# kyotovision-public/DRMNet

Measured on AMD Instinct MI355X. Metric: U-Net denoise steps/sec on 3x128x256 refmaps, higher is better.
Workload: dtype emulated fp32: f16 hi*hi + e4m3 cross terms (~15-bit products), fp32 acc; 1e-4 contract

## Files before the change

### drmnet_amd/_lib.py

```python
from __future__ import annotations

import ctypes as C
import os
from typing import Optional, Sequence

import torch

_HERE = os.path.dirname(os.path.abspath(__file__))
LIB_PATH = os.environ.get("DRM_LIB_PATH") or os.path.join(_HERE, "csrc", "libdrmnet_hip.so")
ABI_VERSION = 3
MAX_LEVELS = 8
LOSS_WORKSPACE_BYTES = 2048
DIFFUSION_LOSS_MAX_PARTS = 32


def diffusion_loss_workspace_bytes(B: int) -> int:
    return int(B) * DIFFUSION_LOSS_MAX_PARTS * 2 * 8


SYMBOLS = [
    "drm_abi_version", "drm_last_error",
    "drm_unet_create", "drm_unet_destroy", "drm_unet_param_count", "drm_unet_param_info", "drm_unet_load_params",
    "drm_unet_workspace_bytes", "drm_unet_forward",
    "drm_linear_forward", "drm_timestep_embedding", "drm_op_norm_act_conv", "drm_op_resblock", "drm_op_attention_block",
    "drm_drmnet_create", "drm_drmnet_destroy", "drm_drmnet_workspace_bytes", "drm_drmnet_set_batch_parts", "drm_drmnet_set_batch_part_min", "drm_drmnet_step", "drm_drmnet_sample",
    "drm_sampler_workspace_bytes", "drm_ddim_sample", "drm_ddim_sample_logged", "drm_ddpm_sample", "drm_ddim_sample_ex", "drm_ddpm_sample_ex", "drm_randn",
    "drm_profile_enable", "drm_profile_reset", "drm_profile_collect", "drm_unet_set_precision", "drm_set_op_precision",
    "drm_refmap_workspace_bytes", "drm_refmap_mask_make", "drm_erode_mask",
    "drm_unet_load_params_set", "drm_unet_use_set", "drm_set_graph_replay", "drm_set_upconv_split", "drm_graph_launches",
    "drm_map_chain", "drm_masked_log_range", "drm_luminance_scale", "drm_mirmap2envmap", "drm_hdr2ldr", "drm_resize", "drm_profile_variants",
    "drm_render_refmap", "drm_brdf_eval", "drm_render_refmap_views", "drm_validation_losses",
    "drm_render_refmap_lit", "drm_render_light_workspace_bytes",
    "drm_render_mesh_workspace_bytes", "drm_render_mesh",
    "drm_mesh_bvh_bytes", "drm_mesh_bvh_build", "drm_mesh_occluded", "drm_render_mesh_shadowed",
    "drm_obs_forward_process", "drm_diffusion_losses",
]


class UNetDesc(C.Structure):
    _fields_ = [
        ("kind", C.c_int32), ("in_channels", C.c_int32), ("model_channels", C.c_int32), ("out_channels", C.c_int32),
        ("num_res_blocks", C.c_int32), ("n_levels", C.c_int32), ("channel_mult", C.c_int32 * MAX_LEVELS),
        ("n_attn", C.c_int32), ("attention_resolutions", C.c_int32 * MAX_LEVELS),
    ]


class MaskBlend(C.Structure):
    _fields_ = [("mask", C.c_void_p), ("mask_channels", C.c_int32), ("x0", C.c_void_p), ("qcoef", C.POINTER(C.c_float)), ("qnoise", C.c_void_p), ("when", C.c_int32)]


class SamplerOptions(C.Structure):
    _fields_ = [("blend", C.POINTER(MaskBlend)), ("uncond", C.c_void_p), ("guidance_scale", C.c_float), ("noise_dropout", C.c_float), ("dropout_keep", C.c_void_p)]


class DrmnetCfg(C.Structure):
    _fields_ = [
        ("z_dim", C.c_int32), ("max_timesteps", C.c_int32), ("gamma", C.c_double), ("epsilon", C.c_float), ("delta", C.c_float),
        ("z0", C.c_float * 8),
    ]


def make_mask_blend(mask, x0, qcoef, qnoise, when: int, img_shape):
    import numpy as np
    import torch

    n, c, h, w = img_shape
    x0 = require_gpu_tensor(x0, "x0").float().contiguous()
    if tuple(x0.shape) != tuple(img_shape):
        raise RuntimeError(f"x0 must be {tuple(img_shape)}")
    mask = require_gpu_tensor(mask, "mask").float()
    if mask.dim() != 4 or mask.shape[2:] != x0.shape[2:] or mask.shape[1] not in (1, c) or mask.shape[0] not in (1, n):
        raise RuntimeError(f"mask must be [N or 1, 1 or {c}, {h}, {w}]")
    mask = mask.expand(n, mask.shape[1], h, w).contiguous()
    qc = np.ascontiguousarray(np.asarray(qcoef, dtype=np.float32))
    qn = None if qnoise is None else require_gpu_tensor(qnoise, "mask_noise").float().contiguous()
    if qn is not None and tuple(qn.shape) != (qc.shape[0],) + tuple(img_shape):
        raise RuntimeError(f"mask_noise must be [steps={qc.shape[0]}, N, C, H, W]")
    b = MaskBlend()
    b.mask, b.mask_channels, b.x0 = mask.data_ptr(), int(mask.shape[1]), x0.data_ptr()
    b.qcoef = qc.ctypes.data_as(C.POINTER(C.c_float))
    b.qnoise = None if qn is None else qn.data_ptr()
    b.when = int(when)
    return b, (mask, x0, qc, qn)


def make_sampler_options(img_shape, steps, blend=None, uncond=None, guidance_scale=1.0, noise_dropout=0.0, dropout_keep=None):
    o = SamplerOptions()
    keep = [blend]
    if blend is not None:
        o.blend = C.pointer(blend[0])
    if uncond is not None:
        u = require_gpu_tensor(uncond, "unconditional_conditioning").float().contiguous()
        if tuple(u.shape) != tuple(img_shape):
            raise RuntimeError(f"unconditional_conditioning must be {tuple(img_shape)}")
        o.uncond = u.data_ptr()
        keep.append(u)
    o.guidance_scale = float(guidance_scale)
    o.noise_dropout = float(noise_dropout)
    if dropout_keep is not None:
        k = require_gpu_tensor(dropout_keep, "dropout_keep").float().contiguous()
        if tuple(k.shape) != (int(steps),) + tuple(img_shape):
            raise RuntimeError(f"dropout_keep must be [steps={steps}, N, C, H, W]")
        o.dropout_keep = k.data_ptr()
        keep.append(k)
    return o, tuple(keep)


_lib: Optional[C.CDLL] = None


def lib() -> C.CDLL:
    global _lib
    if _lib is not None:
        return _lib
    if not os.path.exists(LIB_PATH):
        raise RuntimeError(
            f"{LIB_PATH} is missing: build it with `python -m drmnet_amd.build` (hipcc, gfx950). "
            "drmnet_amd has no CPU / PyTorch fallback for the hot path."
        )
    L = C.CDLL(LIB_PATH)
    vp, i32, i64p, fp = C.c_void_p, C.c_int, C.c_void_p, C.c_void_p
    L.drm_abi_version.restype = C.c_int
    L.drm_last_error.restype = C.c_char_p
    L.drm_unet_create.argtypes = [C.POINTER(UNetDesc), C.POINTER(vp)]
    L.drm_unet_destroy.argtypes = [vp]
    L.drm_unet_destroy.restype = None
    L.drm_unet_param_count.argtypes = [vp]
    L.drm_unet_param_info.argtypes = [vp, i32, C.c_char_p, i32, C.POINTER(C.c_int64), C.POINTER(C.c_int)]
    L.drm_unet_load_params.argtypes = [vp, C.POINTER(vp), i32, vp]
    L.drm_unet_load_params_set.argtypes = [vp, i32, C.POINTER(vp), i32, vp]
    L.drm_unet_use_set.argtypes = [vp, i32]
    L.drm_unet_workspace_bytes.argtypes = [vp, i32, i32, i32]
    L.drm_unet_workspace_bytes.restype = C.c_size_t
    L.drm_unet_forward.argtypes = [vp, fp, i32, fp, i32, vp, fp, i64p, fp, fp, i32, i32, i32, vp, C.c_size_t, vp]
    L.drm_linear_forward.argtypes = [fp, fp, fp, fp, i32, i32, i32, i32, i32, vp]
    L.drm_timestep_embedding.argtypes = [i64p, fp, i32, i32, vp]
    L.drm_op_norm_act_conv.argtypes = [fp, fp, fp, i32, fp, fp, i32, fp, fp, fp, i32, i32, i32, i32, i32, vp]
    L.drm_op_resblock.argtypes = [fp, i32, i32, fp, i32, fp, i32, C.POINTER(vp), i32, fp, i32, i32, i32, i32, vp]
    L.drm_op_attention_block.argtypes = [fp, C.POINTER(vp), fp, i32, i32, i32, i32, vp]
    L.drm_drmnet_create.argtypes = [vp, vp, C.POINTER(vp), C.POINTER(DrmnetCfg), C.POINTER(vp)]
    L.drm_drmnet_destroy.argtypes = [vp]
    L.drm_drmnet_destroy.restype = None
    L.drm_drmnet_workspace_bytes.argtypes = [vp, i32, i32, i32]
    L.drm_drmnet_workspace_bytes.restype = C.c_size_t
    L.drm_drmnet_set_batch_parts.argtypes = [vp, i32]
    L.drm_drmnet_set_batch_parts.restype = i32
    L.drm_drmnet_set_batch_part_min.argtypes = [vp, i32]
    L.drm_drmnet_set_batch_part_min.restype = i32
    L.drm_drmnet_step.argtypes = [vp, fp, fp, vp, i32, i32, fp, C.c_uint64, fp, fp, vp, i32, i32, i32, vp, C.c_size_t, vp]
    L.drm_drmnet_sample.argtypes = [vp, fp, fp, fp, fp, C.c_uint64, i32, fp, fp, vp, C.POINTER(C.c_int32), i32, i32, i32, vp, C.c_size_t, vp]
    L.drm_sampler_workspace_bytes.argtypes = [vp, i32, i32, i32]
    L.drm_sampler_workspace_bytes.restype = C.c_size_t
    L.drm_ddim_sample.argtypes = [vp, fp, fp, C.POINTER(C.c_int64), C.POINTER(C.c_float), i32, i32, fp, C.c_uint64, i32, i32, i32, vp, C.c_size_t, vp]
    L.drm_ddim_sample_logged.argtypes = [vp, fp, fp, C.POINTER(C.c_int64), C.POINTER(C.c_float), i32, i32, fp, C.c_uint64, i32, fp, fp, i32, C.POINTER(C.c_int32),
                                         i32, i32, i32, vp, C.c_size_t, vp]
    L.drm_ddpm_sample.argtypes = [vp, fp, fp, fp, C.POINTER(C.c_float), i32, i32, fp, C.c_uint64, i32, i32, i32, vp, C.c_size_t, vp]
    L.drm_ddim_sample_ex.argtypes = [vp, fp, fp, C.POINTER(C.c_int64), C.POINTER(C.c_float), i32, i32, fp, C.c_uint64, C.POINTER(SamplerOptions), i32, fp, fp, i32,
                                     C.POINTER(C.c_int32), i32, i32, i32, vp, C.c_size_t, vp]
    L.drm_ddpm_sample_ex.argtypes = [vp, fp, fp, fp, C.POINTER(C.c_float), i32, i32, fp, C.c_uint64, C.POINTER(SamplerOptions), i32, i32, i32, vp, C.c_size_t, vp]
    L.drm_randn.argtypes = [fp, C.c_size_t, C.c_uint64, C.c_uint64, vp]
    u8p = vp
    L.drm_refmap_workspace_bytes.argtypes = [C.c_int64, i32, C.c_float]
    L.drm_refmap_workspace_bytes.restype = C.c_size_t
    L.drm_refmap_mask_make.argtypes = [fp, fp, C.c_int64, i32, i32, C.c_float, i32, fp, u8p, vp, C.c_size_t, vp]
    L.drm_erode_mask.argtypes = [u8p, i32, i32, i32, u8p, vp]
    L.drm_unet_set_precision.argtypes = [vp, i32]
    L.drm_set_op_precision.argtypes = [i32]
    L.drm_profile_enable.argtypes = [i32]
    L.drm_profile_enable.restype = None
    L.drm_profile_reset.restype = None
    L.drm_profile_collect.argtypes = [C.POINTER(C.c_double), C.POINTER(C.c_double), C.POINTER(C.c_double), C.POINTER(C.c_int64)]
    L.drm_set_graph_replay.argtypes = [i32]
    L.drm_set_upconv_split.argtypes = [i32]
    L.drm_graph_launches.restype = C.c_int64
    L.drm_map_chain.argtypes = [fp, fp, C.c_int64, i32, C.POINTER(C.c_int32), C.POINTER(C.c_float), i32, fp, fp, fp, vp]
    L.drm_masked_log_range.argtypes = [fp, fp, i32, i32, i32, fp, fp, vp]
    L.drm_luminance_scale.argtypes = [fp, i32, i32, C.c_float, fp, vp]
    L.drm_mirmap2envmap.argtypes = [fp, fp, fp, i32, i32, i32, i32, i32, i32, i32, i32, vp]
    L.drm_hdr2ldr.argtypes = [fp, u8p, i32, C.c_float, C.c_float, fp, vp]
    L.drm_resize.argtypes = [fp, fp, i32, i32, i32, i32, i32, i32, vp]
    L.drm_profile_variants.argtypes = [C.c_char_p, C.c_size_t]
    L.drm_profile_variants.restype = C.c_size_t
    L.drm_render_refmap.argtypes = [fp, fp, fp, i32, i32, i32, i32, i32, i32, i32, vp]
    L.drm_brdf_eval.argtypes = [fp, i32, fp, fp, fp, fp, C.c_int64, vp]
    L.drm_render_refmap_views.argtypes = [fp, i32, fp, fp, fp, i32, i32, i32, i32, i32, i32, i32, vp]
    L.drm_render_refmap_lit.argtypes = [fp, i32, fp, fp, fp, i32, i32, i32, i32, i32, i32, i32, i32, vp, C.c_size_t, vp]
    L.drm_render_light_workspace_bytes.argtypes = [i32, i32, i32, i32]
    L.drm_render_light_workspace_bytes.restype = C.c_size_t
    L.drm_render_mesh_workspace_bytes.argtypes = [C.c_int64, i32, i32, i32, i32]
    L.drm_render_mesh_workspace_bytes.restype = C.c_size_t
    L.drm_render_mesh.argtypes = [fp, fp, vp, C.c_int64, C.c_int64, fp, fp, fp, fp, fp, fp, fp, i32, i32, i32, i32, i32, i32, i32, vp, C.c_size_t, vp]
    L.drm_mesh_bvh_bytes.argtypes = [C.c_int64]
    L.drm_mesh_bvh_bytes.restype = C.c_size_t
    L.drm_mesh_bvh_build.argtypes = [fp, vp, C.c_int64, C.c_int64, vp, C.c_size_t]
    L.drm_mesh_occluded.argtypes = [fp, vp, C.c_int64, C.c_int64, vp, fp, fp, vp, vp, C.c_int64, vp]
    L.drm_render_mesh_shadowed.argtypes = [fp, fp, vp, C.c_int64, C.c_int64, fp, fp, fp, fp, fp, fp, fp, i32, i32, i32, i32, i32, i32, i32, vp, C.c_size_t,
                                           vp, C.c_size_t, vp]
    L.drm_validation_losses.argtypes = [fp, fp, fp, vp, fp, fp, fp, vp, fp, C.c_double, i32, C.c_double, C.c_double, i32, C.c_int64, i32, vp, C.c_size_t,
                                        fp, vp]
    L.drm_obs_forward_process.argtypes = [fp, fp, vp, fp, fp, i32, C.c_float, i32, fp, fp, fp, C.c_uint64, fp, fp, fp, i32, i32, i32, i32, i32, i32, vp]
    L.drm_diffusion_losses.argtypes = [fp, fp, fp, vp, fp, fp, i32, i32, C.c_double, C.c_double, i32, C.c_int64, i32, vp, C.c_size_t, fp, fp, vp]
    if L.drm_abi_version() != ABI_VERSION:
        raise RuntimeError(f"libdrmnet_hip.so ABI version {L.drm_abi_version()} != {ABI_VERSION}: rebuild with `python -m drmnet_amd.build`")
    _lib = L
    return L


def check(status: int) -> None:
    if status != 0:
        msg = lib().drm_last_error()
        raise RuntimeError(f"drmnet_hip error {status}: {msg.decode() if msg else '?'}")


def ptr(t: Optional[torch.Tensor]) -> Optional[int]:
    return None if t is None else t.data_ptr()


def stream_ptr(device=None) -> int:
    return torch.cuda.current_stream(device).cuda_stream


def require_gpu_tensor(t: torch.Tensor, name: str, dtype=torch.float32) -> torch.Tensor:
    if not t.is_cuda:
        raise RuntimeError(f"{name} must live on the GPU (drmnet_amd has no CPU path); got device {t.device}")
    if t.dtype != dtype:
        raise RuntimeError(f"{name} must be {dtype}, got {t.dtype}")
    return t.contiguous()


def ptr_array(tensors: Sequence[torch.Tensor]):
    arr = (C.c_void_p * len(tensors))()
    for i, t in enumerate(tensors):
        arr[i] = t.data_ptr()
    return arr


class Workspace:

    def __init__(self):
        self.buf: Optional[torch.Tensor] = None

    def get(self, nbytes: int, device) -> torch.Tensor:
        if nbytes == 0:
            raise RuntimeError(f"workspace query failed: {lib().drm_last_error().decode()}")
        if self.buf is None or self.buf.numel() < nbytes or self.buf.device != torch.device(device):
            self.buf = None
            self.buf = torch.empty(nbytes, dtype=torch.uint8, device=device)
        return self.buf
```

### drmnet_amd/csrc/abi.hip

```cpp
#include <atomic>
#include <cstring>
#include <memory>

#include "bvh.h"
#include "profiler.h"
#include "samplers.h"

using namespace drm;

struct drm_unet {
  UNet net;
};
struct drm_drmnet {
  DrmnetSampler s;
};

namespace {

int make_arena(Arena& ar, void* ws, size_t bytes, size_t need) {
  if (need == 0) return DRM_ERR_INVALID;
  if (bytes < need || ws == nullptr) {
    set_error("workspace too small: need " + std::to_string(need) + " bytes, got " + std::to_string(bytes));
    return DRM_ERR_WORKSPACE;
  }
// ... 271 lines not shown
  });
}
void drm_drmnet_destroy(drm_drmnet* s) { delete s; }

size_t drm_drmnet_workspace_bytes(const drm_drmnet* s, int N, int H, int W) {
  if (!s) return 0;
  size_t r = 0;
  guarded([&]() -> int {
    r = s->s.workspace_bytes(N, H, W);
    return DRM_OK;
  });
  return r;
}

int drm_drmnet_set_batch_parts(drm_drmnet* s, int parts) {
  return guarded([&]() -> int {
    DRM_REQUIRE(s != nullptr, "drm_drmnet_set_batch_parts: null handle");
    DRM_REQUIRE(parts >= 1 && parts <= DrmnetSampler::PART_MAX, "drm_drmnet_set_batch_parts: 1 .. 4 parts");
    s->s.parts = parts;
    return DRM_OK;
  });
}

int drm_drmnet_set_batch_part_min(drm_drmnet* s, int rows) {
  return guarded([&]() -> int {
    DRM_REQUIRE(s != nullptr, "drm_drmnet_set_batch_part_min: null handle");
    DRM_REQUIRE(rows >= 1, "drm_drmnet_set_batch_part_min: at least one row per part");
    s->s.part_min = rows;
    return DRM_OK;
  });
}

int drm_drmnet_step(drm_drmnet* s, float* Lr_k, const float* LrK, const int32_t* rows, int n_active, int step, const float* noise,
                    uint64_t seed, float* zk_out, float* zK_out, int32_t* converged_out, int B, int H, int W, void* workspace,
                    size_t workspace_bytes, void* stream) {
  return guarded([&]() -> int {
    DRM_REQUIRE(s && Lr_k && LrK, "null argument");
    Arena ar;
    DRM_TRY(make_arena(ar, workspace, workspace_bytes, s->s.workspace_bytes(n_active, H, W)));
    return s->s.step(Lr_k, LrK, rows, n_active, step, noise, seed, zk_out, zK_out, converged_out, B, H, W, ar, static_cast<hipStream_t>(stream));
  });
}

int drm_drmnet_sample(drm_drmnet* s, const float* LrK, const float* cond, const float* noise0, const float* step_noise, uint64_t seed, int early_exit,
                      float* Lr0, float* zK, int32_t* K, int32_t* steps_done, int B, int H, int W, void* workspace, size_t workspace_bytes,
                      void* stream) {
  return guarded([&]() -> int {
    DRM_REQUIRE(s && LrK && cond && Lr0 && zK && K, "null argument");
    Arena ar;
    DRM_TRY(make_arena(ar, workspace, workspace_bytes, s->s.workspace_bytes(B, H, W)));
    return s->s.sample(LrK, cond, noise0, step_noise, seed, early_exit, Lr0, zK, K, steps_done, B, H, W, ar, static_cast<hipStream_t>(stream));
  });
}

size_t drm_sampler_workspace_bytes(const drm_unet* net, int N, int H, int W) {
  if (!net) return 0;
  size_t r = 0;
  guarded([&]() -> int {
    r = sampler_workspace_bytes(&const_cast<drm_unet*>(net)->net, N, H, W);
    return DRM_OK;
  });
  return r;
}

int drm_ddim_sample(drm_unet* net, float* x, const float* cond, const int64_t* timesteps, const float* coef, int S, int num_steps,
                    const float* noise, uint64_t seed, int N, int H, int W, void* workspace, size_t workspace_bytes, void* stream) {
  return guarded([&]() -> int {
    DRM_REQUIRE(net && x && cond, "null argument");
    const ChainIO io{x, cond, noise, seed, N, H, W};
    return run_chain(net, io, workspace, workspace_bytes, [&](Arena& ar) {
      return ddim_sample(&net->net, io, timesteps, coef, S, num_steps, ChainLog{}, drm_sampler_options{}, ar, static_cast<hipStream_t>(stream));
    });
  });
}

int drm_ddim_sample_logged(drm_unet* net, float* x, const float* cond, const int64_t* timesteps, const float* coef, int S, int num_steps,
                           const float* noise, uint64_t seed, int log_every_t, float* log_x, float* log_pred_x0, int log_slots, int32_t* n_logged, int N,
                           int H, int W, void* workspace, size_t workspace_bytes, void* stream) {
  return guarded([&]() -> int {
    DRM_REQUIRE(net && x && cond, "null argument");
    DRM_REQUIRE(log_every_t > 0 && log_x && log_pred_x0 && log_slots > 0, "ddim intermediates: log_every_t, both log buffers and their slot count");
    const ChainIO io{x, cond, noise, seed, N, H, W};
    const ChainLog log{log_every_t, log_x, log_pred_x0, log_slots, n_logged};
    return run_chain(net, io, workspace, workspace_bytes, [&](Arena& ar) {
      return ddim_sample(&net->net, io, timesteps, coef, S, num_steps, log, drm_sampler_options{}, ar, static_cast<hipStream_t>(stream));
    });
  });
}

int drm_ddpm_sample(drm_unet* net, float* x, float* pred_x0, const float* cond, const float* coef, int T_start, int clip_denoised,
                    const float* noise, uint64_t seed, int N, int H, int W, void* workspace, size_t workspace_bytes, void* stream) {
  return guarded([&]() -> int {
    DRM_REQUIRE(net && x && cond, "null argument");
    const ChainIO io{x, cond, noise, seed, N, H, W};
    return run_chain(net, io, workspace, workspace_bytes, [&](Arena& ar) {
      return ddpm_sample(&net->net, io, pred_x0, coef, T_start, clip_denoised, drm_sampler_options{}, ar, static_cast<hipStream_t>(stream));
    });
  });
}

int drm_ddim_sample_ex(drm_unet* net, float* x, const float* cond, const int64_t* timesteps, const float* coef, int S, int num_steps,
                       const float* noise, uint64_t seed, const drm_sampler_options* opt, int log_every_t, float* log_x, float* log_pred_x0, int log_slots,
                       int32_t* n_logged, int N, int H, int W, void* workspace, size_t workspace_bytes, void* stream) {
  return guarded([&]() -> int {
    DRM_REQUIRE(net && x && cond && opt, "null argument");
    DRM_REQUIRE(log_every_t <= 0 || (log_x && log_pred_x0 && log_slots > 0), "ddim intermediates: both log buffers and their slot count");
    const ChainIO io{x, cond, noise, seed, N, H, W};
    ChainLog log{0, nullptr, nullptr, log_slots, n_logged};
    if (log_every_t > 0) log = ChainLog{log_every_t, log_x, log_pred_x0, log_slots, n_logged};
    return run_chain(net, io, workspace, workspace_bytes, [&](Arena& ar) {
      return ddim_sample(&net->net, io, timesteps, coef, S, num_steps, log, *opt, ar, static_cast<hipStream_t>(stream));
    });
  });
}

int drm_ddpm_sample_ex(drm_unet* net, float* x, float* pred_x0, const float* cond, const float* coef, int T_start, int clip_denoised,
                       const float* noise, uint64_t seed, const drm_sampler_options* opt, int N, int H, int W, void* workspace, size_t workspace_bytes,
                       void* stream) {
  return guarded([&]() -> int {
    DRM_REQUIRE(net && x && cond && opt, "null argument");
    DRM_REQUIRE(opt->uncond == nullptr, "drm_ddpm_sample_ex: classifier-free guidance exists on the DDIM chain only (ddim.py:225-232; ddpm.py p_sample has none)");
    const ChainIO io{x, cond, noise, seed, N, H, W};
    return run_chain(net, io, workspace, workspace_bytes, [&](Arena& ar) {
      return ddpm_sample(&net->net, io, pred_x0, coef, T_start, clip_denoised, *opt, ar, static_cast<hipStream_t>(stream));
    });
  });
}

int drm_unet_set_precision(drm_unet* net, int precision) {
  return guarded([&]() -> int {
    DRM_REQUIRE(net && precision_valid(precision),
                "precision must be 0 (fp32 MFMA), 1 (split fp16 x3), 2 (plain fp16 operands), 3 (split fp16 with fp8 cross terms) or 4 (plain bf16 operands)");
    net->net.precision = precision;
    return DRM_OK;
  });
}
int drm_set_op_precision(int precision) {
  return guarded([&]() -> int {
    DRM_REQUIRE(precision_valid(precision),
                "precision must be 0 (fp32 MFMA), 1 (split fp16 x3), 2 (plain fp16 operands), 3 (split fp16 with fp8 cross terms) or 4 (plain bf16 operands)");
    g_op_precision.store(precision, std::memory_order_relaxed);
    return DRM_OK;
  });
}

int drm_set_upconv_split(int mode) {
  return guarded([&]() -> int {
    DRM_REQUIRE(mode >= 0 && mode <= 2, "upconv split mode: 0 = never, 1 = by the measured rule, 2 = wherever the form applies");
    set_upconv_split(mode);
    return DRM_OK;
  });
}

int drm_set_graph_replay(int on) {
  set_graph_replay(on != 0);
  return DRM_OK;
}
int64_t drm_graph_launches(void) { return (int64_t)graph_launches(); }

void drm_profile_enable(int on) { prof_enable(on); }
void drm_profile_reset(void) { prof_reset(); }
int drm_profile_collect(double* ms, double* flops, double* bytes, int64_t* launches) {
  return guarded([&]() -> int {
    DRM_REQUIRE(ms && flops && bytes && launches, "null argument");
    prof_collect(ms, flops, bytes, launches);
    return DRM_OK;
  });
}

int drm_randn(float* out, size_t n, uint64_t seed, uint64_t offset, void* stream) {
  return guarded([&]() -> int { return launch_randn(out, n, seed, offset, static_cast<hipStream_t>(stream)); });
}

size_t drm_refmap_workspace_bytes(int64_t n, int res, float angle_threshold) {
  if (n < 0 || res <= 0 || !(angle_threshold >= 0.f)) return 0;
  return refmap_workspace_bytes(n, res, angle_threshold);
}

int drm_refmap_mask_make(const float* colors, const float* normals, int64_t n, int channels, int res, float angle_threshold, int min_points,
                         float* refmap, uint8_t* refmask, void* workspace, size_t workspace_bytes, void* stream) {
  return guarded([&]() -> int {
    DRM_REQUIRE(refmap && refmask && workspace && (n == 0 || (colors && normals)), "drm_refmap_mask_make: null pointer");
    return launch_refmap_mask_make(colors, normals, n, channels, res, angle_threshold, min_points, refmap, refmask, workspace, workspace_bytes,
                                   static_cast<hipStream_t>(stream));
  });
}

int drm_erode_mask(const uint8_t* mask, int H, int W, int kernel_size, uint8_t* out, void* stream) {
  return guarded([&]() -> int {
    DRM_REQUIRE(mask && out, "drm_erode_mask: null pointer");
    return launch_erode_mask(mask, H, W, kernel_size, out, static_cast<hipStream_t>(stream));
  });
}


int drm_map_chain(const float* x, float* out, int64_t per_image, int B, const int32_t* ops, const float* args, int n_ops, const float* lo,
                  const float* hi, const float* scale, void* stream) {
  return guarded([&]() -> int { return launch_map_chain(x, out, per_image, B, ops, args, n_ops, lo, hi, scale, static_cast<hipStream_t>(stream)); });
}

int drm_masked_log_range(const float* x, const float* mask, int B, int C, int HW, float* lo, float* hi, void* stream) {
  return guarded([&]() -> int { return launch_masked_log_range(x, mask, B, C, HW, lo, hi, static_cast<hipStream_t>(stream)); });
}

int drm_luminance_scale(const float* x, int B, int HW, float scaler, float* scale, void* stream) {
  return guarded([&]() -> int { return launch_luminance_scale(x, B, HW, scaler, scale, static_cast<hipStream_t>(stream)); });
}

int drm_mirmap2envmap(const float* mirmap, const float* basis, float* out, int B, int C, int H, int W, int OH, int OW, int log_scale_interpolation,
                      int channels_last, void* stream) {
  return guarded([&]() -> int {
    return launch_mirmap2envmap(mirmap, basis, out, B, C, H, W, OH, OW, log_scale_interpolation, channels_last, static_cast<hipStream_t>(stream));
  });
}

int drm_hdr2ldr(const float* x, const uint8_t* mask, int HW, float alpha, float gamma, float* out, void* stream) {
  return guarded([&]() -> int { return launch_hdr2ldr(x, mask, HW, alpha, gamma, out, static_cast<hipStream_t>(stream)); });
}

size_t drm_profile_variants(char* buf, size_t cap) { return prof_variants_text(buf, cap); }

int drm_resize(const float* x, float* out, int planes, int IH, int IW, int OH, int OW, int mode, void* stream) {
  return guarded([&]() -> int { return launch_resize(x, out, planes, IH, IW, OH, OW, mode, static_cast<hipStream_t>(stream)); });
}


int drm_render_refmap(const float* z, const float* envmap, float* out, int B, int R, int EH, int EW, int quad, int subpixel, int flip, void* stream) {
  return guarded([&]() -> int {
    return launch_render_refmap(z, envmap, out, B, R, EH, EW, quad, subpixel, flip, static_cast<hipStream_t>(stream));
  });
}

int drm_render_refmap_views(const float* z, int L, const float* envmap, const float* view, float* out, int B, int R, int EH, int EW, int quad,
                            int subpixel, int flip, void* stream) {
  return guarded([&]() -> int {
    return launch_render_refmap_views(z, L, envmap, view, out, B, R, EH, EW, quad, subpixel, flip, static_cast<hipStream_t>(stream));
  });
}

size_t drm_render_light_workspace_bytes(int B, int EH, int EW, int light_samples) { return render_light_workspace_bytes(B, EH, EW, light_samples); }

int drm_render_refmap_lit(const float* z, int L, const float* envmap, const float* view, float* out, int B, int R, int EH, int EW, int quad, int subpixel,
                          int flip, int light_samples, void* workspace, size_t workspace_bytes, void* stream) {
  return guarded([&]() -> int {
    return launch_render_refmap_lit(z, L, envmap, view, out, B, R, EH, EW, quad, subpixel, flip, light_samples, workspace, workspace_bytes,
                                    static_cast<hipStream_t>(stream));
  });
}

size_t drm_render_mesh_workspace_bytes(int64_t F, int B, int H, int W, int subpixel) {
  return render_mesh_workspace_bytes((long long)F, B, H, W, subpixel);
}

int drm_render_mesh(const float* vertex_positions, const float* vertex_normals, const int32_t* faces, int64_t V, int64_t F, const float* z,
                    const float* envmap, const float* view, float* image, float* normal, float* depth, float* alpha, int B, int H, int W, int EH, int EW,
                    int quad, int subpixel, void* workspace, size_t workspace_bytes, void* stream) {
  return guarded([&]() -> int {
    return launch_render_mesh(vertex_positions, vertex_normals, faces, (long long)V, (long long)F, z, envmap, view, image, normal, depth, alpha, B, H, W,
                              EH, EW, quad, subpixel, workspace, workspace_bytes, static_cast<hipStream_t>(stream));
  });
}

size_t drm_mesh_bvh_bytes(int64_t F) { return mesh_bvh_bytes((long long)F); }

int drm_mesh_bvh_build(const float* vertex_positions, const int32_t* faces, int64_t V, int64_t F, void* bvh, size_t bytes) {
  return guarded([&]() -> int { return mesh_bvh_build(vertex_positions, faces, (long long)V, (long long)F, bvh, bytes); });
}

int drm_mesh_occluded(const float* vertex_positions, const int32_t* faces, int64_t V, int64_t F, const void* bvh, const float* origins, const float* dirs,
                      const int32_t* exclude, int32_t* out, int64_t N, void* stream) {
  return guarded([&]() -> int {
    return launch_mesh_occluded(vertex_positions, faces, (long long)V, (long long)F, bvh, origins, dirs, exclude, out, (long long)N,
                                static_cast<hipStream_t>(stream));
  });
}

int drm_render_mesh_shadowed(const float* vertex_positions, const float* vertex_normals, const int32_t* faces, int64_t V, int64_t F, const float* z,
                             const float* envmap, const float* view, float* image, float* normal, float* depth, float* alpha, int B, int H, int W, int EH,
                             int EW, int quad, int subpixel, void* workspace, size_t workspace_bytes, const void* bvh, size_t bvh_bytes, void* stream) {
  return guarded([&]() -> int {
    return launch_render_mesh_shadowed(vertex_positions, vertex_normals, faces, (long long)V, (long long)F, z, envmap, view, image, normal, depth, alpha, B,
                                       H, W, EH, EW, quad, subpixel, workspace, workspace_bytes, bvh, bvh_bytes, static_cast<hipStream_t>(stream));
  });
}

int drm_brdf_eval(const float* z, int z_rows, const float* n, const float* v, const float* l, float* out, int64_t N, void* stream) {
  return guarded([&]() -> int { return launch_brdf_eval(z, z_rows, n, v, l, out, (long long)N, static_cast<hipStream_t>(stream)); });
}


int drm_validation_losses(const float* model_out, const float* Lr_k, const float* Lr_km1, const int32_t* K, const float* z_out, const float* z_k,
                          const float* z_K, const int32_t* reversed_k, const float* z0, double gamma, int loss_type, double l_refmap_weight,
                          double l_refcode_weight, int B, int64_t per_row, int P, void* workspace, size_t workspace_bytes, float* out, void* stream) {
  return guarded([&]() -> int {
    return launch_validation_losses(model_out, Lr_k, Lr_km1, K, z_out, z_k, z_K, reversed_k, z0, gamma, loss_type, l_refmap_weight, l_refcode_weight, B,
                                    (long long)per_row, P, static_cast<double*>(workspace), workspace_bytes, out, static_cast<hipStream_t>(stream));
  });
}


int drm_obs_forward_process(const float* x, const float* mask, const int32_t* t, const float* sqrt_alphas_cumprod,
                            const float* sqrt_one_minus_alphas_cumprod, int T, float noisy_observe, int padding_mode, const float* e_observe,
                            const float* e_padding, const float* e_q, uint64_t seed, float* cond, float* x_noisy, float* noise, int B, int C, int H,
                            int W, int mask_H, int mask_W, void* stream) {
  return guarded([&]() -> int {
    return launch_obs_forward_process(x, mask, t, sqrt_alphas_cumprod, sqrt_one_minus_alphas_cumprod, T, noisy_observe, padding_mode, e_observe, e_padding,
// ... 16 lines not shown
```

### drmnet_amd/csrc/common.h

```cpp
#pragma once
#include <hip/hip_runtime.h>
#include <stdint.h>
#include <stdio.h>
#include <string>
#include "gn_fold.h"

namespace drm {

void set_error(const std::string& msg);
const char* last_error();

#define DRM_OK 0
#define DRM_ERR_INVALID 1
#define DRM_ERR_HIP 2
#define DRM_ERR_WORKSPACE 3
#define DRM_ERR_STATE 4

#define DRM_HIP_CHECK(expr)                                                                              \
  do {                                                                                                   \
    hipError_t _e = (expr);                                                                              \
    if (_e != hipSuccess) {                                                                              \
      ::drm::set_error(std::string(#expr) + " failed: " + hipGetErrorString(_e) + " at " + __FILE__ + ":" + \
                       std::to_string(__LINE__));                                                        \
      return DRM_ERR_HIP;                                                                                \
    }                                                                                                    \
  } while (0)

#define DRM_REQUIRE(cond, msg)                                    \
  do {                                                            \
    if (!(cond)) {                                                \
      ::drm::set_error(std::string("invalid argument: ") + (msg)); \
      return DRM_ERR_INVALID;                                     \
    }                                                             \
  } while (0)

#define DRM_TRY(expr)          \
  do {                         \
    int _s = (expr);           \
    if (_s != DRM_OK) return _s; \
  } while (0)

struct DeviceInfo {
  int ordinal = 0;
  int cus = 0;
  int xcds = 0;
  size_t lds_per_cu = 0;
};
const DeviceInfo* device_info();


struct ConvArgs {
  const float* src0 = nullptr;
  const float* src1 = nullptr;
  int C0 = 0, C1 = 0, up0 = 0;
  int N = 0, H = 0, W = 0;
  const float* gn_scale = nullptr;
  const float* gn_shift = nullptr;
  int silu = 0;
  const float* w = nullptr;
  const float* bias = nullptr;
  int taps = 9;
  int Cout = 0;
  const float* emb = nullptr;
  int emb_stride = 0;
  const float* res = nullptr;
  float* out = nullptr;
  int out_nchw = 0, cout_valid = 0;
  int cin_real = 0;
  int ksplit = 1;
  size_t split_stride = 0;
  float* split_ws = nullptr;
  unsigned* tile_ticket = nullptr;
  int terms = 3;
  int mx_site = 0;
#ifdef DRM_S2_STAMP
  unsigned* stamp_out = nullptr;
  int stamp_block = 0, stamp_tile0 = 0;
#endif
  double2* stat_out = nullptr;
  float* pool_out = nullptr;
  double2* pool_stat = nullptr;
  const float* w_inv_scale = nullptr;
  int ld0 = 0;
  int gn_ld = 0;
  long long w_img_stride_f4 = 0;
  const float* w_inv_img = nullptr;
  int prof_kind = -1;
  const float* in_inv = nullptr;
  GnFold gnf;
};
enum ConvKernel : unsigned char { CONV_NONE, CONV_IGEMM, CONV_PIPELINE };
enum ConvTile : unsigned char { TILE_256x256, TILE_256x192, TILE_256x128, TILE_128x128, TILE_256x64, TILE_128x64, TILE_128x32 };
enum SplitFinish : unsigned char { SPLIT_NONE, SPLIT_IN_LAUNCH, SPLIT_REDUCE };
struct ConvPlan {
  ConvKernel kernel = CONV_NONE;
  int terms = 0;
  ConvTile tile = TILE_128x32;
  int th = 0, tw = 0;
  bool ragged = false;
  int kc = 32;
  int ksplit = 1;
  SplitFinish finish = SPLIT_NONE;
  size_t tickets = 0;
  bool pool = false;
  bool gn_fold = false;
  bool split() const { return kernel == CONV_PIPELINE && terms != 0; }
};
ConvPlan plan_conv(const ConvArgs& a, int precision, bool want_pool = false, bool gn_foldable = false);
bool conv_split_weights(int precision, int cin);
int launch_conv(const ConvArgs& a, const ConvPlan& p, hipStream_t s);
int conv_tile_family(int H, int W, const int (*fam)[2], int n_fam);
size_t packed_conv_weight_split_floats(int taps, int CoutP, int CinP);
int launch_pack_conv_weight_split(const float* w, float* packed, float* scales, unsigned* scratch, int Cout, int Cin, int taps, int CoutP,
                                  int CinP, hipStream_t s, bool mx = false, bool bf16 = false);
enum Precision { PREC_FP32 = 0, PREC_F16X3 = 1, PREC_F16 = 2, PREC_F16MX = 3, PREC_BF16 = 4 };
inline bool precision_valid(int p) { return p >= PREC_FP32 && p <= PREC_BF16; }
inline int precision_terms(int p) { return p == PREC_F16 ? 1 : (p == PREC_BF16 ? 4 : (p == PREC_FP32 ? 0 : 3)); }
int launch_pack_conv_weight(const float* w, float* packed, int Cout, int Cin, int taps, int CoutP, int CinP, hipStream_t s);
int pack_conv_image(int precision, const float* w, float* packed, float* scale, unsigned* scratch, int Cout, int Cin, int taps, int CoutP, int CinP,
                    bool mx_site, hipStream_t s);
int launch_fold_upconv_weight(const float* w, float* wa, float* wb, int Cout, int C0, int C1, hipStream_t s);
int launch_fold_attn_params(const float* qkv_w, const float* qkv_b, const float* proj_w, const float* proj_b, float* w_out, float* b_out, int C,
                            hipStream_t s);
size_t packed_conv_weight_floats(int taps, int CoutP, int CinP);

int launch_chan_moments(const float* x, int N, int HW, int C, double* partial , double2* mom , hipStream_t s);
int chan_moments_splits(int HW, int C);
int launch_act_pow2_scale(const double2* mom0, int C0, int lo0, int hi0, double cnt0, const double2* mom1, int C1, double cnt1,
                          const unsigned* absmax_bits, int Ctab, int N, float* scale, float* shift, float* inv, hipStream_t s, int absmax_parts = 1);
int launch_gn_finalize(const double2* mom0, int C0, double inv0, const double2* mom1, int C1, double inv1, const float* gamma,
                       const float* beta, int N, float* scale, float* shift, hipStream_t s, double cnt0 = 0.0, double cnt1 = 0.0,
                       float* guard_scale = nullptr, float* guard_shift = nullptr, float* guard_inv = nullptr);

size_t refmap_workspace_bytes(long long n, int res, float thr);
int launch_refmap_mask_make(const float* colors, const float* normals, long long n, int C, int res, float thr, int min_points, float* refmap,
                            unsigned char* refmask, void* ws, size_t ws_bytes, hipStream_t s);
int launch_erode_mask(const unsigned char* mask, int H, int W, int k, unsigned char* out, hipStream_t s);
enum AttnForm : unsigned char {
  ATTN_SMALL,
  ATTN_CONV,
  ATTN_FLASH
};
struct AttnPlan {
  AttnForm form = ATTN_SMALL;
  int N = 0, H = 0, W = 0, C = 0;
  int terms = 0;
  bool split_qk = false, split_pv = false, guard = false;
  int group = 1;
  size_t scores_floats = 0;
  size_t ws_floats = 0;
  bool out_stats = true;
  ConvPlan qk[2], pv[2];
};
AttnPlan plan_attention(int N, int H, int W, int C, int precision);
struct AttnTables {
  float *wq = nullptr, *wk = nullptr, *wv = nullptr;
  float *q_tab = nullptr, *p_tab = nullptr, *zero_tab = nullptr;
  float *qk_inv = nullptr, *k_scale = nullptr, *k_inv = nullptr, *pv_inv = nullptr, *v_scale = nullptr, *v_inv = nullptr;
  float* q_scale = nullptr;
};
int launch_attention_core(const AttnPlan& p, const float* qkv, const double2* qkv_mom, const float* x, float* scores, float* out, double2* out_stat,
                          float* ws, hipStream_t s);
bool attention_flash_applicable(int T, int C, int terms);
int launch_attention_flash(const AttnPlan& p, const AttnTables& t, const float* qkv, const float* x, float* out, hipStream_t s);

int launch_map_chain(const float* x, float* out, long long per_image, int B, const int32_t* ops, const float* args, int n_ops, const float* lo,
                     const float* hi, const float* scale, hipStream_t s);
int launch_masked_log_range(const float* x, const float* mask, int B, int C, int HW, float* lo, float* hi, hipStream_t s);
int launch_luminance_scale(const float* x, int B, int HW, float scaler, float* scale, hipStream_t s);
int launch_mirmap2envmap(const float* mir, const float* basis, float* out, int B, int C, int H, int W, int OH, int OW, int log_interp, int nhwc,
                         hipStream_t s);
int launch_hdr2ldr(const float* x, const unsigned char* mask, int HW, float alpha, float gamma, float* out, hipStream_t s);
int launch_resize(const float* x, float* out, int planes, int IH, int IW, int OH, int OW, int mode, hipStream_t s);

int launch_render_refmap(const float* z, const float* env, float* out, int B, int R, int EH, int EW, int quad, int subpixel, int flip, hipStream_t s);
int launch_render_refmap_views(const float* z, int L, const float* env, const float* view, float* out, int B, int R, int EH, int EW, int quad,
                               int subpixel, int flip, hipStream_t s);
size_t render_light_workspace_bytes(int B, int EH, int EW, int light_samples);
int launch_render_refmap_lit(const float* z, int L, const float* env, const float* view, float* out, int B, int R, int EH, int EW, int quad, int subpixel,
                             int flip, int light_samples, void* workspace, size_t workspace_bytes, hipStream_t s);
constexpr int kMeshRecordWords = 20, kMeshHitWords = 4;
constexpr int kMeshRecIndex = 14, kMeshRecValid = 17;
__host__ __device__ __forceinline__ float mesh_sample_x(int c, int WS) { return (float)(2 * c + 1) / (float)WS - 1.0f; }
__host__ __device__ __forceinline__ float mesh_sample_y(int r, int HS, float aspect) { return aspect * (1.0f - (float)(2 * r + 1) / (float)HS); }
size_t render_mesh_workspace_bytes(long long F, int B, int H, int W, int subpixel);
int launch_mesh_visibility(const float* positions, const int32_t* faces, long long V, long long F, const float* view, int B, int H, int W, int subpixel,
                           float* records, float* hits, hipStream_t s);
int launch_render_mesh(const float* positions, const float* normals, const int32_t* faces, long long V, long long F, const float* z, const float* env,
                       const float* view, float* image, float* normal, float* depth, float* alpha, int B, int H, int W, int EH, int EW, int quad,
                       int subpixel, void* workspace, size_t workspace_bytes, hipStream_t s);
int launch_render_mesh_shadowed(const float* positions, const float* normals, const int32_t* faces, long long V, long long F, const float* z,
                                const float* env, const float* view, float* image, float* normal, float* depth, float* alpha, int B, int H, int W, int EH,
                                int EW, int quad, int subpixel, void* workspace, size_t workspace_bytes, const void* bvh, size_t bvh_bytes, hipStream_t s);
int launch_validation_losses(const float* model_out, const float* Lr_k, const float* Lr_km1, const int32_t* K, const float* z_out, const float* z_k,
                             const float* z_K, const int32_t* reversed_k, const float* z0, double gamma, int loss_type, double w_refmap,
                             double w_refcode, int B, long long per_row, int P, double* ws, size_t ws_bytes, float* out, hipStream_t s);
int launch_obs_forward_process(const float* x, const float* mask, const int32_t* t, const float* sqrt_ac, const float* sqrt_1mac, int T,
                               float noisy_observe, int padding_mode, const float* e_obs, const float* e_pad, const float* e_q, uint64_t seed,
                               float* cond, float* x_noisy, float* noise, int B, int C, int H, int W, int mask_H, int mask_W, hipStream_t s);
int launch_diffusion_losses(const float* model_out, const float* target, const float* invmask, const int32_t* t, const float* logvar,
                            const float* lvlb, int T, int loss_type, double w_simple, double w_elbo, int B, long long per_row, int C, double* ws,
                            size_t ws_bytes, float* out, float* rows_out, hipStream_t s);
int launch_brdf_eval(const float* z, int z_rows, const float* n, const float* v, const float* l, float* out, long long N, hipStream_t s);

int pack_input_absmax_parts(int H, int W);
int launch_pack_input(const float* x, const float* cond, const int* idx, float* out, int N, int H, int W, int Cx, int Cc, int CP, hipStream_t s,
                      unsigned* absmax_bits = nullptr);
int launch_avgpool2(const float* x, float* out, int N, int H, int W, int C, hipStream_t s, double2* stat = nullptr);
int launch_linear(const float* in, const float* w, const float* b, float* out, int N, int I, int O, int silu_in, int silu_out, hipStream_t s);
int launch_timestep_embedding(const int64_t* t, const float* tf, float* out, int N, int dim, hipStream_t s);
int launch_encoder_head(const float* x, const float* scale, const float* shift, const float* w, const float* b, float* out, int N, int HW,
                        int C, int O, hipStream_t s);
bool stem_direct_applicable(int Cin, int Cout);
size_t stem_weight_floats();
int launch_pack_stem_weight(const float* w, float* img, int Cout, int Cin, bool exact, hipStream_t s);
int launch_stem_conv(const float* x, int Cx, const float* cond, int Cc, const int* rows, const float* wimg, const float* bias, float* out, double2* stat,
                     int N, int H, int W, int Cout, bool exact, hipStream_t s);
int launch_nhwc_to_nchw(const float* x, float* out, int N, int H, int W, int C, hipStream_t s);
int launch_nchw_to_nhwc(const float* x, float* out, int N, int H, int W, int C, hipStream_t s);

}
```

### drmnet_amd/csrc/conv_split2.hip

```cpp
#include <algorithm>
#include <atomic>
#include <utility>
#include <vector>
#include <cstdio>
#include <string>

#include "common.h"
#include "profiler.h"

#ifdef DRM_S2_STAMP
#define S2_STAMP(id)                                                                               \
  do {                                                                                             \
    if (stamp_on && stamp_n < 120) {                                                               \
      unsigned long long t_;                                                                       \
      __builtin_amdgcn_sched_barrier(0);                                                           \
      asm volatile("s_memtime %0\n\ts_waitcnt lgkmcnt(0)" : "=s"(t_)::"memory");                   \
      __builtin_amdgcn_sched_barrier(0);                                                           \
      if (lane == 0) {                                                                             \
        stamp_lds[(wave * 120 + stamp_n) * 2] = (unsigned)(id);                                    \
        stamp_lds[(wave * 120 + stamp_n) * 2 + 1] = (unsigned)t_;                                  \
      }                                                                                            \
      ++stamp_n;                                                                                   \
    }                                                                                              \
  } while (0)
// ... 51 lines not shown
  static constexpr int G_PER = TPS * B_PER;
  static constexpr int G_F4 = TPS * B_F4;
  static constexpr int ST_F4 = TN * BN;
  static constexpr int LDS_F4 = A_F4 + R * G_F4 + ST_F4;
  static constexpr int A_CNT = 2 * A_SLOTS + 4;
  static __device__ __forceinline__ void rowmap(int row, int& img, int& py, int& px) {
    if constexpr (SUB48) {
      constexpr int SPI = (TH / 4) * (TW / 8);
      const int q = row >> 5, rr = row & 31;
      img = q / SPI;
      const int qq = q % SPI;
      py = (qq / (TW / 8)) * 4 + (rr >> 3);
      px = (qq % (TW / 8)) * 8 + (rr & 7);
    } else {
      img = row / (TH * TW);
      py = (row / TW) % TH;
      px = row % TW;
    }
  }
  static_assert(TAPS == 9 || TAPS == 4 || TAPS == 1, "3x3, 1x1, or the four parity 2x2 convs of a 3x3 over a nearest-x2 input");
  static_assert(TAPS % TPS == 0, "taps per step must divide the taps");
  static_assert(B_DMA_F4 % 64 == 0 && B_PER >= 1, "whole 1-KiB LDS-DMA instructions; a wave issues B_PER of them or none");
  static_assert(TERMS == 4 || TERMS == 3 || TERMS == 2 || TERMS == 1 || TERMS == 0,
                "3 = fp16 hi/lo split (fp32 accuracy), 2 = fp16 hi*hi + both cross terms in one block-scaled fp8 MFMA, 1 = plain fp16 operands, 4 = plain bf16 operands, 0 = fp32 operands (exact fp32 MFMA)");
  static_assert(ONE || B_DMA_F4 % NTHR == 0, "split mode: every wave owns the same number of distinct 1-KiB pieces");
  static_assert(TH * TW * TN == BM && TPI % OCT == 0 && TPI >= OCT, "tile / loader mapping");
  static_assert(R >= 2, "ring needs >= 2 slots");
};

__device__ __forceinline__ float silu2(float v) { return v * __builtin_amdgcn_rcpf(1.0f + __expf(-v)); }
__device__ __forceinline__ void split2(float v, _Float16& hi, _Float16& lo) {
  const float c = __builtin_amdgcn_fmed3f(v, -65504.0f, 65504.0f);
  hi = (_Float16)c;
  lo = (_Float16)fmaf((float)hi, -1.0f, c);
}
typedef float f32x2 __attribute__((ext_vector_type(2)));
typedef _Float16 f16x2 __attribute__((ext_vector_type(2)));
__device__ __forceinline__ unsigned cvt_pk_f16(float a, float b) { return __builtin_bit_cast(unsigned, __builtin_convertvector(f32x2{a, b}, f16x2)); }
template <int HALF>
__device__ __forceinline__ float sub_packed_f16(float c, unsigned pk) {
  float r;
  if constexpr (HALF == 0) asm("v_fma_mix_f32 %0, %1, 1.0, -%2 op_sel_hi:[0,0,1]" : "=v"(r) : "v"(c), "v"(pk));
  else asm("v_fma_mix_f32 %0, %1, 1.0, -%2 op_sel:[0,0,1] op_sel_hi:[0,0,1]" : "=v"(r) : "v"(c), "v"(pk));
  return r;
}
__device__ __forceinline__ void split8(const float (&v)[8], float lim_n, float lim_p, float (&c8)[8], unsigned (&hi)[4], float (&l8)[8]) {
#pragma unroll
  for (int k = 0; k < 8; ++k) c8[k] = __builtin_amdgcn_fmed3f(v[k], lim_n, lim_p);
#pragma unroll
  for (int k = 0; k < 4; ++k) {
    hi[k] = cvt_pk_f16(c8[2 * k], c8[2 * k + 1]);
    l8[2 * k] = sub_packed_f16<0>(c8[2 * k], hi[k]);
    l8[2 * k + 1] = sub_packed_f16<1>(c8[2 * k + 1], hi[k]);
  }
}
union F4H8b {
  float4 f4;
  f16x8 h8;
  bf16x8 b8;
};

template <int N>
__device__ __forceinline__ void wait_vmcnt() {
  static_assert(N >= 0 && N < 64, "vmcnt is a 6-bit counter");
  asm volatile("s_waitcnt vmcnt(%0)" ::"n"(N) : "memory");
}

__device__ __forceinline__ void glds16s(const void* sbase, unsigned voff, unsigned lds_dst) {
  unsigned keep;
  asm volatile("s_mov_b32 %0, m0\n\ts_mov_b32 m0, %3\n\ts_nop 0\n\tglobal_load_lds_dwordx4 %1, %2\n\ts_mov_b32 m0, %0"
               : "=&s"(keep)
               : "v"(voff), "s"(sbase), "s"(lds_dst)
               : "memory");
}
__device__ __forceinline__ void glds16(const void* gsrc, unsigned lds_dst) {
  unsigned keep;
  asm volatile("s_mov_b32 %0, m0\n\ts_mov_b32 m0, %2\n\ts_nop 0\n\tglobal_load_lds_dwordx4 %1, off\n\ts_mov_b32 m0, %0"
               : "=&s"(keep)
               : "v"(gsrc), "s"(lds_dst)
               : "memory");
}

typedef float f32x4 __attribute__((ext_vector_type(4)));
__device__ __forceinline__ void gload16x2(f32x4& d0, f32x4& d1, const void* p) {
  asm volatile("global_load_dwordx4 %0, %2, off\n\tglobal_load_dwordx4 %1, %2, off offset:16" : "=&v"(d0), "=&v"(d1) : "v"(p) : "memory");
}
__device__ __forceinline__ void tie_regs(f32x4& x0, f32x4& x1) { asm volatile("" : "+v"(x0), "+v"(x1)::"memory"); }
#ifdef DRM_SK_FENCED
__device__ __forceinline__ void gstore16_agent(void* p, const f32x4& v) { asm volatile("global_store_dwordx4 %0, %1, off\n\ts_nop 1" ::"v"(p), "v"(v) : "memory"); }
__device__ __forceinline__ void gload16_agent(f32x4& d, const void* p) { asm volatile("global_load_dwordx4 %0, %1, off" : "=&v"(d) : "v"(p) : "memory"); }
#else
__device__ __forceinline__ void gstore16_agent(void* p, const f32x4& v) { asm volatile("global_store_dwordx4 %0, %1, off sc1\n\ts_nop 1" ::"v"(p), "v"(v) : "memory"); }
__device__ __forceinline__ void gload16_agent(f32x4& d, const void* p) { asm volatile("global_load_dwordx4 %0, %1, off sc1" : "=&v"(d) : "v"(p) : "memory"); }
#endif
__device__ __forceinline__ void tie_reg(f32x4& x) { asm volatile("" : "+v"(x)::"memory"); }

template <int CTRL>
__device__ __forceinline__ float quad_perm(float x) {
  return __builtin_bit_cast(float, __builtin_amdgcn_update_dpp(0, __builtin_bit_cast(int, x), CTRL, 0xF, 0xF, false));
}
__device__ __forceinline__ void quad_transpose(float& x0, float& x1, float& x2, float& x3, int lane) {
  const bool b0 = lane & 1, b1 = lane & 2;
  float t;
  t = quad_perm<0xB1>(b0 ? x0 : x1);
  if (b0) x0 = t; else x1 = t;
  t = quad_perm<0xB1>(b0 ? x2 : x3);
  if (b0) x2 = t; else x3 = t;
  t = quad_perm<0x4E>(b1 ? x0 : x2);
  if (b1) x0 = t; else x2 = t;
  t = quad_perm<0x4E>(b1 ? x1 : x3);
  if (b1) x1 = t; else x3 = t;
}

template <int... I, typename F>
__device__ __forceinline__ void static_for(std::integer_sequence<int, I...>, F&& f) {
  (f(std::integral_constant<int, I>{}), ...);
}

struct TilePos {
  int n0, ty0, tx0, co0;
  long long wofs;
};

template <int TAPS, int TH, int TW, int WM, int WN, int MT, int NT, int R, int TPS, int TERMS = 3, bool RAG = false, bool SK = false, bool POOL = false>
__global__ __launch_bounds__(WM* WN * 64, 2) void conv_split2_kernel(ConvArgs a) {
  using C = S2Cfg<TAPS, TH, TW, WM, WN, MT, NT, R, TPS, TERMS>;
  static_assert(!POOL || (C::SUB48 && C::TN == 1 && !RAG && !SK), "pooled output: one-image tiles of 4 x 8 patches");
  extern __shared__ float4 lds[];
  float4* As = lds;
  float4* Bs = lds + C::A_F4;
  double* lst = reinterpret_cast<double*>(lds + C::A_F4 + R * C::G_F4);
  [[maybe_unused]] double* lst2 = lst + C::TN * C::BN * 2;

#ifndef DRM_NO_KERNARG_TOUCH
  {
    typedef const __attribute__((address_space(4))) int* kptr_t;
    kptr_t ka = (kptr_t)__builtin_amdgcn_kernarg_segment_ptr();
    int touch = 0;
#pragma unroll
    for (int o = 0; o < (int)sizeof(ConvArgs); o += 64) touch ^= __builtin_nontemporal_load(ka + o / 4);
    asm volatile("" ::"s"(touch));
  }
#endif
  const int tid = threadIdx.x;
  const int lane = tid & 63;
  const int wave = __builtin_amdgcn_readfirstlane(tid >> 6);
  const int r = lane & 31, h = lane >> 5;
  const int wm = wave / WN, wn = wave % WN;

  const int tiles_x = RAG ? (a.W + TW - 1) / TW : a.W / TW, tiles_y = RAG ? (a.H + TH - 1) / TH : a.H / TH;
  const int n_tiles = a.Cout / C::BN;
  const int total = ((a.N + C::TN - 1) / C::TN) * tiles_y * tiles_x * n_tiles;
  const int xcd = blockIdx.x & 7, jx = blockIdx.x >> 3;
  const int q8 = total >> 3, r8 = total & 7;
  const int x_start = xcd < r8 ? xcd * (q8 + 1) : r8 * (q8 + 1) + (xcd - r8) * q8;
  const int x_count = q8 + (xcd < r8 ? 1 : 0);
  const int J = ((int)gridDim.x - xcd + 7) >> 3;
  auto decode = [&](int logical) {
    TilePos t;
    const int n_tile = logical % n_tiles;
    int m_tile = logical / n_tiles;
    const int tx = m_tile % tiles_x;
    m_tile /= tiles_x;
    const int ty = m_tile % tiles_y;
    t.n0 = (m_tile / tiles_y) * C::TN;
    t.ty0 = ty * TH;
    t.tx0 = tx * TW;
    t.co0 = n_tile * C::BN;
    t.wofs = t.co0 + (long long)t.n0 * a.w_img_stride_f4;
    return t;
  };
  int k_tile = jx;
  if (k_tile >= x_count) return;
  TilePos cur = decode(x_start + k_tile);
#ifdef DRM_S2_STAMP
  unsigned* stamp_lds = reinterpret_cast<unsigned*>(lds + C::LDS_F4);
  int stamp_n = 0;
  int stamp_tiles = 0;
  bool stamp_on = false;
  if (a.stamp_out && (int)blockIdx.x == (a.stamp_block & 0xFFFF))
    for (int k = tid; k < C::NW * 240; k += C::NTHR) stamp_lds[k] = 0;
  stamp_on = a.stamp_out && (int)blockIdx.x == (a.stamp_block & 0xFFFF) && a.stamp_tile0 == 0;
  S2_STAMP(60);
#endif

  const int Ctot = a.C0 + a.C1;
  const int nch_all = Ctot / C::KC;
  const int ks = a.ksplit > 1 ? a.ksplit : 1;
  const int split = blockIdx.y;
  const int chunk0 = split * nch_all / ks;
  const int nchunks = (split + 1) * nch_all / ks - chunk0;
  const int NGT = nchunks * C::NG;
  constexpr bool FUSE = SK;
  static_assert(!SK || (WM == 4 && WN == 1 && MT == 1 && NT == 1 && !RAG), "split-K launches use the 128-row x 32-channel tiles (plan_conv)");
  const bool fused = FUSE && ks > 1 && a.split_ws != nullptr;
  float* const out_s = (fused ? a.split_ws : a.out) + (size_t)split * a.split_stride;
  const bool has_gn = a.gn_scale != nullptr;

  const int l_img = tid / C::TPI;
  const int l_tid = tid % C::TPI;
  const int l_o = tid % C::OCT;
  f32x4 areg[C::A_SLOTS][2];
  f32x4 sc[2], sh[2];
  unsigned avalid = 0;

  auto load_A_piece = [&](const TilePos& tp, int chunk, int piece) {
    const int c = (chunk0 + chunk) * C::KC;
    const float* src;
    int Cs, coff, up;
    if (c < a.C0) {
      src = a.src0; Cs = a.ld0 ? a.ld0 : a.C0; coff = c; up = a.up0;
    } else {
      src = a.src1; Cs = a.C1; coff = c - a.C0; up = 0;
    }
    const int Hs = up ? (a.H >> 1) : a.H, Ws = up ? (a.W >> 1) : a.W;
    const int l_n = tp.n0 + l_img;
    const int l_nc = l_n < a.N ? l_n : a.N - 1;
    if (piece == 0) avalid = 0;
#pragma unroll
    for (int j = 0; j < C::A_SLOTS; ++j) {
      if (j != piece) continue;
      const int lidx = l_tid + C::TPI * j;
      const int hpl = lidx / C::OCT;
      const int hy = hpl / C::WT, hx = hpl % C::WT;
      const int y = tp.ty0 + hy - C::HALO, x = tp.tx0 + hx - C::HALO;
      const bool ok = (lidx < C::HPI * C::OCT) && (l_n < a.N) && (y >= 0) && (y < a.H) && (x >= 0) && (x < a.W);
      const int yc = min(max(y, 0), a.H - 1), xc = min(max(x, 0), a.W - 1);
      const int ys = up ? (yc >> 1) : yc, xs = up ? (xc >> 1) : xc;
      const size_t pix = ((size_t)l_nc * Hs + ys) * Ws + xs;
      gload16x2(areg[j][0], areg[j][1], src + pix * Cs + coff + 8 * l_o);
      if (ok) avalid |= 1u << j;
    }
    if (piece == C::A_SLOTS) {
      const int tab_ld = a.gn_ld ? a.gn_ld : Ctot;
      const float* gs = has_gn ? a.gn_scale + (size_t)l_nc * tab_ld + c + 8 * l_o : a.src0;
      const float* gb = has_gn ? a.gn_shift + (size_t)l_nc * tab_ld + c + 8 * l_o : a.src0;
      gload16x2(sc[0], sc[1], gs);
      gload16x2(sh[0], sh[1], gb);
    }
  };
  auto load_A = [&](const TilePos& tp, int chunk) {
#pragma unroll
    for (int p = 0; p <= C::A_SLOTS; ++p) load_A_piece(tp, chunk, p);
  };
  auto tie_A = [&]() {
#pragma unroll
    for (int j = 0; j < C::A_SLOTS; ++j) tie_regs(areg[j][0], areg[j][1]);
    tie_regs(sc[0], sc[1]);
    tie_regs(sh[0], sh[1]);
  };
  auto transform_A_slot = [&](int j) {
    const int lidx = l_tid + C::TPI * j;
    if (lidx < C::HPI * C::OCT) {
      float v[8] = {areg[j][0].x, areg[j][0].y, areg[j][0].z, areg[j][0].w, areg[j][1].x, areg[j][1].y, areg[j][1].z, areg[j][1].w};
      if (has_gn) {
        const float s8[8] = {sc[0].x, sc[0].y, sc[0].z, sc[0].w, sc[1].x, sc[1].y, sc[1].z, sc[1].w};
        const float b8[8] = {sh[0].x, sh[0].y, sh[0].z, sh[0].w, sh[1].x, sh[1].y, sh[1].z, sh[1].w};
#pragma unroll
        for (int k = 0; k < 8; ++k) v[k] = fmaf(v[k], s8[k], b8[k]);
      }
      if (a.silu) {
#pragma unroll
        for (int k = 0; k < 8; ++k) v[k] = silu2(v[k]);
      }
      const bool ok = (avalid >> j) & 1u;
      if constexpr (TERMS == 0) {
        areg[j][0] = ok ? f32x4{v[0], v[1], v[2], v[3]} : f32x4{0.f, 0.f, 0.f, 0.f};
        areg[j][1] = ok ? f32x4{v[4], v[5], v[6], v[7]} : f32x4{0.f, 0.f, 0.f, 0.f};
      } else if constexpr (TERMS == 2) {
        float c8[8], l8[8];
        unsigned hi[4];
        split8(v, ok ? -MX_A_LIM : 0.f, ok ? MX_A_LIM : 0.f, c8, hi, l8);
        s16x2 q[4];
#pragma unroll
        for (int k = 0; k < 2; ++k) {
          s16x2 z = {0, 0};
          z = __builtin_amdgcn_cvt_scalef32_pk_fp8_f32(z, l8[4 * k], l8[4 * k + 1], MX_AL_DIV, false);
          q[k] = __builtin_amdgcn_cvt_scalef32_pk_fp8_f32(z, l8[4 * k + 2], l8[4 * k + 3], MX_AL_DIV, true);
          s16x2 y = {0, 0};
          y = __builtin_amdgcn_cvt_scalef32_pk_fp8_f32(y, c8[4 * k], c8[4 * k + 1], MX_AH_DIV, false);
          q[2 + k] = __builtin_amdgcn_cvt_scalef32_pk_fp8_f32(y, c8[4 * k + 2], c8[4 * k + 3], MX_AH_DIV, true);
        }
        areg[j][0] = f32x4{__builtin_bit_cast(float, hi[0]), __builtin_bit_cast(float, hi[1]), __builtin_bit_cast(float, hi[2]), __builtin_bit_cast(float, hi[3])};
        areg[j][1] = f32x4{__builtin_bit_cast(float, q[0]), __builtin_bit_cast(float, q[1]), __builtin_bit_cast(float, q[2]), __builtin_bit_cast(float, q[3])};
      } else if constexpr (TERMS == 4) {
        F4H8b hi;
#pragma unroll
        for (int k = 0; k < 8; ++k) hi.b8[k] = (__bf16)(ok ? v[k] : 0.f);
        areg[j][0] = f32x4{hi.f4.x, hi.f4.y, hi.f4.z, hi.f4.w};
      } else {
        float c8[8], l8[8];
        unsigned hi[4];
        split8(v, ok ? -65504.0f : 0.f, ok ? 65504.0f : 0.f, c8, hi, l8);
        areg[j][0] = f32x4{__builtin_bit_cast(float, hi[0]), __builtin_bit_cast(float, hi[1]), __builtin_bit_cast(float, hi[2]), __builtin_bit_cast(float, hi[3])};
        if constexpr (TERMS == 3)
          areg[j][1] = f32x4{__builtin_bit_cast(float, cvt_pk_f16(l8[0], l8[1])), __builtin_bit_cast(float, cvt_pk_f16(l8[2], l8[3])),
                             __builtin_bit_cast(float, cvt_pk_f16(l8[4], l8[5])), __builtin_bit_cast(float, cvt_pk_f16(l8[6], l8[7]))};
      }
    }
  };
  auto write_A_slot = [&](float4* Ad, int j) {
    const int lidx = l_tid + C::TPI * j;
    if (lidx < C::HPI * C::OCT) {
      const int hpl = lidx / C::OCT;
      const int pixel = l_img * C::HPIP + (hpl / C::WT) * C::WTP + (hpl % C::WT);
      const float4 w0 = make_float4(areg[j][0].x, areg[j][0].y, areg[j][0].z, areg[j][0].w);
      const float4 w1 = make_float4(areg[j][1].x, areg[j][1].y, areg[j][1].z, areg[j][1].w);
      if constexpr (TERMS == 0) {
        Ad[(2 * l_o) * C::HPS + pixel] = w0;
        Ad[(2 * l_o + 1) * C::HPS + pixel] = w1;
      } else if constexpr (TERMS == 2) {
        Ad[l_o * C::HPS + pixel] = w0;
        reinterpret_cast<float2*>(Ad + (4 + (l_o >> 1)) * C::HPS + pixel)[l_o & 1] = make_float2(w1.x, w1.y);
        reinterpret_cast<float2*>(Ad + (6 + (l_o >> 1)) * C::HPS + pixel)[l_o & 1] = make_float2(w1.z, w1.w);
      } else {
        Ad[l_o * C::HPS + pixel] = w0;
        if (TERMS == 3) Ad[(4 + l_o) * C::HPS + pixel] = w1;
      }
    }
  };
  auto transform_A = [&]() {
    tie_A();
#pragma unroll
    for (int j = 0; j < C::A_SLOTS; ++j) transform_A_slot(j);
  };
  auto write_A = [&](float4* Ad) {
#pragma unroll
    for (int j = 0; j < C::A_SLOTS; ++j) write_A_slot(Ad, j);
  };
  auto store_A = [&](float4* Ad) {
    transform_A();
    write_A(Ad);
  };
  const unsigned lds_bs = __builtin_amdgcn_readfirstlane(
      (unsigned)(uintptr_t)(__attribute__((address_space(3))) void*)(Bs));
  unsigned dma_voff[C::B_PER];
#pragma unroll
  for (int j = 0; j < C::B_PER; ++j) {
    const int idx = (wave * 64 + C::NTHR * j) % C::B_DMA_F4 + lane;
    dma_voff[j] = (unsigned)((idx / C::BN) * a.Cout + idx % C::BN) * 16u;
  }
  auto issue_G1 = [&](int gseq, int g_in_tile, long long co0, int k) {
    const int slot = gseq % R;
    const int chunk = g_in_tile / C::NG, g = g_in_tile - chunk * C::NG;
    const int u = k / C::B_PER, j = k % C::B_PER;
    const int tap = g * TPS + u;
    const float4* wp = reinterpret_cast<const float4*>(a.w) + (((size_t)tap * nch_all + chunk0 + chunk) * 8) * a.Cout + co0;
    const int base = (wave * 64 + C::NTHR * j) % C::B_DMA_F4;
    unsigned vo = dma_voff[0];
#pragma unroll
    for (int jj = 1; jj < C::B_PER; ++jj) vo = (j == jj) ? dma_voff[jj] : vo;
    glds16s(wp, vo, lds_bs + (unsigned)(slot * C::G_F4 + u * C::B_F4 + base) * 16u);
  };
  auto issue_G = [&](int gseq, int g_in_tile, long long co0) {
    const int slot = gseq % R;
    const int chunk = g_in_tile / C::NG, g = g_in_tile - chunk * C::NG;
#pragma unroll
    for (int u = 0; u < TPS; ++u) {
      const int tap = g * TPS + u;
      const float4* wp = reinterpret_cast<const float4*>(a.w) + (((size_t)tap * nch_all + chunk0 + chunk) * 8) * a.Cout + co0;
#pragma unroll
      for (int j = 0; j < C::B_PER; ++j) {
        const int base = (wave * 64 + C::NTHR * j) % C::B_DMA_F4;
        glds16s(wp, dma_voff[j], lds_bs + (unsigned)(slot * C::G_F4 + u * C::B_F4 + base) * 16u);
      }
    }
  };

  int a_base[MT], b_base[NT];
#pragma unroll
  for (int i = 0; i < MT; ++i) {
    const int row = (wm * MT + i) * 32 + r;
    int img, py, px;
    C::rowmap(row, img, py, px);
    a_base[i] = img * C::HPIP + py * C::WTP + px;
  }
#pragma unroll
  for (int c = 0; c < NT; ++c) b_base[c] = (wn * NT + c) * 32 + r;

  f32x16 acc[MT][NT];
#pragma unroll
  for (int i = 0; i < MT; ++i)
#pragma unroll
    for (int c = 0; c < NT; ++c)
#pragma unroll
      for (int e = 0; e < 16; ++e) acc[i][c][e] = 0.f;

  const float inv_scale = a.w_inv_scale ? *a.w_inv_scale : 1.0f;
  constexpr int PPI = TH * TW;
  const bool st = a.stat_out != nullptr;
  if (st) {
    for (int k = tid; k < C::TN * C::BN * 2; k += C::NTHR) lst[k] = 0.0;
  }
  if constexpr (POOL) {
    for (int k = tid; k < C::TN * C::BN * 2; k += C::NTHR) lst2[k] = 0.0;
  }

  int gseq = 0;
  {
    int k2 = k_tile;
    TilePos tp = cur;
    int gi = 0;
#pragma unroll
    for (int G = 0; G < R - 1; ++G) {
      if (gi >= NGT) {
        gi = 0;
        if (k2 + J < x_count) {
          k2 += J;
          tp = decode(x_start + k2);
        }
      }
      issue_G(gseq++, gi++, tp.wofs);
    }
  }
  S2_STAMP(61);
  if (a.gnf.mom0) {
    float* scr = reinterpret_cast<float*>(As);
    const bool tab_in_lds = a.N == 1 && (80 + 2 * Ctot) * (int)sizeof(float) <= C::A_F4 * 16;
#pragma unroll
    for (int p = 0; p < C::A_SLOTS; ++p) load_A_piece(cur, 0, p);
    for (int n = 0; n < a.N; ++n) gn_finalize_image(a.gnf, n, tid, C::NTHR, scr, tab_in_lds ? scr + 80 : nullptr);
    S2_STAMP(62);
    wait_vmcnt<0>();
    if (!tab_in_lds) {
      gn_lds_barrier();
      load_A_piece(cur, 0, C::A_SLOTS);
    } else {
      const float4* t4 = reinterpret_cast<const float4*>(scr + 80 + chunk0 * C::KC + 8 * l_o);
      const float4 s0 = t4[0], s1 = t4[1], b0 = t4[Ctot / 4], b1 = t4[Ctot / 4 + 1];
      sc[0] = f32x4{s0.x, s0.y, s0.z, s0.w}; sc[1] = f32x4{s1.x, s1.y, s1.z, s1.w};
      sh[0] = f32x4{b0.x, b0.y, b0.z, b0.w}; sh[1] = f32x4{b1.x, b1.y, b1.z, b1.w};
      gn_lds_barrier();
    }
  } else {
    load_A(cur, 0);
  }
  wait_vmcnt<0>();
  S2_STAMP(63);
  store_A(As);
  if (TAPS == 1) {
    if (nchunks > 1) load_A(cur, 1);
    else if (k_tile + J < x_count) load_A(decode(x_start + k_tile + J), 0);
  }
  asm volatile("s_waitcnt lgkmcnt(0)" ::: "memory");
  __builtin_amdgcn_s_barrier();
  S2_STAMP(64);

  constexpr int A_G = (C::NG >= 3) ? C::NG - 2 : 0;
  const bool y_first = (C::NW == 8) && (wave >= C::NW / 2);
  if (TAPS != 1 && C::NW == 8 && wave >= C::NW / 2) __builtin_amdgcn_s_setprio(1);
  constexpr int BASE = C::G_PER * (R - 2);
  int step = 0;
  while (true) {
    const bool has_next = k_tile + J < x_count;
    const TilePos nxt = has_next ? decode(x_start + k_tile + J) : cur;
#ifdef DRM_S2_STAMP
    stamp_on = a.stamp_out && (int)blockIdx.x == (a.stamp_block & 0xFFFF) && stamp_tiles >= a.stamp_tile0;
    ++stamp_tiles;
    S2_STAMP(1);
#endif
    [[maybe_unused]] int par_off = 0;
    if constexpr (TAPS == 4) {
      const int par = cur.co0 / (a.Cout >> 2);
      par_off = __builtin_amdgcn_readfirstlane((par >> 1) * C::WTP + (par & 1));
    }
    auto mma_tap = [&](const float4* Ab, const float4* Bc, int tapoff, auto&& hook) {
      if constexpr (TERMS == 0) {
#pragma unroll
        for (int j = 0; j < 4; ++j) {
          const int gi = 2 * j + h;
          float4 af[MT], bf[NT];
#pragma unroll
          for (int i = 0; i < MT; ++i) af[i] = Ab[gi * C::HPS + a_base[i] + tapoff];
#pragma unroll
          for (int c = 0; c < NT; ++c) bf[c] = Bc[gi * C::BN + b_base[c]];
#pragma unroll
          for (int i = 0; i < MT; ++i)
#pragma unroll
            for (int c = 0; c < NT; ++c) {
              acc[i][c] = __builtin_amdgcn_mfma_f32_32x32x2f32(af[i].x, bf[c].x, acc[i][c], 0, 0, 0);
              acc[i][c] = __builtin_amdgcn_mfma_f32_32x32x2f32(af[i].y, bf[c].y, acc[i][c], 0, 0, 0);
              acc[i][c] = __builtin_amdgcn_mfma_f32_32x32x2f32(af[i].z, bf[c].z, acc[i][c], 0, 0, 0);
              acc[i][c] = __builtin_amdgcn_mfma_f32_32x32x2f32(af[i].w, bf[c].w, acc[i][c], 0, 0, 0);
            }
          if (j == 0 || j == 2) {
            __builtin_amdgcn_sched_barrier(0);
            hook(j >> 1);
            __builtin_amdgcn_sched_barrier(0);
          }
        }
        return;
      }
      if constexpr (TERMS == 2) {
        {
          i32x8 am[MT], bm[NT];
#pragma unroll
          for (int i = 0; i < MT; ++i) {
            const float4 p0 = Ab[(4 + h) * C::HPS + a_base[i] + tapoff], p1 = Ab[(6 + h) * C::HPS + a_base[i] + tapoff];
            am[i] = i32x8{__builtin_bit_cast(int, p0.x), __builtin_bit_cast(int, p0.y), __builtin_bit_cast(int, p0.z), __builtin_bit_cast(int, p0.w),
                          __builtin_bit_cast(int, p1.x), __builtin_bit_cast(int, p1.y), __builtin_bit_cast(int, p1.z), __builtin_bit_cast(int, p1.w)};
          }
#pragma unroll
          for (int c = 0; c < NT; ++c) {
            const float4 p0 = Bc[(4 + h) * C::BN + b_base[c]], p1 = Bc[(6 + h) * C::BN + b_base[c]];
            bm[c] = i32x8{__builtin_bit_cast(int, p0.x), __builtin_bit_cast(int, p0.y), __builtin_bit_cast(int, p0.z), __builtin_bit_cast(int, p0.w),
                          __builtin_bit_cast(int, p1.x), __builtin_bit_cast(int, p1.y), __builtin_bit_cast(int, p1.z), __builtin_bit_cast(int, p1.w)};
          }
          const int sa = h ? MX_SA_AH : MX_SA_AL, sb = h ? MX_SB_BL : MX_SB_BH;
#pragma unroll
          for (int i = 0; i < MT; ++i)
#pragma unroll
            for (int c = 0; c < NT; ++c) acc[i][c] = __builtin_amdgcn_mfma_scale_f32_32x32x64_f8f6f4(am[i], bm[c], acc[i][c], 0, 0, 0, sa, 0, sb);
        }
        __builtin_amdgcn_sched_barrier(0);
        hook(0);
        __builtin_amdgcn_sched_barrier(0);
#pragma unroll
        for (int s2 = 0; s2 < 2; ++s2) {
          const int seg = s2 * 2 + h;
          F4H8b ah[MT], bh[NT];
#pragma unroll
          for (int i = 0; i < MT; ++i) ah[i].f4 = Ab[seg * C::HPS + a_base[i] + tapoff];
#pragma unroll
          for (int c = 0; c < NT; ++c) bh[c].f4 = Bc[seg * C::BN + b_base[c]];
#pragma unroll
          for (int i = 0; i < MT; ++i)
#pragma unroll
            for (int c = 0; c < NT; ++c) acc[i][c] = __builtin_amdgcn_mfma_f32_32x32x16_f16(ah[i].h8, bh[c].h8, acc[i][c], 0, 0, 0);
          if (s2 == 0) {
            __builtin_amdgcn_sched_barrier(0);
            hook(1);
            __builtin_amdgcn_sched_barrier(0);
          }
        }
        return;
      }
#pragma unroll
      for (int s2 = 0; s2 < 2; ++s2) {
        const int seg = s2 * 2 + h;
        F4H8b ah[MT], al[MT], bh[NT], bl[NT];
#pragma unroll
        for (int i = 0; i < MT; ++i) {
          ah[i].f4 = Ab[seg * C::HPS + a_base[i] + tapoff];
          if (TERMS == 3) al[i].f4 = Ab[(4 + seg) * C::HPS + a_base[i] + tapoff];
        }
#pragma unroll
        for (int c = 0; c < NT; ++c) {
          bh[c].f4 = Bc[seg * C::BN + b_base[c]];
          if (TERMS == 3) bl[c].f4 = Bc[(4 + seg) * C::BN + b_base[c]];
        }
        static_for(std::make_integer_sequence<int, 3>{}, [&](auto tc) {
          constexpr int t = decltype(tc)::value;
          constexpr int T0 = (TERMS == 3) ? 0 : 2;
          if constexpr (t >= T0) {
#pragma unroll
            for (int i = 0; i < MT; ++i)
#pragma unroll
              for (int c = 0; c < NT; ++c) {
                if constexpr (t == 0) acc[i][c] = __builtin_amdgcn_mfma_f32_32x32x16_f16(al[i].h8, bh[c].h8, acc[i][c], 0, 0, 0);
                if constexpr (t == 1) acc[i][c] = __builtin_amdgcn_mfma_f32_32x32x16_f16(ah[i].h8, bl[c].h8, acc[i][c], 0, 0, 0);
                if constexpr (t == 2 && TERMS != 4) acc[i][c] = __builtin_amdgcn_mfma_f32_32x32x16_f16(ah[i].h8, bh[c].h8, acc[i][c], 0, 0, 0);
                if constexpr (t == 2 && TERMS == 4) acc[i][c] = __builtin_amdgcn_mfma_f32_32x32x16_bf16(ah[i].b8, bh[c].b8, acc[i][c], 0, 0, 0);
              }
            if constexpr (t == T0) {
              __builtin_amdgcn_sched_barrier(0);
              hook(s2);
              __builtin_amdgcn_sched_barrier(0);
            }
          }
        });
      }
    };
    auto issue_ahead = [&](int gi0) {
      int gi = gi0 + (R - 1);
// ... 383 lines not shown
            for (int g = 0; g < 4; ++g) ev[g] = a.emb ? a.emb[(size_t)nimg[g] * a.emb_stride + co] : 0.f;
#pragma unroll
            for (int e = 0; e < 16; ++e) rv[e] = a.res ? a.res[(pixb[e >> 2] + (e & 3)) * a.Cout + co] : 0.f;
            auto sum_groups = [&](auto G0c, auto NGc, auto NKc) {
              constexpr int G0 = decltype(G0c)::value, NGR = decltype(NGc)::value, NK = decltype(NKc)::value;
              f32x4 t[NGR][NK];
#pragma unroll
              for (int gg = 0; gg < NGR; ++gg)
#pragma unroll
                for (int k = 0; k < NK; ++k)
                  gload16_agent(t[gg][k], &a.split_ws[(size_t)(k < ks ? k : 0) * a.split_stride + (pixb[G0 + gg] + (r & 3)) * a.Cout + cq]);
              asm volatile("s_waitcnt vmcnt(0)" ::: "memory");
#pragma unroll
              for (int gg = 0; gg < NGR; ++gg)
#pragma unroll
                for (int k = 0; k < NK; ++k) tie_reg(t[gg][k]);
#pragma unroll
              for (int gg = 0; gg < NGR; ++gg) {
                f32x4 sacc = t[gg][0];
#pragma unroll
                for (int k = 1; k < NK; ++k)
                  if (k < ks) { sacc.x += t[gg][k].x; sacc.y += t[gg][k].y; sacc.z += t[gg][k].z; sacc.w += t[gg][k].w; }
                const int g = G0 + gg;
                v[4 * g] = sacc.x; v[4 * g + 1] = sacc.y; v[4 * g + 2] = sacc.z; v[4 * g + 3] = sacc.w;
                quad_transpose(v[4 * g], v[4 * g + 1], v[4 * g + 2], v[4 * g + 3], r);
              }
            };
            using I0 = std::integral_constant<int, 0>;
            using I2 = std::integral_constant<int, 2>;
            using I4 = std::integral_constant<int, 4>;
            using I8 = std::integral_constant<int, 8>;
            if (ks <= 4) {
              sum_groups(I0{}, I4{}, I4{});
            } else {
              sum_groups(I0{}, I2{}, I8{});
              sum_groups(I2{}, I2{}, I8{});
            }
            S2_STAMP(74);
            float s0 = 0.f, q0 = 0.f, s1 = 0.f, q1 = 0.f;
#pragma unroll
            for (int e = 0; e < 16; ++e) {
              const int g = e >> 2;
              const float x = v[e] + bias + ev[g] + rv[e];
              v[e] = x;
              if (okg[g]) {
                if (e < 8) { s0 += x; q0 += x * x; } else { s1 += x; q1 += x * x; }
              }
            }
#pragma unroll
            for (int g = 0; g < 4; ++g) {
              quad_transpose(v[4 * g], v[4 * g + 1], v[4 * g + 2], v[4 * g + 3], r);
              if (okg[g]) *reinterpret_cast<float4*>(&a.out[(pixb[g] + (r & 3)) * a.Cout + cq]) = make_float4(v[4 * g], v[4 * g + 1], v[4 * g + 2], v[4 * g + 3]);
            }
            if (st) {
              const int row0 = wm * 32;
              if (PPI >= 32) {
                s0 += s1;
                q0 += q1;
              }
              double* d = lst + ((size_t)(row0 / PPI) * C::BN + col) * 2;
              atomicAdd(d, (double)s0);
              atomicAdd(d + 1, (double)q0);
              if (PPI < 32) {
                double* d2 = lst + ((size_t)((row0 + 16) / PPI) * C::BN + col) * 2;
                atomicAdd(d2, (double)s1);
                atomicAdd(d2 + 1, (double)q1);
              }
            }
            fused_last = true;
            S2_STAMP(75);
          }
        }
      }
    }
    if constexpr (TAPS == 4) {
      static_assert(!RAG && !SK && !POOL, "the parity form has no ragged, split-K or pooled instantiation");
      const int CoutR = a.Cout >> 2;
      const int par = cur.co0 / CoutR, pa = par >> 1, pb = par & 1;
      const int cob = cur.co0 - par * CoutR;
      const size_t H2 = 2 * (size_t)a.H, W2 = 2 * (size_t)a.W;
#pragma unroll
      for (int i = 0; i < MT; ++i) {
        size_t pix2[4];
        bool okg[4];
#pragma unroll
        for (int g = 0; g < 4; ++g) {
          const int row = (wm * MT + i) * 32 + 8 * g + 4 * h;
          int img, py, px;
          C::rowmap(row, img, py, px);
          const int n = cur.n0 + img;
          okg[g] = n < a.N;
          pix2[g] = ((size_t)(okg[g] ? n : a.N - 1) * H2 + (2 * (cur.ty0 + py) + pa)) * W2 + (2 * (cur.tx0 + px) + pb);
        }
#pragma unroll
        for (int c = 0; c < NT; ++c) {
          const int cq = cob + (wn * NT + c) * 32 + (r & ~3);
#pragma unroll
          for (int g = 0; g < 4; ++g) {
            float v0 = acc[i][c][4 * g] * inv_scale, v1 = acc[i][c][4 * g + 1] * inv_scale, v2 = acc[i][c][4 * g + 2] * inv_scale,
                  v3 = acc[i][c][4 * g + 3] * inv_scale;
#pragma unroll
            for (int k = 0; k < 4; ++k) acc[i][c][4 * g + k] = 0.f;
            quad_transpose(v0, v1, v2, v3, r);
            if (okg[g]) *reinterpret_cast<float4*>(&a.out[(pix2[g] + 2 * (r & 3)) * CoutR + cq]) = make_float4(v0, v1, v2, v3);
          }
        }
      }
    }
    if (st && (ks == 1 || fused_last) && (!has_next || nxt.n0 != cur.n0 || nxt.co0 != cur.co0)) {
      asm volatile("s_waitcnt lgkmcnt(0)" ::: "memory");
      __builtin_amdgcn_s_barrier();
      for (int k = tid; k < C::TN * C::BN * 2; k += C::NTHR) {
        const int img = k / (C::BN * 2), rem = k % (C::BN * 2);
        const int n = cur.n0 + img;
#ifdef DRM_S2_STAMP
        if (a.stamp_block & 0x40000) {
          if (n < a.N) *(reinterpret_cast<double*>(a.stat_out + (size_t)n * a.Cout + cur.co0) + rem) = lst[k];
        } else
#endif
        if (n < a.N) atomicAdd(reinterpret_cast<double*>(a.stat_out + (size_t)n * a.Cout + cur.co0) + rem, lst[k]);
        lst[k] = 0.0;
        if constexpr (POOL) {
          atomicAdd(reinterpret_cast<double*>(a.pool_stat + (size_t)n * a.Cout + cur.co0) + rem, lst2[k]);
          lst2[k] = 0.0;
        }
      }
      asm volatile("s_waitcnt lgkmcnt(0)" ::: "memory");
      __builtin_amdgcn_s_barrier();
    }
    S2_STAMP(10);
    if (!has_next) break;
    k_tile += J;
    cur = nxt;
  }
  wait_vmcnt<0>();
#ifdef DRM_S2_STAMP
  if (a.stamp_out && (int)blockIdx.x == (a.stamp_block & 0xFFFF)) {
    asm volatile("s_waitcnt lgkmcnt(0)" ::: "memory");
    __builtin_amdgcn_s_barrier();
    for (int k = tid; k < C::NW * 240; k += C::NTHR) a.stamp_out[k] = stamp_lds[k];
  }
#endif
}

template <int TAPS, int TH, int TW, int WM, int WN, int MT, int NT, int R, int TPS, int TERMS = 3, bool RAG = false, bool SK = false, bool POOL = false>
static int launch_s2(const ConvArgs& a, hipStream_t s) {
  using C = S2Cfg<TAPS, TH, TW, WM, WN, MT, NT, R, TPS, TERMS>;
  auto kern = conv_split2_kernel<TAPS, TH, TW, WM, WN, MT, NT, R, TPS, TERMS, RAG, SK, POOL>;
  DRM_REQUIRE(RAG || (a.H % TH == 0 && a.W % TW == 0), "conv tile does not divide the map");
  DRM_REQUIRE(POOL == (a.pool_out != nullptr), "pooled output: only launches plan_conv pools");
  DRM_REQUIRE(!POOL || (a.pool_stat && a.stat_out && a.ksplit <= 1 && !a.out_nchw), "pooled output: needs both statistics tables, no split-K");
  if constexpr (TAPS == 4) {
    static_assert(!RAG && !SK && !POOL, "the parity form has no ragged, split-K or pooled instantiation");
    DRM_REQUIRE(!a.bias && !a.emb && !a.res && !a.stat_out && !a.out_nchw && a.ksplit <= 1 && !a.gnf.mom0 && !a.in_inv && a.w_img_stride_f4 == 0,
                "parity (4-tap) conv: weight un-scaling only -- no bias, emb, residual, statistics, split-K or GroupNorm fold");
    DRM_REQUIRE(a.C1 == 0 && !a.up0 && a.Cout % 4 == 0 && (a.Cout / 4) % C::BN == 0, "parity (4-tap) conv: one stored source, a Cout tile inside one parity");
  }
  const size_t lds_bytes = (size_t)(C::LDS_F4 + (POOL ? C::ST_F4 : 0)) * sizeof(float4);
  static_assert((C::LDS_F4 + (POOL ? C::ST_F4 : 0)) * 16 <= 160 * 1024, "LDS budget");
  const DeviceInfo* di = device_info();
  if (!di) return DRM_ERR_STATE;
  static std::atomic<uint64_t> attr_mask{0};
  if (lds_bytes > 48 * 1024 && !(attr_mask.load(std::memory_order_acquire) >> di->ordinal & 1)) {
    DRM_HIP_CHECK(hipFuncSetAttribute(reinterpret_cast<const void*>(kern), hipFuncAttributeMaxDynamicSharedMemorySize, (int)lds_bytes));
    attr_mask.fetch_or(uint64_t(1) << di->ordinal, std::memory_order_release);
  }
  const int groups = (a.N + C::TN - 1) / C::TN;
  const long long tiles = (long long)groups * ((a.H + TH - 1) / TH) * ((a.W + TW - 1) / TW) * (a.Cout / C::BN);
  DRM_REQUIRE(tiles > 0 && tiles < (1ll << 31), "conv grid size");
  const int per_cu = std::max(1, std::min((int)(di->lds_per_cu / lds_bytes), 8 / C::NW));
  long long grid = (long long)di->cus * per_cu;
  const int ngt = ((a.C0 + a.C1) / C::KC) * C::NG;
  const int ks = a.ksplit > 1 ? a.ksplit : 1;
  constexpr bool FUSE = SK;
  DRM_REQUIRE(ks == 1 || (!a.out_nchw && a.split_stride > 0 && a.w_img_stride_f4 == 0 && ((a.C0 + a.C1) / C::KC) / ks >= 1 && ks <= 8 &&
                          (a.split_ws ? (FUSE && a.tile_ticket != nullptr) : !a.stat_out)),
              "split-K launch contract");
  if (tiles < grid || ngt < R - 1 || (TAPS == 1 && ngt < 2) || ks > 1) grid = tiles;
  {
    const double cin = a.cin_real > 0 ? a.cin_real : (a.C0 + a.C1), cout = a.out_nchw ? a.cout_valid : a.Cout;
    const double px = (double)a.N * a.H * a.W;
    const double px_in = (double)a.N * ((a.H >> a.up0) * (a.W >> a.up0)) * a.C0 + px * a.C1;
    prof_tag(a.N, a.H, a.W, a.C0 + a.C1, a.Cout);
    if (prof_enabled()) {
      static const std::string vname = [] {
        char b[192];
        snprintf(b, sizeof b, "void drm::conv_split2_kernel<%d, %d, %d, %d, %d, %d, %d, %d, %d, %d, %s, %s, %s>", TAPS, TH, TW, WM, WN, MT, NT, R, TPS, TERMS,
                 RAG ? "true" : "false", SK ? "true" : "false", POOL ? "true" : "false");
        return std::string(b);
      }();
      prof_variant(vname.c_str());
    }
    DRM_REQUIRE(a.w_img_stride_f4 == 0 || (C::TN == 1 && ks == 1), "per-image weights need one image per tile (H*W a multiple of the 256-pixel tile)");
    constexpr int ALG_TAPS = (TAPS == 4) ? 9 : TAPS;
    ProfScope ps(a.prof_kind == PROF_KINDS ? -1 : (a.prof_kind >= 0 ? a.prof_kind : (TAPS != 1 ? PROF_CONV3 : PROF_CONV1)), 2.0 * px * ALG_TAPS * cin * cout,
                 4.0 * (px_in + px * cout * (a.res ? 2 : 1) + (double)TAPS * cin * cout), s);
#ifdef DRM_S2_STAMP
    static const char* stamp_file = getenv("DRM_S2_STAMP_FILE");
    if (stamp_file && lds_bytes + 7680 <= di->lds_per_cu) {
      static unsigned* dbuf = nullptr;
      if (!dbuf) DRM_HIP_CHECK(hipMalloc(reinterpret_cast<void**>(&dbuf), 8192));
      DRM_HIP_CHECK(hipMemsetAsync(dbuf, 0, 8192, s));
      ConvArgs at = a;
      at.stamp_out = dbuf;
      at.stamp_block = getenv("DRM_S2_STAMP_BLOCK") ? atoi(getenv("DRM_S2_STAMP_BLOCK")) : 8;
      at.stamp_tile0 = getenv("DRM_S2_STAMP_TILE0") ? atoi(getenv("DRM_S2_STAMP_TILE0")) : 2;
      DRM_HIP_CHECK(hipFuncSetAttribute(reinterpret_cast<const void*>(kern), hipFuncAttributeMaxDynamicSharedMemorySize, (int)lds_bytes + 7680));
      hipLaunchKernelGGL(kern, dim3((unsigned)grid, (unsigned)ks), dim3(C::NTHR), lds_bytes + 7680, s, at);
      DRM_HIP_CHECK(hipStreamSynchronize(s));
      std::vector<unsigned> h(2048);
      DRM_HIP_CHECK(hipMemcpy(h.data(), dbuf, 8192, hipMemcpyDeviceToHost));
      if (FILE* f = fopen(stamp_file, "a")) {
        fprintf(f, "launch taps %d tile %dx%d C %d->%d map %dx%d N %d grid %lld\n", TAPS, TH, TW, a.C0 + a.C1, a.Cout, a.H, a.W, a.N, grid);
        for (int w = 0; w < 8; ++w) {
          fprintf(f, "wave %d:", w);
          for (int k = 0; k < 120 && h[(w * 120 + k) * 2]; ++k) fprintf(f, " %u:%u", h[(w * 120 + k) * 2], h[(w * 120 + k) * 2 + 1]);
          fprintf(f, "\n");
        }
        fclose(f);
      }
    } else if (static const char* fl = getenv("DRM_S2_FLAGS"); fl) {
      ConvArgs at = a;
      at.stamp_block = atoi(fl) & ~0xFFFF;
      hipLaunchKernelGGL(kern, dim3((unsigned)grid, (unsigned)ks), dim3(C::NTHR), lds_bytes, s, at);
    } else
#endif
    hipLaunchKernelGGL(kern, dim3((unsigned)grid, (unsigned)ks), dim3(C::NTHR), lds_bytes, s, a);
  }
  DRM_HIP_CHECK(hipGetLastError());
  return DRM_OK;
}

static int no_form(const ConvPlan& p) {
  set_error("conv plan: form " + std::to_string((int)p.tile) + " on " + std::to_string(p.th) + "x" + std::to_string(p.tw) + (p.ragged ? " ragged" : "") +
            " pixel tiles, terms " + std::to_string(p.terms) + ", is not instantiated");
  return DRM_ERR_STATE;
}

template <int TAPS, int TH, int TW, int TERMS>
static int launch_s2_tile(const ConvArgs& a, const ConvPlan& p, hipStream_t s) {
  constexpr int TPS = (TAPS == 9) ? 3 : (TAPS == 4 ? 2 : 1), RG = (TAPS == 1) ? 4 : 2;
  constexpr bool T16 = TH == 16 && TW == 16, ROWS256 = TAPS == 1 || TH >= 8;
  if constexpr (TAPS == 4) {
    if (p.ragged || p.pool || p.ksplit > 1) return no_form(p);
    if (p.tile == TILE_256x192) {
      if constexpr (T16 && (TERMS == 3 || TERMS == 2)) return launch_s2<TAPS, TH, TW, 4, 2, 2, 3, RG, TPS, TERMS>(a, s);
    } else if (p.tile == TILE_256x128) {
      if constexpr (ROWS256) return launch_s2<TAPS, TH, TW, 4, 2, 2, 2, RG, TPS, TERMS>(a, s);
    } else if (p.tile == TILE_128x128) {
      if constexpr (!ROWS256) return launch_s2<TAPS, TH, TW, 2, 2, 2, 2, RG, TPS, TERMS>(a, s);
    } else if (p.tile == TILE_256x64) {
      if constexpr (ROWS256) return launch_s2<TAPS, TH, TW, 4, 2, 2, 1, RG, TPS, TERMS>(a, s);
    } else if constexpr (!T16) {
      if (p.tile == TILE_128x64) return launch_s2<TAPS, TH, TW, 2, 2, 2, 1, RG, TPS, TERMS>(a, s);
      if (p.tile == TILE_128x32) return launch_s2<TAPS, TH, TW, 4, 1, 1, 1, RG, TPS, TERMS>(a, s);
    }
    return no_form(p);
  } else if (p.ragged) {
    if constexpr (TERMS != 0 && !T16 && !(TH == 4 && TW == 8)) {
      if (p.tile == TILE_128x64) return launch_s2<TAPS, TH, TW, 2, 2, 2, 1, RG, TPS, TERMS, true>(a, s);
      if (p.tile == TILE_128x32) return launch_s2<TAPS, TH, TW, 4, 1, 1, 1, RG, TPS, TERMS, true>(a, s);
    }
  } else if (p.tile == TILE_256x256) {
    if constexpr (TAPS == 1 && T16 && TERMS == 3) return launch_s2<TAPS, TH, TW, 4, 2, 2, 4, 2, 1, TERMS>(a, s);
  } else if (p.tile == TILE_256x192) {
    if constexpr (T16 && (TERMS == 3 || (TAPS == 9 && TERMS == 2))) return launch_s2<TAPS, TH, TW, 4, 2, 2, 3, 3, 1, TERMS>(a, s);
  } else if (p.tile == TILE_256x128 && p.pool) {
    if constexpr (TAPS == 9 && T16) return launch_s2<TAPS, TH, TW, 4, 2, 2, 2, RG, TPS, TERMS, false, false, true>(a, s);
  } else if (p.tile == TILE_256x128) {
    if constexpr (ROWS256) return launch_s2<TAPS, TH, TW, 4, 2, 2, 2, RG, TPS, TERMS>(a, s);
  } else if (p.tile == TILE_128x128) {
    if constexpr (!ROWS256) return launch_s2<TAPS, TH, TW, 2, 2, 2, 2, 3, 1, TERMS>(a, s);
  } else if (p.tile == TILE_256x64) {
    if constexpr (ROWS256) return launch_s2<TAPS, TH, TW, 4, 2, 2, 1, RG, TPS, TERMS>(a, s);
  } else if constexpr (!T16) {
    if (p.tile == TILE_128x64) return launch_s2<TAPS, TH, TW, 2, 2, 2, 1, RG, TPS, TERMS>(a, s);
    if (p.tile == TILE_128x32 && p.finish == SPLIT_IN_LAUNCH) return launch_s2<TAPS, TH, TW, 4, 1, 1, 1, RG, TPS, TERMS, false, true>(a, s);
    if (p.tile == TILE_128x32) return launch_s2<TAPS, TH, TW, 4, 1, 1, 1, RG, TPS, TERMS>(a, s);
  }
  return no_form(p);
}

template <int TAPS, int TERMS>
int dispatch_s2(const ConvArgs& a, const ConvPlan& p, hipStream_t s) {
  if (p.th == 16 && p.tw == 16) return launch_s2_tile<TAPS, 16, 16, TERMS>(a, p, s);
  if (p.th == 8 && p.tw == 16) return launch_s2_tile<TAPS, 8, 16, TERMS>(a, p, s);
  if (p.th == 8 && p.tw == 8) return launch_s2_tile<TAPS, 8, 8, TERMS>(a, p, s);
  if (p.th == 4 && p.tw == 8) return launch_s2_tile<TAPS, 4, 8, TERMS>(a, p, s);
  if (p.th == 4 && p.tw == 4) return launch_s2_tile<TAPS, 4, 4, TERMS>(a, p, s);
  return no_form(p);
}

#ifdef DRM_S2_UNIT
template int dispatch_s2<DRM_S2_UNIT / 10, DRM_S2_UNIT % 10>(const ConvArgs&, const ConvPlan&, hipStream_t);
#else
extern template int dispatch_s2<9, 0>(const ConvArgs&, const ConvPlan&, hipStream_t);
extern template int dispatch_s2<1, 0>(const ConvArgs&, const ConvPlan&, hipStream_t);
extern template int dispatch_s2<9, 1>(const ConvArgs&, const ConvPlan&, hipStream_t);
extern template int dispatch_s2<1, 1>(const ConvArgs&, const ConvPlan&, hipStream_t);
extern template int dispatch_s2<9, 4>(const ConvArgs&, const ConvPlan&, hipStream_t);
extern template int dispatch_s2<1, 4>(const ConvArgs&, const ConvPlan&, hipStream_t);
extern template int dispatch_s2<9, 2>(const ConvArgs&, const ConvPlan&, hipStream_t);
extern template int dispatch_s2<9, 3>(const ConvArgs&, const ConvPlan&, hipStream_t);
extern template int dispatch_s2<4, 0>(const ConvArgs&, const ConvPlan&, hipStream_t);
extern template int dispatch_s2<4, 1>(const ConvArgs&, const ConvPlan&, hipStream_t);
extern template int dispatch_s2<4, 2>(const ConvArgs&, const ConvPlan&, hipStream_t);
extern template int dispatch_s2<4, 3>(const ConvArgs&, const ConvPlan&, hipStream_t);
extern template int dispatch_s2<4, 4>(const ConvArgs&, const ConvPlan&, hipStream_t);
extern template int dispatch_s2<1, 3>(const ConvArgs&, const ConvPlan&, hipStream_t);
int launch_igemm(const ConvArgs& a, const ConvPlan& p, hipStream_t s);

constexpr long long S2_MIN_WIDE_TILES = 176;
constexpr int GN_FOLD_MAX_N = 4;

bool conv_split_weights(int precision, int cin) { return precision != PREC_FP32 && cin % 32 == 0; }

ConvPlan plan_conv(const ConvArgs& a, int precision, bool want_pool, bool gn_foldable) {
  ConvPlan p;
  const int Ctot = a.C0 + a.C1, hw = a.H * a.W;
  const bool split = precision != PREC_FP32, chunks = Ctot % 32 == 0 && a.C0 % 32 == 0;
  const long long rows = (long long)a.N * hw;
  auto wgs = [&](int bm, int bn) { return ((rows + bm - 1) / bm) * (a.Cout / bn); };
  if (a.w_img_stride_f4 != 0) {
    if (!split || a.H % 16 != 0 || a.W % 16 != 0 || a.Cout % 128 != 0 || Ctot % 128 != 0) return p;
  }
  if (!chunks || (!split && (a.H % 4 != 0 || a.W % 4 != 0))) {
    static const int fam[4][2] = {{8, 16}, {8, 8}, {4, 8}, {4, 4}};
    const int f = conv_tile_family(a.H, a.W, fam, 4);
    p.kernel = CONV_IGEMM;
    p.th = fam[f][0]; p.tw = fam[f][1];
    p.tile = a.Cout % 128 == 0 ? TILE_128x128 : (a.Cout % 64 == 0 ? TILE_128x64 : TILE_128x32);
    p.kc = chunks ? 32 : 8;
    return p;
  }
  p.kernel = CONV_PIPELINE;
  p.terms = (precision == PREC_F16MX && a.mx_site) ? 2 : precision_terms(precision);
  p.gn_fold = gn_foldable && a.N <= GN_FOLD_MAX_N;
  static const int whole[5][4] = {{16, 16, 8, 16}, {8, 16, 8, 16}, {8, 8, 8, 8}, {4, 8, 4, 8}, {4, 4, 4, 4}};
  const int* fw = nullptr;
  for (const auto& f : whole)
    if (!fw && a.H % f[0] == 0 && a.W % f[1] == 0) fw = f;
  if (!fw) {
    static const int fam[3][2] = {{8, 16}, {8, 8}, {4, 4}};
    const int f = conv_tile_family(a.H, a.W, fam, 3);
    p.th = fam[f][0]; p.tw = fam[f][1];
    p.ragged = true;
    p.tile = a.Cout % 64 == 0 ? TILE_128x64 : TILE_128x32;
    return p;
  }
  int wide = 1;
  if (a.taps == 9 && !a.out_nchw && a.w_img_stride_f4 == 0 && a.Cout % 128 == 0 && hw <= 128 &&
      ((a.H % 8 == 0 && a.W % 16 == 0) || (a.H % 4 == 0 && a.W % 8 == 0)) && rows >= 1024) {
    const int bm = (a.taps == 1 || (a.H % 8 == 0 && a.W % 16 == 0)) ? 256 : 128;
    const long long tiles = ((rows + bm - 1) / bm) * (a.Cout / 128);
    if (tiles < S2_MIN_WIDE_TILES) wide = (int)std::max<long long>(std::min<long long>(std::min<long long>(8, Ctot / 32 / 2), std::max<long long>(1, 256 / tiles)), 1);
  }
  const bool t16 = fw[0] == 16 && fw[1] == 16, rows256 = a.taps == 1 || fw[0] >= 8;
  auto tile = [&](ConvTile t, bool r256) {
    p.tile = t;
    p.th = r256 ? fw[0] : fw[2];
    p.tw = r256 ? fw[1] : fw[3];
  };
  if (a.taps == 1 && t16 && p.terms == 3 && a.Cout % 256 == 0 && wgs(256, 256) >= 512) {
    tile(TILE_256x256, true);
  } else if (t16 && (p.terms == 3 || (a.taps != 1 && p.terms == 2)) && a.Cout % 192 == 0 && wgs(256, 192) >= 512) {
    tile(TILE_256x192, true);
  } else if (a.Cout % 128 == 0 && (wgs(256, 128) >= S2_MIN_WIDE_TILES || wide > 1)) {
    tile(rows256 ? TILE_256x128 : TILE_128x128, rows256);
    p.pool = want_pool && split && a.taps == 9 && t16 && !a.out_nchw;
  } else if (a.Cout % 64 == 0 && wgs(256, 64) >= 256) {
    tile(rows256 ? TILE_256x64 : TILE_128x64, rows256);
  } else if (a.Cout % 64 == 0 && wgs(128, 64) >= 256) {
    tile(TILE_128x64, false);
  } else {
    tile(TILE_128x32, false);
  }
  p.ksplit = wide;
  if (wide == 1 && p.tile == TILE_128x32 && !a.out_nchw && a.w_img_stride_f4 == 0)
    p.ksplit = (int)std::max<long long>(std::min<long long>(std::min<long long>(8, Ctot / 32 / 4), 640 / std::max<long long>(wgs(128, 32), 1)), 1);
  if (p.ksplit > 1) {
    p.finish = (hw >= 128 && wide == 1) ? SPLIT_IN_LAUNCH : SPLIT_REDUCE;
    if (p.finish == SPLIT_IN_LAUNCH) p.tickets = ((size_t)a.N * hw / 128 + (size_t)hw / 16 + 2) * (size_t)(a.Cout / 32);
  }
  return p;
}

__global__ __launch_bounds__(256) void splitk_reduce_small_kernel(const float4* __restrict__ partial, size_t slab_f4, int ks, const float* __restrict__ bias,
                                                                  const float* __restrict__ emb, int emb_stride, const float* res ,
                                                                  float4* out, double2* __restrict__ stat, int HW, int Cout) {
  __shared__ float red[256][8];
  const int n = blockIdx.y, q4 = Cout >> 2;
  const int ql = threadIdx.x & 15, pl = threadIdx.x >> 4;
  const int q = blockIdx.x * 16 + ql;
  float4 b = make_float4(0.f, 0.f, 0.f, 0.f);
  if (q < q4) {
    if (bias) b = reinterpret_cast<const float4*>(bias)[q];
    if (emb) {
      const float4 e = *reinterpret_cast<const float4*>(emb + (size_t)n * emb_stride + 4 * q);
      b.x += e.x; b.y += e.y; b.z += e.z; b.w += e.w;
    }
  }
  float s[4] = {0.f, 0.f, 0.f, 0.f}, ss[4] = {0.f, 0.f, 0.f, 0.f};
#pragma unroll 4
  for (int p = pl; p < HW && q < q4; p += 16) {
    const size_t idx = ((size_t)n * HW + p) * q4 + q;
    float4 acc = partial[idx];
    for (int k = 1; k < ks; ++k) {
      const float4 t = partial[idx + (size_t)k * slab_f4];
      acc.x += t.x; acc.y += t.y; acc.z += t.z; acc.w += t.w;
    }
    float4 v = make_float4(acc.x + b.x, acc.y + b.y, acc.z + b.z, acc.w + b.w);
    if (res) {
      const float4 r = reinterpret_cast<const float4*>(res)[idx];
      v.x += r.x; v.y += r.y; v.z += r.z; v.w += r.w;
    }
    out[idx] = v;
    s[0] += v.x; s[1] += v.y; s[2] += v.z; s[3] += v.w;
    ss[0] += v.x * v.x; ss[1] += v.y * v.y; ss[2] += v.z * v.z; ss[3] += v.w * v.w;
  }
  if (stat) {
#pragma unroll
    for (int k = 0; k < 4; ++k) {
      red[threadIdx.x][k] = s[k];
      red[threadIdx.x][4 + k] = ss[k];
    }
    __syncthreads();
    if (pl == 0 && q < q4) {
#pragma unroll
      for (int k = 0; k < 4; ++k) {
        double a = 0.0, c2 = 0.0;
        for (int j = 0; j < 16; ++j) {
          a += (double)red[j * 16 + ql][k];
          c2 += (double)red[j * 16 + ql][4 + k];
        }
        double2* d = stat + (size_t)n * Cout + 4 * q + k;
        *d = make_double2(d->x + a, d->y + c2);
      }
    }
  }
}

static int launch_splitk_reduce(const ConvArgs& a, const float* partial, hipStream_t s) {
  const int HW = a.H * a.W;
  DRM_REQUIRE(a.ksplit > 1 && a.split_stride % 4 == 0 && a.Cout % 4 == 0 && HW <= 256, "split-K reduction arguments (maps of more than 256 pixels finish inside the conv launch)");
  hipLaunchKernelGGL(splitk_reduce_small_kernel, dim3((a.Cout / 4 + 15) / 16, a.N), dim3(256), 0, s, reinterpret_cast<const float4*>(partial),
                     a.split_stride / 4, a.ksplit, a.bias, a.emb, a.emb_stride, a.res, reinterpret_cast<float4*>(a.out), a.stat_out, HW, a.Cout);
  DRM_HIP_CHECK(hipGetLastError());
  return DRM_OK;
}

int launch_conv(const ConvArgs& a, const ConvPlan& p, hipStream_t s) {
  DRM_REQUIRE(a.taps == 9 || a.taps == 1 || a.taps == 4, "conv taps must be 9, 1 or 4 (the parity form of a 3x3 over a nearest-x2 input)");
  DRM_REQUIRE(a.taps != 4 || (p.kernel == CONV_PIPELINE && p.finish == SPLIT_NONE), "the parity (4-tap) form runs on the pipeline kernel, un-split");
  DRM_REQUIRE(a.N > 0 && a.H > 0 && a.W > 0, "conv shape");
  DRM_REQUIRE(!a.up0 || (a.H % 2 == 0 && a.W % 2 == 0), "upsampled source needs even output size");
  DRM_REQUIRE(a.ksplit == p.ksplit && (p.ksplit == 1 || a.split_ws), "split-K launch without its slab workspace");
  if (p.kernel == CONV_IGEMM) return launch_igemm(a, p, s);
  DRM_REQUIRE(p.kernel == CONV_PIPELINE, "no conv kernel takes this shape (per-image weights: split modes, maps of whole 16x16 tiles, 128-channel multiples)");
  DRM_REQUIRE(a.Cout % 32 == 0 && (a.C0 + a.C1) % 32 == 0 && a.C0 % 32 == 0, "split conv needs channels % 32 == 0");
  DRM_REQUIRE(a.terms == p.terms, "ConvArgs::terms differs from the plan");
  DRM_REQUIRE(p.terms != 2 || (a.taps != 1 && a.gn_scale && !a.in_inv && a.w_img_stride_f4 == 0), "f16mx: 3x3 convs on a GroupNorm-ed input only");
  auto run = [&](const ConvArgs& x) -> int {
    if (a.taps == 4) switch (p.terms) {
      case 0: return dispatch_s2<4, 0>(x, p, s);
      case 1: return dispatch_s2<4, 1>(x, p, s);
      case 2: return dispatch_s2<4, 2>(x, p, s);
      case 3: return dispatch_s2<4, 3>(x, p, s);
      case 4: return dispatch_s2<4, 4>(x, p, s);
      default: return no_form(p);
    }
    switch (p.terms) {
      case 0: return a.taps == 9 ? dispatch_s2<9, 0>(x, p, s) : dispatch_s2<1, 0>(x, p, s);
      case 1: return a.taps == 9 ? dispatch_s2<9, 1>(x, p, s) : dispatch_s2<1, 1>(x, p, s);
      case 2: return dispatch_s2<9, 2>(x, p, s);
      case 3: return a.taps == 9 ? dispatch_s2<9, 3>(x, p, s) : dispatch_s2<1, 3>(x, p, s);
      case 4: return a.taps == 9 ? dispatch_s2<9, 4>(x, p, s) : dispatch_s2<1, 4>(x, p, s);
    }
    return no_form(p);
  };
  if (p.finish != SPLIT_REDUCE) return run(a);
  ConvArgs part = a;
  part.out = a.split_ws;
  part.split_ws = nullptr;
  part.bias = nullptr; part.emb = nullptr; part.res = nullptr; part.stat_out = nullptr;
  DRM_TRY(run(part));
  return launch_splitk_reduce(a, a.split_ws, s);
}
#endif

}
```

### drmnet_amd/csrc/engine.hip

```cpp
#include "engine.h"

#include <algorithm>
#include <atomic>
#include <deque>
#include <mutex>

namespace drm {

static thread_local std::string g_err;
void set_error(const std::string& msg) { g_err = msg; }
const char* last_error() { return g_err.c_str(); }

const DeviceInfo* device_info() {
  constexpr int MAX_DEV = 64;
  static DeviceInfo info[MAX_DEV];
  static std::atomic<int> state[MAX_DEV];
  int dev = 0;
  if (hipGetDevice(&dev) != hipSuccess || dev < 0 || dev >= MAX_DEV) {
    set_error("device_info: no current HIP device");
    return nullptr;
  }
  int st = state[dev].load(std::memory_order_acquire);
  if (st == 0) {
    static std::mutex mu;
// ... 258 lines not shown
      DRM_REQUIRE(i + 3 < params.size() && ptrs[i + 1] && ptrs[i + 2] && ptrs[i + 3], "attention block parameters of " + p.name);
      float* fb = staging + (size_t)p.cout * p.cin;
      DRM_TRY(launch_fold_attn_params(ptrs[i], ptrs[i + 1], ptrs[i + 2], ptrs[i + 3], staging, fb, p.cin, s));
      DRM_HIP_CHECK(hipMemcpyAsync(wbuf + params[i + 1].dst, fb, (size_t)p.cout * sizeof(float), hipMemcpyDeviceToDevice, s));
      w = staging;
    }
    if (p.kind == PK_COPY) {
      DRM_HIP_CHECK(hipMemcpyAsync(wbuf + p.dst, w, p.count * sizeof(float), hipMemcpyDeviceToDevice, s));
    } else {
      DRM_TRY(conv(w, p.dst, p.scale_dst, p.cout, p.cin, p.taps, p.coutp, p.cinp, p.mx_site));
      if (p.up_c0) {
        const int c0 = p.up_c0, c1 = p.cin - p.up_c0;
        float* wa = staging;
        float* wb = staging + (size_t)16 * p.cout * c0;
        DRM_TRY(launch_fold_upconv_weight(w, wa, wb, p.cout, c0, c1, s));
        DRM_TRY(conv(wa, p.upa_dst, p.upa_scale, 4 * p.cout, c0, 4, 4 * p.cout, c0, p.mx_site));
        DRM_TRY(conv(wb, p.upb_dst, p.upb_scale, p.cout, c1, 9, p.cout, c1, p.mx_site));
      }
    }
  }
  return DRM_OK;
}

int UNet::load(const float* const* ptrs, int count, hipStream_t s, int set) {
  DRM_REQUIRE(set >= 0 && set < NSETS, "weight set index");
  if (!wsets[set]) DRM_HIP_CHECK(hipMalloc(reinterpret_cast<void**>(&wsets[set]), wbuf_floats * sizeof(float)));
  float* wbuf = wsets[set];
  loaded[set] = false;
  Scratch staging(s);
  if (staging_floats()) DRM_TRY(staging.reserve(staging_floats() * sizeof(float)));
  DRM_TRY(pack(ptrs, count, wbuf, precision, static_cast<float*>(staging.p), s));
  if (stem_direct_w >= 0) DRM_TRY(launch_pack_stem_weight(ptrs[stem_param], wbuf + stem_direct_w, desc.model_channels, desc.in_channels, precision == PREC_FP32, s));
  loaded[set] = true;
  loaded_precision[set] = precision;
  return DRM_OK;
}


Act new_act(Ctx& c, int C, int H, int W) {
  Act a;
  a.C = C; a.H = H; a.W = W;
  a.p = c.ar->alloc<float>((size_t)c.N * H * W * C);
  a.mom = reinterpret_cast<double2*>(c.ar->alloc_stats((size_t)c.N * C * sizeof(double2), &a.mom_zeroed));
  return a;
}

int ensure_moments(Ctx& c, Act& a) {
  if (a.mom_valid) return DRM_OK;
  const int hs = a.H >> a.up, ws = a.W >> a.up;
  const size_t m = c.ar->mark();
  const int splits = chan_moments_splits(hs * ws, a.C);
  double* partial = c.ar->alloc<double>((size_t)c.N * splits * a.C * 2);
  if (!c.dry()) DRM_TRY(launch_chan_moments(a.p, c.N, hs * ws, a.C, partial, a.mom, c.s));
  c.ar->release(m);
  a.mom_valid = true;
  return DRM_OK;
}

int expect_raw_sums(Ctx& c, Act& a) {
  if (!c.dry() && !a.mom_zeroed) DRM_HIP_CHECK(hipMemsetAsync(a.mom, 0, (size_t)c.N * a.C * sizeof(double2), c.s));
  a.mom_valid = true;
  a.mom_sums = true;
  return DRM_OK;
}

static void splitk_workspace(Ctx& c, ConvArgs& a, const ConvPlan& p) {
  a.ksplit = p.ksplit;
  if (p.ksplit <= 1) return;
  a.split_stride = (size_t)a.N * a.H * a.W * a.Cout;
  if (p.finish == SPLIT_IN_LAUNCH) {
    bool zeroed = false;
    a.tile_ticket = reinterpret_cast<unsigned*>(c.ar->alloc_stats(p.tickets * sizeof(unsigned), &zeroed));
    if (!zeroed && !c.dry()) (void)hipMemsetAsync(a.tile_ticket, 0, p.tickets * sizeof(unsigned), c.s);
  }
  a.split_ws = c.ar->alloc<float>(a.split_stride * a.ksplit);
}

int run_conv(Ctx& c, ConvArgs& a, const ConvPlan& p, const float* Wb, size_t scale_off, Act* stats_for) {
  if (p.kernel == CONV_PIPELINE) {
    a.w_inv_scale = c.split() ? Wb + scale_off + 1 : nullptr;
    a.terms = p.terms;
    if (stats_for && !a.out_nchw) {
      DRM_TRY(expect_raw_sums(c, *stats_for));
      a.stat_out = stats_for->mom;
    }
  }
  return launch_conv(a, p, c.s);
}

int raw_input_guard(Ctx& c, ConvArgs& a, const ConvPlan& p, Act* x0, int lo0, int hi0, Act* x1, const unsigned* absmax_bits, int Ctab, int absmax_parts) {
  if (!p.split()) return DRM_OK;
  float* sc = c.ar->alloc<float>((size_t)c.N * Ctab);
  float* sh = c.ar->alloc<float>((size_t)c.N * Ctab);
  float* inv = c.ar->alloc<float>((size_t)c.N);
  if (x0) DRM_TRY(ensure_moments(c, *x0));
  if (x1) DRM_TRY(ensure_moments(c, *x1));
  if (c.dry()) return DRM_OK;
  DRM_TRY(launch_act_pow2_scale(x0 ? x0->mom : nullptr, x0 ? x0->C : 0, lo0, hi0, x0 ? x0->mom_cnt() : 0.0, x1 ? x1->mom : nullptr, x1 ? x1->C : 0,
                                x1 ? x1->mom_cnt() : 0.0, absmax_bits, Ctab, c.N, sc, sh, inv, c.s, absmax_parts));
  a.gn_scale = sc;
  a.gn_shift = sh;
  a.in_inv = inv;
  return DRM_OK;
}

int gn_params(Ctx& c, Act& x0, Act* x1, const float* gamma, const float* beta, float* scale, float* shift, ConvArgs* guard_for, ConvArgs* fold_into) {
  DRM_TRY(ensure_moments(c, x0));
  if (x1) DRM_TRY(ensure_moments(c, *x1));
  const int Ctot = x0.C + (x1 ? x1->C : 0);
  float *gs = nullptr, *gh = nullptr, *gi = nullptr;
  if (guard_for) {
    gs = c.ar->alloc<float>((size_t)c.N * Ctot);
    gh = c.ar->alloc<float>((size_t)c.N * Ctot);
    gi = c.ar->alloc<float>((size_t)c.N);
    guard_for->gn_scale = gs;
    guard_for->gn_shift = gh;
    guard_for->in_inv = gi;
  }
  if (c.dry()) return DRM_OK;
  if (fold_into) {
    GnFold& f = fold_into->gnf;
    f.mom0 = x0.mom; f.C0 = x0.C; f.inv0 = x0.mom_inv(); f.cnt0 = x0.mom_cnt();
    f.mom1 = x1 ? x1->mom : nullptr; f.C1 = x1 ? x1->C : 0; f.inv1 = x1 ? x1->mom_inv() : 1.0; f.cnt1 = x1 ? x1->mom_cnt() : 0.0;
    f.gamma = gamma; f.beta = beta; f.scale = scale; f.shift = shift;
    f.guard_scale = gs; f.guard_shift = gh; f.guard_inv = gi;
    return DRM_OK;
  }
  return launch_gn_finalize(x0.mom, x0.C, x0.mom_inv(), x1 ? x1->mom : nullptr, x1 ? x1->C : 0, x1 ? x1->mom_inv() : 1.0, gamma, beta, c.N, scale,
                            shift, c.s, x0.mom_cnt(), x1 ? x1->mom_cnt() : 0.0, gs, gh, gi);
}

static int arena_ok(const Ctx& c) {
  if (!c.ar->failed) return DRM_OK;
  set_error("workspace too small: need more than " + std::to_string(c.ar->cap) + " bytes (query drm_unet_workspace_bytes for this shape and precision)");
  return DRM_ERR_WORKSPACE;
}

static std::atomic<int> g_upconv_split{1};
void set_upconv_split(int mode) { g_upconv_split.store(mode); }

struct UpconvSplit {
  bool on = false;
  ConvArgs a4, b9;
  ConvPlan p4, p9;
};
static UpconvSplit plan_upconv_split(const Ctx& c, const ResLayer& r, const ConvArgs& a, const ConvPlan& pa, const Act& x0, const Act* x1) {
  UpconvSplit u;
  const int mode = g_upconv_split.load(std::memory_order_relaxed);
  if (mode == 0 || !r.up_c0 || !x0.up || !x1 || x0.C != r.up_c0 || !upconv_split_packable(x0.C, x1->C, r.cout)) return u;
  auto plain = [](const ConvPlan& p) { return p.kernel == CONV_PIPELINE && !p.ragged && p.ksplit == 1 && !p.gn_fold && !p.pool; };
  if (!plain(pa)) return u;
  u.a4.C0 = x0.C; u.a4.N = a.N; u.a4.H = a.H >> 1; u.a4.W = a.W >> 1; u.a4.taps = 4; u.a4.Cout = 4 * r.cout; u.a4.mx_site = 1;
  u.b9.C0 = x1->C; u.b9.N = a.N; u.b9.H = a.H; u.b9.W = a.W; u.b9.taps = 9; u.b9.Cout = r.cout; u.b9.mx_site = 1;
  u.p4 = plan_conv(u.a4, c.precision);
  u.p9 = plan_conv(u.b9, c.precision);
  if (!plain(u.p4) || !plain(u.p9)) return u;
  static const int tile_bn[] = {256, 192, 128, 128, 64, 64, 32};
  if (r.cout % tile_bn[u.p4.tile] != 0) return u;
  if (mode == 1 && (u.p4.tile > TILE_256x128 || u.p9.tile > TILE_256x128)) return u;
  u.on = true;
  return u;
}

int run_resblock(Ctx& c, const float* Wb, const ResLayer& r, Act& x0, Act* x1, const float* emb_all, int emb_stride, Act& out, Act* pool, bool* pooled) {
  DRM_TRY(arena_ok(c));
  const int H = x0.H, W = x0.W;
  const int C0 = x0.C, C1 = x1 ? x1->C : 0;
  DRM_REQUIRE(C0 + C1 == r.cin, "resblock input channels");
  DRM_REQUIRE(!x1 || (x1->H == H && x1->W == W && !x1->up), "resblock skip tensor shape");
  DRM_REQUIRE(r.has_skip || (!x1 && !x0.up), "identity skip on a concatenated / upsampled input is not supported");
  const size_t mark = c.ar->mark();
  float* sc1 = c.ar->alloc<float>((size_t)c.N * r.cin);
  float* sh1 = c.ar->alloc<float>((size_t)c.N * r.cin);
  Act h1 = new_act(c, r.cout, H, W);
  float* sc2 = c.ar->alloc<float>((size_t)c.N * r.cout);
  float* sh2 = c.ar->alloc<float>((size_t)c.N * r.cout);
  ConvArgs k;
  ConvArgs a;
  a.src0 = x0.p; a.src1 = x1 ? x1->p : nullptr; a.C0 = C0; a.C1 = C1; a.up0 = x0.up;
  a.N = c.N; a.H = H; a.W = W; a.taps = 9; a.Cout = r.cout; a.mx_site = 1;
  const ConvPlan pa = plan_conv(a, c.precision, false, true);
  ConvPlan pk;
  if (r.has_skip) {
    k.C0 = C0; k.C1 = C1; k.N = c.N; k.H = H; k.W = W; k.taps = 1; k.Cout = r.cout;
    pk = plan_conv(k, c.precision);
  }
  DRM_TRY(gn_params(c, x0, x1, Wb + r.n1_w, Wb + r.n1_b, sc1, sh1, pk.split() ? &k : nullptr, pa.gn_fold ? &a : nullptr));
  splitk_workspace(c, a, pa);
  UpconvSplit up = plan_upconv_split(c, r, a, pa, x0, x1);
  if (up.on) {
    if (!c.dry()) {
      ConvArgs& a4 = up.a4;
      a4.src0 = x0.p; a4.gn_scale = sc1; a4.gn_shift = sh1; a4.gn_ld = r.cin; a4.silu = 1;
      a4.w = Wb + r.c1a_w; a4.out = h1.p;
      DRM_TRY(run_conv(c, a4, up.p4, Wb, r.c1a_s, nullptr));
      ConvArgs& b9 = up.b9;
      b9.src0 = x1->p; b9.gn_scale = sc1 + x0.C; b9.gn_shift = sh1 + x0.C; b9.gn_ld = r.cin; b9.silu = 1;
      b9.w = Wb + r.c1b_w; b9.bias = Wb + r.c1_b;
      b9.emb = emb_all ? emb_all + r.emb_off : nullptr; b9.emb_stride = emb_stride;
      b9.res = h1.p; b9.out = h1.p;
      DRM_TRY(run_conv(c, b9, up.p9, Wb, r.c1b_s, &h1));
    }
  } else if (!c.dry()) {
    a.gn_scale = sc1; a.gn_shift = sh1; a.silu = 1;
    a.w = Wb + r.c1_w; a.bias = Wb + r.c1_b;
    a.emb = emb_all ? emb_all + r.emb_off : nullptr; a.emb_stride = emb_stride;
    a.out = h1.p;
    DRM_TRY(run_conv(c, a, pa, Wb, r.c1_s, &h1));
  }
  ConvArgs b;
  b.src0 = h1.p; b.C0 = r.cout; b.N = c.N; b.H = H; b.W = W; b.taps = 9; b.Cout = r.cout; b.mx_site = 1;
  const ConvPlan pb = plan_conv(b, c.precision, pool != nullptr, true);
  DRM_TRY(gn_params(c, h1, nullptr, Wb + r.n2_w, Wb + r.n2_b, sc2, sh2, nullptr, pb.gn_fold ? &b : nullptr));
  splitk_workspace(c, b, pb);
  if (pooled) *pooled = pb.pool;
  if (pb.pool) DRM_TRY(expect_raw_sums(c, *pool));
  if (r.has_skip) splitk_workspace(c, k, pk);
  if (!c.dry()) {
    const float* res = x0.p;
    if (r.has_skip) {
      k.src0 = x0.p; k.src1 = x1 ? x1->p : nullptr; k.up0 = x0.up;
      k.w = Wb + r.sk_w; k.bias = Wb + r.sk_b;
      k.out = out.p;
      DRM_TRY(run_conv(c, k, pk, Wb, r.sk_s, nullptr));
      res = out.p;
    }
    b.gn_scale = sc2; b.gn_shift = sh2; b.silu = 1;
    b.w = Wb + r.c2_w; b.bias = Wb + r.c2_b;
    b.res = res; b.out = out.p;
    if (pb.pool) {
      b.pool_out = pool->p;
      b.pool_stat = pool->mom;
    }
    DRM_TRY(run_conv(c, b, pb, Wb, r.c2_s, &out));
  }
  c.ar->release(mark);
  return DRM_OK;
}

int run_attention(Ctx& c, const float* Wb, const AttnLayer& l, Act& x, Act& out) {
  DRM_REQUIRE(!x.up && x.C == l.ch, "attention input");
  DRM_TRY(arena_ok(c));
  const int H = x.H, W = x.W, T = H * W, C = l.ch;
  const size_t mark = c.ar->mark();
  float* sc = c.ar->alloc<float>((size_t)c.N * C);
  float* sh = c.ar->alloc<float>((size_t)c.N * C);
  ConvArgs a;
  a.C0 = C; a.N = c.N; a.H = H; a.W = W; a.taps = 1; a.Cout = 3 * C;
  const ConvPlan pa = plan_conv(a, c.precision, false, true);
  DRM_TRY(gn_params(c, x, nullptr, Wb + l.n_w, Wb + l.n_b, sc, sh, nullptr, pa.gn_fold ? &a : nullptr));
  Act qkv_act = new_act(c, 3 * C, H, W);
  float* qkv = qkv_act.p;
  const AttnPlan ap = plan_attention(c.N, H, W, C, c.precision);
  float* scores = ap.scores_floats ? c.ar->alloc<float>(ap.scores_floats) : nullptr;
  (void)c.ar->alloc<float>((size_t)c.N * T * C);
  const size_t proj_tab = (size_t)c.N * C;
  float* aws = ap.ws_floats ? c.ar->alloc<float>(ap.ws_floats + proj_tab) : nullptr;
  splitk_workspace(c, a, pa);
  {
    ConvArgs p;
    p.C0 = C; p.N = c.N; p.H = H; p.W = W; p.taps = 1; p.Cout = C;
    const ConvPlan pp = plan_conv(p, c.precision);
    if (pp.ksplit > 1) {
      bool zeroed = false;
      if (pp.finish == SPLIT_IN_LAUNCH) (void)c.ar->alloc_stats(pp.tickets * sizeof(unsigned), &zeroed);
      (void)c.ar->alloc<float>((size_t)c.N * T * C * pp.ksplit);
    }
  }
  if (ap.out_stats) DRM_TRY(expect_raw_sums(c, out));
  if (!c.dry()) {
    a.src0 = x.p;
    a.gn_scale = sc; a.gn_shift = sh; a.silu = 0;
    a.w = Wb + l.qkv_w; a.bias = Wb + l.qkv_b; a.out = qkv;
    DRM_TRY(run_conv(c, a, pa, Wb, l.qkv_s, &qkv_act));
    DRM_TRY(launch_attention_core(ap, qkv, qkv_act.mom, x.p, scores, out.p, out.mom, aws, c.s));
  }
  c.ar->release(mark);
  if (!ap.out_stats) {
    out.mom_valid = false;
    DRM_TRY(ensure_moments(c, out));
  }
  return DRM_OK;
}


int UNet::dry_forward(int N, int H, int W, Arena& probe) {
  probe.dry = true;
  const int Cx = desc.kind == 0 ? desc.out_channels : desc.in_channels / 2;
  return forward(nullptr, Cx, nullptr, desc.in_channels - Cx, nullptr, nullptr, nullptr, nullptr, nullptr, N, H, W, probe, nullptr);
}

int UNet::forward(const float* x, int Cx, const float* cond, int Cc, const int32_t* rows, const float* t_emb, const int64_t* t,
                  const float* tf, float* out, int N, int H, int W, Arena& ar, hipStream_t s) {
  DRM_REQUIRE(ar.dry || loaded[active], "drm_unet_forward before drm_unet_load_params (weight set " + std::to_string(active) + ")");
  DRM_REQUIRE(N > 0, "batch size");
  DRM_REQUIRE(Cx + Cc == desc.in_channels, "x/cond channels must sum to in_channels");
  const int down = 1 << (desc.n_levels - 1);
  DRM_REQUIRE(H > 0 && W > 0 && H % down == 0 && W % down == 0,
              "H and W must be multiples of " + std::to_string(down) + " (2^(levels-1): each of the " + std::to_string(desc.n_levels - 1) + " Downsample layers halves the map)");
  const int n_t = (t_emb != nullptr) + (t != nullptr) + (tf != nullptr);
  if (!ar.dry) {
    if (desc.kind == 0) DRM_REQUIRE(n_t == 1, "timesteps and t_emb cannot be specified at the same time");
    else DRM_REQUIRE(n_t == 1 && t_emb == nullptr, "EncoderUNetModel takes timesteps");
  }
  DRM_REQUIRE(ar.dry || loaded_precision[active] == precision, "precision changed after drm_unet_load_params: reload the parameters");
  Ctx c{&ar, s, N, precision};
  const float* Wb = wsets[active];
  const int mc = desc.model_channels;

  ar.st_active = true;
  ar.st_off = 0;
  if (!ar.dry) {
    const auto key = std::make_tuple(N, H, W, precision);
    auto it = stats_pool_cache.find(key);
    if (it == stats_pool_cache.end()) {
      Arena probe;
      DRM_TRY(dry_forward(N, H, W, probe));
      it = stats_pool_cache.emplace(key, probe.st_off).first;
    }
    ar.st_cap = it->second;
    ar.st_base = reinterpret_cast<char*>(ar.alloc_bytes(ar.st_cap));
    if (ar.st_base) DRM_HIP_CHECK(hipMemsetAsync(ar.st_base, 0, ar.st_cap, s));
  }
  struct PoolScope {
    Arena& a;
    ~PoolScope() {
      if (a.dry) a.peak += (a.st_off + 255) & ~size_t(255);
      a.st_active = false;
      a.st_base = nullptr;
    }
  } pool_scope{ar};

  const bool stem_direct = stem_direct_w >= 0;
  Act xin;
  const int amax_parts = pack_input_absmax_parts(H, W);
  unsigned* amax = nullptr;
  if (!stem_direct) {
    xin = new_act(c, in_cp, H, W);
    amax = c.ar->alloc<unsigned>((size_t)N * amax_parts);
  }
  float* temb = c.ar->alloc<float>((size_t)N * mc);
  float* e1 = c.ar->alloc<float>((size_t)N * emb_dim);
  float* emb = c.ar->alloc<float>((size_t)N * emb_dim);
  float* emb_all = c.ar->alloc<float>((size_t)N * emb_total);
  DRM_TRY(arena_ok(c));
  if (!c.dry()) {
    if (!stem_direct) DRM_TRY(launch_pack_input(x, cond, rows, xin.p, N, H, W, Cx, Cc, in_cp, s, amax));
    const float* te = t_emb;
    if (!te) {
      DRM_TRY(launch_timestep_embedding(t, tf, temb, N, mc, s));
      te = temb;
    }
    DRM_TRY(launch_linear(te, Wb + te0_w, Wb + te0_b, e1, N, mc, emb_dim, 0, 1, s));
    DRM_TRY(launch_linear(e1, Wb + te2_w, Wb + te2_b, emb, N, emb_dim, emb_dim, 0, 0, s));
    DRM_TRY(launch_linear(emb, Wb + embcat_w, Wb + embcat_b, emb_all, N, emb_dim, emb_total, 1, 0, s));
  }

  std::deque<Act> acts;
  auto make = [&](int C_, int H_, int W_) -> Act* {
    acts.push_back(new_act(c, C_, H_, W_));
    return &acts.back();
  };
  std::vector<Act*> hs;
  Act* h = make(mc, H, W);
  if (stem_direct) {
    DRM_TRY(expect_raw_sums(c, *h));
    if (!c.dry()) DRM_TRY(launch_stem_conv(x, Cx, cond, Cc, rows, Wb + stem_direct_w, Wb + stem_b, h->p, h->mom, N, H, W, mc, precision == PREC_FP32, s));
  } else {
    ConvArgs a;
    a.C0 = in_cp; a.N = N; a.H = H; a.W = W; a.taps = 9; a.Cout = mc;
    const ConvPlan pa = plan_conv(a, precision);
    DRM_TRY(raw_input_guard(c, a, pa, nullptr, 0, 0, nullptr, amax, in_cp, amax_parts));
    if (!c.dry()) {
      a.src0 = xin.p; a.w = Wb + stem_w; a.bias = Wb + stem_b; a.out = h->p; a.cin_real = desc.in_channels;
      DRM_TRY(run_conv(c, a, pa, Wb, stem_s, h));
    }
  }
  hs.push_back(h);

  Act* pool_buf = nullptr;
  bool pool_done = false;
  auto run_layers = [&](std::vector<Layer>& ls, Act* skip, bool down_next = false) -> int {
    for (size_t li = 0; li < ls.size(); ++li) {
      Layer& l = ls[li];
      if (l.kind == Layer::RES) {
        Act* o = make(l.res.cout, h->H, h->W);
        Act* po = nullptr;
        bool pooled = false;
        if (down_next && li + 1 == ls.size() && h->H % 2 == 0 && h->W % 2 == 0) po = make(l.res.cout, h->H / 2, h->W / 2);
        DRM_TRY(run_resblock(c, Wb, l.res, *h, (li == 0) ? skip : nullptr, emb_all, emb_total, *o, po, &pooled));
        pool_buf = po;
        pool_done = pooled;
        h = o;
      } else if (l.kind == Layer::ATTN) {
        Act* o = make(l.attn.ch, h->H, h->W);
        DRM_TRY(run_attention(c, Wb, l.attn, *h, *o));
        h = o;
      } else if (l.kind == Layer::DOWN) {
        DRM_REQUIRE(!h->up, "downsample of an upsampled tensor");
        Act* o = pool_buf ? pool_buf : make(h->C, h->H / 2, h->W / 2);
        const bool done = pool_buf && pool_done;
        pool_buf = nullptr;
        pool_done = false;
// ... 58 lines not shown
```

### drmnet_amd/csrc/gn.hip

```cpp
#include "common.h"
#include "gn_fold.h"
#include "profiler.h"

namespace drm {

int chan_moments_splits(int HW, int C) {
  int s = HW / 64;
  if (s < 1) s = 1;
  if (s > 64) s = 64;
  return s;
}

__global__ __launch_bounds__(256) void chan_moments_partial_kernel(const float* __restrict__ x, int HW, int C, int splits,
                                                                    double* __restrict__ partial) {
  __shared__ double red[2][4][64][4];
  const int s = blockIdx.x, n = blockIdx.y;
  const int qx = threadIdx.x, py = threadIdx.y;
  const int q4 = C >> 2;
  const int p0 = (int)(((long long)HW * s) / splits), p1 = (int)(((long long)HW * (s + 1)) / splits);
  const float4* xp = reinterpret_cast<const float4*>(x) + (size_t)n * HW * q4;
  for (int qb = 0; qb < q4; qb += 64) {
    const int q = qb + qx;
    double sum[4] = {0.0, 0.0, 0.0, 0.0}, sq[4] = {0.0, 0.0, 0.0, 0.0};
    if (q < q4) {
      for (int p = p0 + py; p < p1; p += 4) {
        const float4 v = xp[(size_t)p * q4 + q];
        sum[0] += v.x; sum[1] += v.y; sum[2] += v.z; sum[3] += v.w;
        sq[0] += (double)v.x * v.x; sq[1] += (double)v.y * v.y; sq[2] += (double)v.z * v.z; sq[3] += (double)v.w * v.w;
      }
    }
#pragma unroll
    for (int k = 0; k < 4; ++k) {
      red[0][py][qx][k] = sum[k];
      red[1][py][qx][k] = sq[k];
    }
    __syncthreads();
    if (py == 0 && q < q4) {
      double* o = partial + (((size_t)n * splits + s) * C + 4 * q) * 2;
#pragma unroll
      for (int k = 0; k < 4; ++k) {
        o[2 * k] = red[0][0][qx][k] + red[0][1][qx][k] + red[0][2][qx][k] + red[0][3][qx][k];
        o[2 * k + 1] = red[1][0][qx][k] + red[1][1][qx][k] + red[1][2][qx][k] + red[1][3][qx][k];
      }
    }
    __syncthreads();
  }
}

__global__ void chan_moments_reduce_kernel(const double* __restrict__ partial, int N, int C, int splits, double inv_hw, double2* __restrict__ mom) {
  const int i = blockIdx.x * blockDim.x + threadIdx.x;
  if (i >= N * C) return;
  const int n = i / C, c = i % C;
  double s = 0.0, q = 0.0;
  for (int k = 0; k < splits; ++k) {
    const double* p = partial + (((size_t)n * splits + k) * C + c) * 2;
    s += p[0];
    q += p[1];
  }
  mom[i] = make_double2(s * inv_hw, q * inv_hw);
}

int launch_chan_moments(const float* x, int N, int HW, int C, double* partial, double2* mom, hipStream_t s) {
  DRM_REQUIRE(C % 4 == 0, "chan_moments: C % 4");
  const int splits = chan_moments_splits(HW, C);
  prof_tag(N, HW, 1, C, C);
  ProfScope ps(PROF_GNSTATS, 3.0 * N * (double)HW * C, 4.0 * N * (double)HW * C, s);
  hipLaunchKernelGGL(chan_moments_partial_kernel, dim3(splits, N), dim3(64, 4), 0, s, x, HW, C, splits, partial);
  DRM_HIP_CHECK(hipGetLastError());
  const int total = N * C;
  hipLaunchKernelGGL(chan_moments_reduce_kernel, dim3((total + 255) / 256), dim3(256), 0, s, partial, N, C, splits, 1.0 / (double)HW, mom);
  DRM_HIP_CHECK(hipGetLastError());
  return DRM_OK;
}

__global__ __launch_bounds__(256) void gn_finalize_kernel(const double2* __restrict__ mom0, int C0, double inv0,
                                                           const double2* __restrict__ mom1, int C1, double inv1,
                                                           const float* __restrict__ gamma, const float* __restrict__ beta,
                                                           float* __restrict__ scale, float* __restrict__ shift, double cnt0, double cnt1,
                                                           float* __restrict__ guard_scale, float* __restrict__ guard_shift,
                                                           float* __restrict__ guard_inv) {
  __shared__ __attribute__((aligned(16))) float scratch[72];
  GnFold f;
  f.mom0 = mom0; f.mom1 = mom1; f.C0 = C0; f.C1 = C1; f.inv0 = inv0; f.inv1 = inv1; f.cnt0 = cnt0; f.cnt1 = cnt1;
  f.gamma = gamma; f.beta = beta; f.scale = scale; f.shift = shift;
  f.guard_scale = guard_scale; f.guard_shift = guard_shift; f.guard_inv = guard_inv;
  gn_finalize_image(f, blockIdx.x, threadIdx.x, 256, scratch);
}

__global__ __launch_bounds__(256) void act_pow2_scale_kernel(const double2* __restrict__ mom0, int C0, int lo0, int hi0, double cnt0,
                                                             const double2* __restrict__ mom1, int C1, double cnt1,
                                                             const unsigned* __restrict__ absmax_bits, int absmax_parts, int Ctab,
                                                             float* __restrict__ scale, float* __restrict__ shift, float* __restrict__ inv) {
  __shared__ double red[4];
  __shared__ float s_scale;
  const int n = blockIdx.x, t = threadIdx.x;
  double m = 0.0;
  if (mom0)
    for (int c = lo0 + t; c < hi0; c += 256) m = fmax(m, mom0[(size_t)n * C0 + c].y * (cnt0 > 0 ? cnt0 : 1.0));
  if (mom1)
    for (int c = t; c < C1; c += 256) m = fmax(m, mom1[(size_t)n * C1 + c].y * (cnt1 > 0 ? cnt1 : 1.0));
  if (absmax_bits)
    for (int i = t; i < absmax_parts; i += 256) {
      const double v = (double)__uint_as_float(absmax_bits[(size_t)n * absmax_parts + i]);
      m = fmax(m, v * v);
    }
#pragma unroll
  for (int o = 32; o > 0; o >>= 1) m = fmax(m, __shfl_xor(m, o));
  if ((t & 63) == 0) red[t >> 6] = m;
  __syncthreads();
  if (t == 0) {
    double bound = sqrt(fmax(fmax(red[0], red[1]), fmax(red[2], red[3])));
    int k = 0;
    if (bound > 0.0 && bound < INFINITY) {
      int e;
      frexp(bound, &e);
      k = 15 - e;
      k = k > 90 ? 90 : (k < -90 ? -90 : k);
    }
    s_scale = ldexpf(1.0f, k);
    inv[n] = ldexpf(1.0f, -k);
  }
  __syncthreads();
  const float sc = s_scale;
  for (int c = t; c < Ctab; c += 256) {
    scale[(size_t)n * Ctab + c] = sc;
    shift[(size_t)n * Ctab + c] = 0.f;
  }
}

int launch_act_pow2_scale(const double2* mom0, int C0, int lo0, int hi0, double cnt0, const double2* mom1, int C1, double cnt1,
                          const unsigned* absmax_bits, int Ctab, int N, float* scale, float* shift, float* inv, hipStream_t s, int absmax_parts) {
  DRM_REQUIRE((mom0 || absmax_bits) && scale && shift && inv && N > 0 && Ctab > 0, "act_pow2_scale: arguments");
  hipLaunchKernelGGL(act_pow2_scale_kernel, dim3(N), dim3(256), 0, s, mom0, C0, lo0, hi0, cnt0, mom1, C1, cnt1, absmax_bits, absmax_parts, Ctab, scale,
                     shift, inv);
  DRM_HIP_CHECK(hipGetLastError());
  return DRM_OK;
}

int launch_gn_finalize(const double2* mom0, int C0, double inv0, const double2* mom1, int C1, double inv1, const float* gamma,
                       const float* beta, int N, float* scale, float* shift, hipStream_t s, double cnt0, double cnt1, float* guard_scale,
                       float* guard_shift, float* guard_inv) {
  DRM_REQUIRE((C0 + C1) % 32 == 0, "GroupNorm32 needs channels % 32 == 0");
  hipLaunchKernelGGL(gn_finalize_kernel, dim3(N), dim3(256), 0, s, mom0, C0, inv0, mom1, C1, inv1, gamma, beta, scale, shift, cnt0, cnt1, guard_scale,
                     guard_shift, guard_inv);
  DRM_HIP_CHECK(hipGetLastError());
  return DRM_OK;
}

}
```

### drmnet_amd/csrc/gn_fold.h

```cpp
#pragma once
#include <hip/hip_runtime.h>

namespace drm {

struct GnFold {
  const double2* mom0 = nullptr;
  const double2* mom1 = nullptr;
  int C0 = 0, C1 = 0;
  double inv0 = 1.0, inv1 = 1.0;
  double cnt0 = 0.0, cnt1 = 0.0;
  const float* gamma = nullptr;
  const float* beta = nullptr;
  float* scale = nullptr;
  float* shift = nullptr;
  float* guard_scale = nullptr;
  float* guard_shift = nullptr;
  float* guard_inv = nullptr;
};

__device__ __forceinline__ void gn_lds_barrier() {
  asm volatile("s_waitcnt lgkmcnt(0)" ::: "memory");
  __builtin_amdgcn_s_barrier();
  asm volatile("" ::: "memory");
}

constexpr int GN_FOLD_PRELOAD = 6;
__device__ __forceinline__ void gn_finalize_image(const GnFold& f, int n, int t, int nthreads, float* lds, float* lds_tab = nullptr) {
  float* g_mean = lds;
  float* g_rstd = lds + 32;
  const int C0 = f.C0, C1 = f.C1, C = C0 + C1, cpg = C / 32;
  float gm[GN_FOLD_PRELOAD], bt[GN_FOLD_PRELOAD];
  const bool pre = C <= GN_FOLD_PRELOAD * nthreads;
  if (pre) {
#pragma unroll
    for (int k = 0; k < GN_FOLD_PRELOAD; ++k) {
      const int c = min(t + k * nthreads, C - 1);
      gm[k] = f.gamma[c];
      bt[k] = f.beta[c];
    }
  }
  if (f.guard_scale) {
    double* red = reinterpret_cast<double*>(lds + 64);
    double m = 0.0;
    if (t < 256) {
      for (int c = t; c < C; c += 256)
        m = fmax(m, c < C0 ? f.mom0[(size_t)n * C0 + c].y * (f.cnt0 > 0 ? f.cnt0 : 1.0) : f.mom1[(size_t)n * C1 + (c - C0)].y * (f.cnt1 > 0 ? f.cnt1 : 1.0));
#pragma unroll
      for (int o = 32; o > 0; o >>= 1) m = fmax(m, __shfl_xor(m, o));
      if ((t & 63) == 0) red[t >> 6] = m;
    }
    gn_lds_barrier();
    const double bound = sqrt(fmax(fmax(red[0], red[1]), fmax(red[2], red[3])));
    int k = 0;
    if (bound > 0.0 && bound < INFINITY) {
      int e;
      frexp(bound, &e);
      k = 15 - e;
      k = k > 90 ? 90 : (k < -90 ? -90 : k);
    }
    const float gs = ldexpf(1.0f, k);
    if (t == 0) f.guard_inv[n] = ldexpf(1.0f, -k);
    for (int c = t; c < C; c += nthreads) {
      f.guard_scale[(size_t)n * C + c] = gs;
      f.guard_shift[(size_t)n * C + c] = 0.f;
    }
  }
  if (t < 256) {
    const int g = t >> 3, j = t & 7;
    double m = 0.0, q = 0.0;
    for (int k = j; k < cpg; k += 8) {
      const int c = g * cpg + k;
      if (c < C0) {
        const double2 v = f.mom0[(size_t)n * C0 + c];
        m += v.x * f.inv0;
        q += v.y * f.inv0;
      } else {
        const double2 v = f.mom1[(size_t)n * C1 + (c - C0)];
        m += v.x * f.inv1;
        q += v.y * f.inv1;
      }
    }
#pragma unroll
    for (int o = 4; o > 0; o >>= 1) {
      m += __shfl_xor(m, o);
      q += __shfl_xor(q, o);
    }
    if (j == 0) {
      m /= cpg;
      q /= cpg;
      double var = q - m * m;
      if (var < 0.0) var = 0.0;
      g_mean[g] = (float)m;
      g_rstd[g] = (float)(1.0 / sqrt(var + 1e-5));
    }
  }
  gn_lds_barrier();
  if (pre) {
#pragma unroll
    for (int k = 0; k < GN_FOLD_PRELOAD; ++k) {
      const int c = t + k * nthreads;
      if (c < C) {
        const int g = c / cpg;
        const float sc = g_rstd[g] * gm[k], sh = bt[k] - g_mean[g] * sc;
        f.scale[(size_t)n * C + c] = sc;
        f.shift[(size_t)n * C + c] = sh;
        if (lds_tab) {
          lds_tab[c] = sc;
          lds_tab[C + c] = sh;
        }
      }
    }
  } else {
    for (int c = t; c < C; c += nthreads) {
      const int g = c / cpg;
      const float sc = g_rstd[g] * f.gamma[c], sh = f.beta[c] - g_mean[g] * sc;
      f.scale[(size_t)n * C + c] = sc;
      f.shift[(size_t)n * C + c] = sh;
      if (lds_tab) {
        lds_tab[c] = sc;
        lds_tab[C + c] = sh;
      }
    }
  }
  gn_lds_barrier();
}

}
```

### drmnet_amd/ops.py

```python
from __future__ import annotations

from typing import Optional, Sequence

import torch

from . import _lib


def set_precision(precision: str) -> None:
    modes = {"fp32": 0, "f16x3": 1, "f16": 2, "f16mx": 3, "bf16": 4}
    if precision not in modes:
        raise ValueError(f"precision must be one of {list(modes)}")
    _lib.check(_lib.lib().drm_set_op_precision(modes[precision]))


def set_graph_replay(on: bool) -> None:
    _lib.check(_lib.lib().drm_set_graph_replay(int(bool(on))))


def set_upconv_split(mode: int) -> None:
    _lib.check(_lib.lib().drm_set_upconv_split(int(mode)))


UPCONV_TAP_GROUPS = {0: {0: (0,), 1: (1, 2)}, 1: {0: (0, 1), 1: (2,)}}


def fold_upconv_weight(w: torch.Tensor, c0: int):
    cout = w.shape[0]
    w0 = w[:, :c0].double()
    wa = torch.zeros((4, cout, c0, 2, 2), dtype=torch.float64, device=w.device)
    for a in (0, 1):
        for b in (0, 1):
            for dy in (0, 1):
                for dx in (0, 1):
                    for ky in UPCONV_TAP_GROUPS[a][dy]:
                        for kx in UPCONV_TAP_GROUPS[b][dx]:
                            wa[2 * a + b, :, :, dy, dx] += w0[:, :, ky, kx]
    return wa.reshape(4 * cout, c0, 2, 2).to(w.dtype), w[:, c0:].contiguous()


def graph_launches() -> int:
    return int(_lib.lib().drm_graph_launches())


def _dev(t: torch.Tensor):
    return torch.cuda.device(t.device)


@torch.no_grad()
def linear(x, weight, bias=None, silu_in=False, silu_out=False):
    x = _lib.require_gpu_tensor(x, "x")
    weight = _lib.require_gpu_tensor(weight, "weight")
    bias = None if bias is None else _lib.require_gpu_tensor(bias, "bias")
    n, i = x.shape
    o = weight.shape[0]
    out = torch.empty((n, o), dtype=torch.float32, device=x.device)
    with _dev(x):
        _lib.check(_lib.lib().drm_linear_forward(x.data_ptr(), weight.data_ptr(), _lib.ptr(bias), out.data_ptr(), n, i, o, int(silu_in), int(silu_out), _lib.stream_ptr(x.device)))
    return out


@torch.no_grad()
def timestep_embedding(timesteps, dim):
    t = _lib.require_gpu_tensor(timesteps.long(), "timesteps", torch.int64)
    out = torch.empty((t.shape[0], dim), dtype=torch.float32, device=t.device)
    with _dev(t):
        _lib.check(_lib.lib().drm_timestep_embedding(t.data_ptr(), out.data_ptr(), t.shape[0], dim, _lib.stream_ptr(t.device)))
    return out


@torch.no_grad()
def norm_act_conv(x, weight, bias=None, gamma=None, beta=None, silu=False, emb=None, residual=None):
    x = _lib.require_gpu_tensor(x, "x")
    weight = _lib.require_gpu_tensor(weight, "weight")
    n, cin, h, w = x.shape
    cout, k = weight.shape[0], weight.shape[-1]
    ts = [None if t is None else _lib.require_gpu_tensor(t, "arg") for t in (bias, gamma, beta, emb, residual)]
    bias, gamma, beta, emb, residual = ts
    out = torch.empty((n, cout, h, w), dtype=torch.float32, device=x.device)
    with _dev(x):
        _lib.check(_lib.lib().drm_op_norm_act_conv(x.data_ptr(), _lib.ptr(gamma), _lib.ptr(beta), int(silu), weight.data_ptr(), _lib.ptr(bias), k,
                                                    _lib.ptr(emb), _lib.ptr(residual), out.data_ptr(), n, cin, cout, h, w, _lib.stream_ptr(x.device)))
    return out


@torch.no_grad()
def resblock(params: Sequence[torch.Tensor], x0, emb, x1=None, up0=False):
    x0 = _lib.require_gpu_tensor(x0, "x0")
    emb = _lib.require_gpu_tensor(emb, "emb")
    params = [_lib.require_gpu_tensor(p, "param") for p in params]
    n, c0 = x0.shape[0], x0.shape[1]
    h, w = x0.shape[2] * (2 if up0 else 1), x0.shape[3] * (2 if up0 else 1)
    c1 = 0
    if x1 is not None:
        x1 = _lib.require_gpu_tensor(x1, "x1")
        c1 = x1.shape[1]
    cout = params[2].shape[0]
    out = torch.empty((n, cout, h, w), dtype=torch.float32, device=x0.device)
    arr = _lib.ptr_array(params)
    with _dev(x0):
        _lib.check(_lib.lib().drm_op_resblock(x0.data_ptr(), c0, int(up0), _lib.ptr(x1), c1, emb.data_ptr(), emb.shape[1], arr, len(params),
                                               out.data_ptr(), n, cout, h, w, _lib.stream_ptr(x0.device)))
    return out


@torch.no_grad()
def attention_block(params: Sequence[torch.Tensor], x):
    x = _lib.require_gpu_tensor(x, "x")
    params = [_lib.require_gpu_tensor(p, "param") for p in params]
    n, c, h, w = x.shape
    out = torch.empty_like(x)
    arr = _lib.ptr_array(params)
    with _dev(x):
        _lib.check(_lib.lib().drm_op_attention_block(x.data_ptr(), arr, out.data_ptr(), n, c, h, w, _lib.stream_ptr(x.device)))
    return out


@torch.no_grad()
def randn(shape, seed: int, offset: int = 0, device="cuda"):
    out = torch.empty(shape, dtype=torch.float32, device=device)
    with torch.cuda.device(out.device):
        _lib.check(_lib.lib().drm_randn(out.data_ptr(), out.numel(), seed, offset, _lib.stream_ptr(out.device)))
    return out



LOSS_TYPES = {"l1": 0, "l2": 1}


@torch.no_grad()
def validation_losses(model_out, Lr_k, Lr_km1, K, z_out, z_k, z_K, reversed_k, z0, gamma: float, loss_type: str = "l2", l_refmap_weight: float = 1.0,
                      l_refcode_weight: float = 1.0) -> torch.Tensor:
    if loss_type not in LOSS_TYPES:
        raise NotImplementedError(f"unknown loss type '{loss_type}'")
    model_out = _lib.require_gpu_tensor(model_out, "model_out")
    dev = model_out.device
    B = model_out.shape[0]
    maps = [model_out] + [_lib.require_gpu_tensor(t, n) for t, n in ((Lr_k, "Lr_k"), (Lr_km1, "Lr_km1"))]
    if any(t.shape != model_out.shape for t in maps):
        raise RuntimeError(f"model_out, Lr_k and Lr_km1 must share one shape, got {[tuple(t.shape) for t in maps]}")
    codes = [_lib.require_gpu_tensor(t, n) for t, n in ((z_out, "z_out"), (z_k, "z_k"), (z_K, "z_K"))]
    P = codes[0].shape[-1]
    if any(tuple(t.shape) != (B, P) for t in codes):
        raise RuntimeError(f"z_out, z_k and z_K must be [B={B}, P], got {[tuple(t.shape) for t in codes]}")
    ints = [_lib.require_gpu_tensor(t.to(torch.int32), n, torch.int32) for t, n in ((K, "K"), (reversed_k, "reversed_k"))]
    if any(tuple(t.shape) != (B,) for t in ints):
        raise RuntimeError(f"K and reversed_k must be [B={B}]")
    z0 = _lib.require_gpu_tensor(z0.to(dev, torch.float32), "z0")
    if z0.numel() != P:
        raise RuntimeError(f"z0 must have {P} entries")
    ws = torch.empty(_lib.LOSS_WORKSPACE_BYTES // 8, dtype=torch.float64, device=dev)
    out = torch.empty(3, dtype=torch.float32, device=dev)
    with torch.cuda.device(dev):
        _lib.check(_lib.lib().drm_validation_losses(maps[0].data_ptr(), maps[1].data_ptr(), maps[2].data_ptr(), ints[0].data_ptr(), codes[0].data_ptr(),
                                                    codes[1].data_ptr(), codes[2].data_ptr(), ints[1].data_ptr(), z0.data_ptr(), float(gamma),
                                                    LOSS_TYPES[loss_type], float(l_refmap_weight), float(l_refcode_weight), B,
                                                    model_out.numel() // B, P, ws.data_ptr(), ws.numel() * 8, out.data_ptr(), _lib.stream_ptr(dev)))
    return out



PADDING_MODES = {"zeros": 0, "noise": 1}


@torch.no_grad()
def obs_forward_process(x, mask, t, sqrt_alphas_cumprod, sqrt_one_minus_alphas_cumprod, noisy_observe: float = 0.0, padding_mode: str = "noise", *,
                        e_observe=None, e_padding=None, e_q=None, seed: int = 0, want_cond: bool = True, want_q: bool = True):
    if padding_mode not in PADDING_MODES:
        raise NotImplementedError(f"padding_mode {padding_mode!r}")
    if not (want_cond or want_q):
        raise ValueError("obs_forward_process: nothing asked for")
    x = _lib.require_gpu_tensor(x, "x")
    if x.ndim != 4:
        raise RuntimeError("obs_forward_process expects x [B, C, H, W]")
# ... 179 lines not shown
```

### include/drmnet_hip.h

```cpp
#ifndef DRMNET_HIP_H
#define DRMNET_HIP_H

#include <stddef.h>
#include <stdint.h>

#ifdef __cplusplus
extern "C" {
#endif

#define DRM_ABI_VERSION 3
#define DRM_MAX_LEVELS 8

int drm_abi_version(void);
const char* drm_last_error(void);

typedef struct drm_unet_desc {
  int32_t kind;
  int32_t in_channels;
  int32_t model_channels;
  int32_t out_channels;
  int32_t num_res_blocks;
  int32_t n_levels;
  int32_t channel_mult[DRM_MAX_LEVELS];
  int32_t n_attn;
  int32_t attention_resolutions[DRM_MAX_LEVELS];
} drm_unet_desc;

typedef struct drm_unet drm_unet;

int drm_unet_create(const drm_unet_desc* desc, drm_unet** out);
void drm_unet_destroy(drm_unet* net);

int drm_unet_param_count(const drm_unet* net);
int drm_unet_param_info(const drm_unet* net, int index, char* name, int name_cap, int64_t shape[4], int* ndim);

int drm_unet_load_params(drm_unet* net, const float* const* ptrs, int count, void* stream);

#define DRM_WEIGHT_SETS 2
int drm_unet_load_params_set(drm_unet* net, int set, const float* const* ptrs, int count, void* stream);
int drm_unet_use_set(drm_unet* net, int set);

#define DRM_PREC_FP32 0
#define DRM_PREC_F16X3 1
#define DRM_PREC_F16 2
#define DRM_PREC_F16MX 3
#define DRM_PREC_BF16 4
int drm_unet_set_precision(drm_unet* net, int precision);
int drm_set_op_precision(int precision);

size_t drm_unet_workspace_bytes(const drm_unet* net, int N, int H, int W);

int drm_unet_forward(drm_unet* net, const float* x, int Cx, const float* cond, int Cc, const int32_t* rows, const float* t_emb,
                     const int64_t* timesteps, const float* timesteps_f, float* out, int N, int H, int W, void* workspace,
                     size_t workspace_bytes, void* stream);

int drm_linear_forward(const float* in, const float* w, const float* b, float* out, int N, int I, int O, int silu_in, int silu_out, void* stream);
int drm_timestep_embedding(const int64_t* timesteps, float* out, int N, int dim, void* stream);
int drm_op_norm_act_conv(const float* x, const float* gamma, const float* beta, int silu, const float* w, const float* b, int ksize,
                         const float* emb, const float* residual, float* out, int N, int Cin, int Cout, int H, int W, void* stream);
int drm_op_resblock(const float* x0, int C0, int up0, const float* x1, int C1, const float* emb, int emb_dim, const float* const* params,
                    int n_params, float* out, int N, int Cout, int H, int W, void* stream);
int drm_op_attention_block(const float* x, const float* const* params, float* out, int N, int C, int H, int W, void* stream);

typedef struct drm_drmnet_cfg {
  int32_t z_dim;
  int32_t max_timesteps;
  double gamma;
  float epsilon, delta;
  float z0[8];
} drm_drmnet_cfg;

typedef struct drm_drmnet drm_drmnet;

int drm_drmnet_create(drm_unet* illnet, drm_unet* refnet, const float* const* zemb, const drm_drmnet_cfg* cfg, drm_drmnet** out);
void drm_drmnet_destroy(drm_drmnet* s);
size_t drm_drmnet_workspace_bytes(const drm_drmnet* s, int N, int H, int W);
int drm_drmnet_set_batch_parts(drm_drmnet* s, int parts);
int drm_drmnet_set_batch_part_min(drm_drmnet* s, int rows);

int drm_drmnet_step(drm_drmnet* s, float* Lr_k, const float* LrK, const int32_t* rows, int n_active, int step, const float* noise,
                    uint64_t seed, float* zk_out, float* zK_out, int32_t* converged_out, int B, int H, int W, void* workspace,
                    size_t workspace_bytes, void* stream);

int drm_drmnet_sample(drm_drmnet* s, const float* LrK, const float* cond, const float* noise0, const float* step_noise, uint64_t seed, int early_exit,
                      float* Lr0, float* zK, int32_t* K, int32_t* steps_done, int B, int H, int W, void* workspace, size_t workspace_bytes,
                      void* stream);

int drm_ddim_sample(drm_unet* net, float* x, const float* cond, const int64_t* timesteps, const float* coef, int S, int num_steps,
                    const float* noise, uint64_t seed, int N, int H, int W, void* workspace, size_t workspace_bytes, void* stream);

int drm_ddim_sample_logged(drm_unet* net, float* x, const float* cond, const int64_t* timesteps, const float* coef, int S, int num_steps,
                           const float* noise, uint64_t seed, int log_every_t, float* log_x, float* log_pred_x0, int log_slots, int32_t* n_logged, int N,
                           int H, int W, void* workspace, size_t workspace_bytes, void* stream);

int drm_ddpm_sample(drm_unet* net, float* x, float* pred_x0, const float* cond, const float* coef, int T_start, int clip_denoised,
                    const float* noise, uint64_t seed, int N, int H, int W, void* workspace, size_t workspace_bytes, void* stream);

typedef struct drm_mask_blend {
  const float* mask;
  int mask_channels;
  const float* x0;
  const float* qcoef;
  const float* qnoise;
  int when;
} drm_mask_blend;

typedef struct drm_sampler_options {
  const drm_mask_blend* blend;
  const float* uncond;
  float guidance_scale;
  float noise_dropout;
  const float* dropout_keep;
} drm_sampler_options;

int drm_ddim_sample_ex(drm_unet* net, float* x, const float* cond, const int64_t* timesteps, const float* coef, int S, int num_steps,
                       const float* noise, uint64_t seed, const drm_sampler_options* opt, int log_every_t, float* log_x, float* log_pred_x0, int log_slots,
                       int32_t* n_logged, int N, int H, int W, void* workspace, size_t workspace_bytes, void* stream);
int drm_ddpm_sample_ex(drm_unet* net, float* x, float* pred_x0, const float* cond, const float* coef, int T_start, int clip_denoised,
                       const float* noise, uint64_t seed, const drm_sampler_options* opt, int N, int H, int W, void* workspace, size_t workspace_bytes,
                       void* stream);

size_t drm_sampler_workspace_bytes(const drm_unet* net, int N, int H, int W);

int drm_set_graph_replay(int on);

int drm_set_upconv_split(int mode);
int64_t drm_graph_launches(void);

#define DRM_PROFILE_KINDS 5
void drm_profile_enable(int on);
void drm_profile_reset(void);
int drm_profile_collect(double* ms, double* flops, double* bytes, int64_t* launches);
size_t drm_profile_variants(char* buf, size_t cap);

int drm_randn(float* out, size_t n, uint64_t seed, uint64_t offset, void* stream);

size_t drm_refmap_workspace_bytes(int64_t n, int res, float angle_threshold);
int drm_refmap_mask_make(const float* colors, const float* normals, int64_t n, int channels, int res, float angle_threshold, int min_points,
                         float* refmap, uint8_t* refmask, void* workspace, size_t workspace_bytes, void* stream);

int drm_erode_mask(const uint8_t* mask, int H, int W, int kernel_size, uint8_t* out, void* stream);

#define DRM_MAP_LOG_P1 0
#define DRM_MAP_LOG10 1
#define DRM_MAP_LOWERBOUND 2
#define DRM_MAP_UNIT_TO_SIGNED 3
#define DRM_MAP_NORM_LOG 4
#define DRM_MAP_EXP_M1 5
#define DRM_MAP_EXP10 6
#define DRM_MAP_SIGNED_TO_UNIT 7
#define DRM_MAP_DENORM_LOG 8
#define DRM_MAP_IMG_MUL 9
#define DRM_MAP_IMG_DIV 10
#define DRM_MAP_CLIP0 11
int drm_map_chain(const float* x, float* out, int64_t per_image, int B, const int32_t* ops, const float* args, int n_ops, const float* lo,
                  const float* hi, const float* scale, void* stream);
int drm_masked_log_range(const float* x, const float* mask, int B, int C, int HW, float* lo, float* hi, void* stream);
int drm_luminance_scale(const float* x, int B, int HW, float scaler, float* scale, void* stream);
int drm_mirmap2envmap(const float* mirmap, const float* basis, float* out, int B, int C, int H, int W, int OH, int OW, int log_scale_interpolation,
                      int channels_last, void* stream);
int drm_hdr2ldr(const float* x, const uint8_t* mask, int HW, float alpha, float gamma, float* out, void* stream);
#define DRM_RESIZE_NEAREST 0
#define DRM_RESIZE_BILINEAR_AA 1
#define DRM_RESIZE_BICUBIC_AA 2
int drm_resize(const float* x, float* out, int planes, int IH, int IW, int OH, int OW, int mode, void* stream);

int drm_render_refmap(const float* z, const float* envmap, float* out, int B, int R, int EH, int EW, int quad, int subpixel, int flip, void* stream);
int drm_render_refmap_views(const float* z, int L, const float* envmap, const float* view, float* out, int B, int R, int EH, int EW, int quad,
                            int subpixel, int flip, void* stream);
size_t drm_render_light_workspace_bytes(int B, int EH, int EW, int light_samples);
int drm_render_refmap_lit(const float* z, int L, const float* envmap, const float* view, float* out, int B, int R, int EH, int EW, int quad,
                          int subpixel, int flip, int light_samples, void* workspace, size_t workspace_bytes, void* stream);
size_t drm_render_mesh_workspace_bytes(int64_t F, int B, int H, int W, int subpixel);
int drm_render_mesh(const float* vertex_positions, const float* vertex_normals, const int32_t* faces, int64_t V, int64_t F, const float* z,
                    const float* envmap, const float* view, float* image, float* normal, float* depth, float* alpha, int B, int H, int W, int EH, int EW,
                    int quad, int subpixel, void* workspace, size_t workspace_bytes, void* stream);
size_t drm_mesh_bvh_bytes(int64_t F);
int drm_mesh_bvh_build(const float* vertex_positions, const int32_t* faces, int64_t V, int64_t F, void* bvh, size_t bytes);
int drm_mesh_occluded(const float* vertex_positions, const int32_t* faces, int64_t V, int64_t F, const void* bvh, const float* origins, const float* dirs,
                      const int32_t* exclude, int32_t* out, int64_t N, void* stream);
int drm_render_mesh_shadowed(const float* vertex_positions, const float* vertex_normals, const int32_t* faces, int64_t V, int64_t F, const float* z,
                             const float* envmap, const float* view, float* image, float* normal, float* depth, float* alpha, int B, int H, int W, int EH,
                             int EW, int quad, int subpixel, void* workspace, size_t workspace_bytes, const void* bvh, size_t bvh_bytes, void* stream);
int drm_brdf_eval(const float* z, int z_rows, const float* n, const float* v, const float* l, float* out, int64_t N, void* stream);

#define DRM_LOSS_L1 0
#define DRM_LOSS_L2 1
#define DRM_LOSS_WORKSPACE_BYTES 2048
int drm_validation_losses(const float* model_out, const float* Lr_k, const float* Lr_km1, const int32_t* K, const float* z_out, const float* z_k,
                          const float* z_K, const int32_t* reversed_k, const float* z0, double gamma, int loss_type, double l_refmap_weight,
                          double l_refcode_weight, int B, int64_t per_row, int P, void* workspace, size_t workspace_bytes, float* out, void* stream);

#define DRM_PAD_ZEROS 0
#define DRM_PAD_NOISE 1
int drm_obs_forward_process(const float* x, const float* mask, const int32_t* t, const float* sqrt_alphas_cumprod,
                            const float* sqrt_one_minus_alphas_cumprod, int T, float noisy_observe, int padding_mode, const float* e_observe,
                            const float* e_padding, const float* e_q, uint64_t seed, float* cond, float* x_noisy, float* noise, int B, int C, int H,
                            int W, int mask_H, int mask_W, void* stream);
#define DRM_DIFFUSION_LOSS_MAX_PARTS 32
#define DRM_DIFFUSION_LOSS_WORKSPACE_BYTES(B) ((size_t)(B) * DRM_DIFFUSION_LOSS_MAX_PARTS * 2 * sizeof(double))
int drm_diffusion_losses(const float* model_out, const float* target, const float* invmask, const int32_t* t, const float* logvar,
                         const float* lvlb_weights, int T, int loss_type, double l_simple_weight, double original_elbo_weight, int B,
                         int64_t per_row, int C, void* workspace, size_t workspace_bytes, float* out, float* loss_simple_rows, void* stream);

#ifdef __cplusplus
}
#endif
#endif
```

Baseline: 888.6.

## Fold GroupNorm finalize into conv prologue per XCD image range for larger batches

Extends the GroupNorm-finalize fold into the conv pipeline prologue. Previously it applied only to batches of at most 4. Now each XCD finalizes just the images its tile range covers, using a batched, unrolled finalize routine, up to a capped range. It also enables the fold for the 4-tap parity upconv split path. This removes separate gn_finalize kernel launches for bigger batches. In exchange each workgroup does redundant finalize work for several images in its prologue, which adds prologue latency.

```diff
diff --git a/drmnet_amd/_lib.py b/drmnet_amd/_lib.py
--- a/drmnet_amd/_lib.py
+++ b/drmnet_amd/_lib.py
@@ -28,6 +28,7 @@
     "drm_profile_enable", "drm_profile_reset", "drm_profile_collect", "drm_unet_set_precision", "drm_set_op_precision",
     "drm_refmap_workspace_bytes", "drm_refmap_mask_make", "drm_erode_mask",
     "drm_unet_load_params_set", "drm_unet_use_set", "drm_set_graph_replay", "drm_set_upconv_split", "drm_graph_launches",
+    "drm_set_gn_fold", "drm_conv_xcd_images", "drm_conv_max_xcd_images", "drm_conv_plan_gn_fold",
     "drm_map_chain", "drm_masked_log_range", "drm_luminance_scale", "drm_mirmap2envmap", "drm_hdr2ldr", "drm_resize", "drm_profile_variants",
     "drm_render_refmap", "drm_brdf_eval", "drm_render_refmap_views", "drm_validation_losses",
     "drm_render_refmap_lit", "drm_render_light_workspace_bytes",
@@ -172,6 +173,10 @@
     L.drm_profile_collect.argtypes = [C.POINTER(C.c_double), C.POINTER(C.c_double), C.POINTER(C.c_double), C.POINTER(C.c_int64)]
     L.drm_set_graph_replay.argtypes = [i32]
     L.drm_set_upconv_split.argtypes = [i32]
+    L.drm_set_gn_fold.argtypes = [i32]
+    L.drm_conv_xcd_images.argtypes = [i32, i32, i32, i32, C.POINTER(C.c_int), C.POINTER(C.c_int)]
+    L.drm_conv_max_xcd_images.argtypes = [i32, i32, i32]
+    L.drm_conv_plan_gn_fold.argtypes = [i32, i32, i32, i32, i32, i32, i32, C.POINTER(C.c_int)]
     L.drm_graph_launches.restype = C.c_int64
     L.drm_map_chain.argtypes = [fp, fp, C.c_int64, i32, C.POINTER(C.c_int32), C.POINTER(C.c_float), i32, fp, fp, fp, vp]
     L.drm_masked_log_range.argtypes = [fp, fp, i32, i32, i32, fp, fp, vp]
diff --git a/drmnet_amd/csrc/abi.hip b/drmnet_amd/csrc/abi.hip
--- a/drmnet_amd/csrc/abi.hip
+++ b/drmnet_amd/csrc/abi.hip
@@ -447,6 +447,40 @@
   });
 }
 
+int drm_set_gn_fold(int mode) {
+  return guarded([&]() -> int {
+    DRM_REQUIRE(mode >= 0 && mode <= 2, "GroupNorm fold mode: 0 = batches of at most 4 only, 1 = by the measured rule, 2 = wherever the routine takes the range");
+    set_gn_fold(mode);
+    return DRM_OK;
+  });
+}
+int drm_conv_xcd_images(int N, int images_per_tile, int tiles_per_group, int xcd, int* first, int* last) {
+  if (N <= 0 || images_per_tile <= 0 || tiles_per_group <= 0 || xcd < 0 || xcd > 7 || !first || !last) return -1;
+  if ((long long)((N + images_per_tile - 1) / images_per_tile) * tiles_per_group >= (1ll << 31)) return -1;
+  return conv_xcd_images(N, images_per_tile, tiles_per_group, xcd, *first, *last) ? 1 : 0;
+}
+int drm_conv_max_xcd_images(int N, int images_per_tile, int tiles_per_group) {
+  if (N <= 0 || images_per_tile <= 0 || tiles_per_group <= 0) return -1;
+  if ((long long)((N + images_per_tile - 1) / images_per_tile) * tiles_per_group >= (1ll << 31)) return -1;
+  return conv_max_xcd_images(N, images_per_tile, tiles_per_group);
+}
+int drm_conv_plan_gn_fold(int N, int H, int W, int Cin, int Cout, int taps, int precision, int* out) {
+  return guarded([&]() -> int {
+    DRM_REQUIRE(out && N > 0 && H > 0 && W > 0 && Cin > 0 && Cout > 0 && (taps == 9 || taps == 1) && precision_valid(precision), "drm_conv_plan_gn_fold: arguments");
+    ConvArgs a;
+    a.C0 = Cin; a.N = N; a.H = H; a.W = W; a.taps = taps; a.Cout = Cout; a.mx_site = taps == 9;
+    const ConvPlan p = plan_conv(a, precision, false, true);
+    DRM_REQUIRE(p.kernel == CONV_PIPELINE, "drm_conv_plan_gn_fold: the shape does not run on the pipeline kernel");
+    static const int bm[] = {256, 256, 256, 128, 256, 128, 128}, bn[] = {256, 192, 128, 128, 64, 64, 32};
+    out[0] = p.th; out[1] = p.tw;
+    out[2] = bm[p.tile] / (p.th * p.tw);
+    out[3] = ((H + p.th - 1) / p.th) * ((W + p.tw - 1) / p.tw) * (Cout / bn[p.tile]);
+    out[4] = conv_plan_max_xcd_images(a, p);
+    out[5] = p.folds_gn() ? 1 : 0;
+    return DRM_OK;
+  });
+}
+
 int drm_set_graph_replay(int on) {
   set_graph_replay(on != 0);
   return DRM_OK;
diff --git a/drmnet_amd/csrc/common.h b/drmnet_amd/csrc/common.h
--- a/drmnet_amd/csrc/common.h
+++ b/drmnet_amd/csrc/common.h
@@ -104,9 +104,13 @@
   size_t tickets = 0;
   bool pool = false;
   bool gn_fold = false;
+  bool gn_fold_range = false;
+  bool folds_gn() const { return gn_fold || gn_fold_range; }
   bool split() const { return kernel == CONV_PIPELINE && terms != 0; }
 };
 ConvPlan plan_conv(const ConvArgs& a, int precision, bool want_pool = false, bool gn_foldable = false);
+void set_gn_fold(int mode);
+int conv_plan_max_xcd_images(const ConvArgs& a, const ConvPlan& p);
 bool conv_split_weights(int precision, int cin);
 int launch_conv(const ConvArgs& a, const ConvPlan& p, hipStream_t s);
 int conv_tile_family(int H, int W, const int (*fam)[2], int n_fam);
diff --git a/drmnet_amd/csrc/conv_split2.hip b/drmnet_amd/csrc/conv_split2.hip
--- a/drmnet_amd/csrc/conv_split2.hip
+++ b/drmnet_amd/csrc/conv_split2.hip
@@ -227,9 +227,8 @@
   const int n_tiles = a.Cout / C::BN;
   const int total = ((a.N + C::TN - 1) / C::TN) * tiles_y * tiles_x * n_tiles;
   const int xcd = blockIdx.x & 7, jx = blockIdx.x >> 3;
-  const int q8 = total >> 3, r8 = total & 7;
-  const int x_start = xcd < r8 ? xcd * (q8 + 1) : r8 * (q8 + 1) + (xcd - r8) * q8;
-  const int x_count = q8 + (xcd < r8 ? 1 : 0);
+  int x_start, x_count;
+  conv_xcd_tiles(total, xcd, x_start, x_count);
   const int J = ((int)gridDim.x - xcd + 7) >> 3;
   auto decode = [&](int logical) {
     TilePos t;
@@ -490,11 +489,14 @@
   }
   S2_STAMP(61);
   if (a.gnf.mom0) {
+    static_assert(GN_FOLD_RANGE_CAP * GN_FOLD_SCRATCH * (int)sizeof(float) <= C::A_F4 * 16, "GroupNorm fold scratch: the activation tile");
     float* scr = reinterpret_cast<float*>(As);
     const bool tab_in_lds = a.N == 1 && (80 + 2 * Ctot) * (int)sizeof(float) <= C::A_F4 * 16;
 #pragma unroll
     for (int p = 0; p < C::A_SLOTS; ++p) load_A_piece(cur, 0, p);
-    for (int n = 0; n < a.N; ++n) gn_finalize_image(a.gnf, n, tid, C::NTHR, scr, tab_in_lds ? scr + 80 : nullptr);
+    int gn_lo = 0, gn_hi = 0;
+    conv_xcd_images(a.N, C::TN, tiles_y * tiles_x * n_tiles, xcd, gn_lo, gn_hi);
+    gn_finalize_range<4>(a.gnf, gn_lo, gn_hi - gn_lo + 1, tid, C::NTHR, scr, tab_in_lds ? scr + 80 : nullptr);
     S2_STAMP(62);
     wait_vmcnt<0>();
     if (!tab_in_lds) {
@@ -1184,8 +1186,8 @@
   DRM_REQUIRE(!POOL || (a.pool_stat && a.stat_out && a.ksplit <= 1 && !a.out_nchw), "pooled output: needs both statistics tables, no split-K");
   if constexpr (TAPS == 4) {
     static_assert(!RAG && !SK && !POOL, "the parity form has no ragged, split-K or pooled instantiation");
-    DRM_REQUIRE(!a.bias && !a.emb && !a.res && !a.stat_out && !a.out_nchw && a.ksplit <= 1 && !a.gnf.mom0 && !a.in_inv && a.w_img_stride_f4 == 0,
-                "parity (4-tap) conv: weight un-scaling only -- no bias, emb, residual, statistics, split-K or GroupNorm fold");
+    DRM_REQUIRE(!a.bias && !a.emb && !a.res && !a.stat_out && !a.out_nchw && a.ksplit <= 1 && !a.in_inv && a.w_img_stride_f4 == 0,
+                "parity (4-tap) conv: weight un-scaling only -- no bias, emb, residual, statistics or split-K");
     DRM_REQUIRE(a.C1 == 0 && !a.up0 && a.Cout % 4 == 0 && (a.Cout / 4) % C::BN == 0, "parity (4-tap) conv: one stored source, a Cout tile inside one parity");
   }
   const size_t lds_bytes = (size_t)(C::LDS_F4 + (POOL ? C::ST_F4 : 0)) * sizeof(float4);
@@ -1200,6 +1202,8 @@
   const int groups = (a.N + C::TN - 1) / C::TN;
   const long long tiles = (long long)groups * ((a.H + TH - 1) / TH) * ((a.W + TW - 1) / TW) * (a.Cout / C::BN);
   DRM_REQUIRE(tiles > 0 && tiles < (1ll << 31), "conv grid size");
+  DRM_REQUIRE(!a.gnf.mom0 || conv_max_xcd_images(a.N, C::TN, (int)(tiles / groups)) <= GN_FOLD_RANGE_CAP,
+              "GroupNorm fold: an XCD's tile range holds more images than the prologue finalises (plan_conv decides)");
   const int per_cu = std::max(1, std::min((int)(di->lds_per_cu / lds_bytes), 8 / C::NW));
   long long grid = (long long)di->cus * per_cu;
   const int ngt = ((a.C0 + a.C1) / C::KC) * C::NG;
@@ -1344,6 +1348,19 @@
 
 constexpr long long S2_MIN_WIDE_TILES = 176;
 constexpr int GN_FOLD_MAX_N = 4;
+constexpr int GN_FOLD_MAX_RANGE = 5;
+static std::atomic<int> g_gn_fold{1};
+void set_gn_fold(int mode) { g_gn_fold.store(mode); }
+int conv_plan_max_xcd_images(const ConvArgs& a, const ConvPlan& p) {
+  static const int bm[] = {256, 256, 256, 128, 256, 128, 128}, bn[] = {256, 192, 128, 128, 64, 64, 32};
+  const int tn = bm[p.tile] / (p.th * p.tw);
+  return conv_max_xcd_images(a.N, tn, ((a.H + p.th - 1) / p.th) * ((a.W + p.tw - 1) / p.tw) * (a.Cout / bn[p.tile]));
+}
+static void plan_gn_fold_range(const ConvArgs& a, ConvPlan& p, bool gn_foldable) {
+  const int mode = g_gn_fold.load(std::memory_order_relaxed);
+  if (!gn_foldable || p.gn_fold || mode == 0) return;
+  p.gn_fold_range = conv_plan_max_xcd_images(a, p) <= (mode == 2 ? GN_FOLD_RANGE_CAP : GN_FOLD_MAX_RANGE);
+}
 
 bool conv_split_weights(int precision, int cin) { return precision != PREC_FP32 && cin % 32 == 0; }
 
@@ -1378,6 +1395,7 @@
     p.th = fam[f][0]; p.tw = fam[f][1];
     p.ragged = true;
     p.tile = a.Cout % 64 == 0 ? TILE_128x64 : TILE_128x32;
+    plan_gn_fold_range(a, p, gn_foldable);
     return p;
   }
   int wide = 1;
@@ -1414,6 +1432,7 @@
     p.finish = (hw >= 128 && wide == 1) ? SPLIT_IN_LAUNCH : SPLIT_REDUCE;
     if (p.finish == SPLIT_IN_LAUNCH) p.tickets = ((size_t)a.N * hw / 128 + (size_t)hw / 16 + 2) * (size_t)(a.Cout / 32);
   }
+  plan_gn_fold_range(a, p, gn_foldable);
   return p;
 }
 
diff --git a/drmnet_amd/csrc/engine.hip b/drmnet_amd/csrc/engine.hip
--- a/drmnet_amd/csrc/engine.hip
+++ b/drmnet_amd/csrc/engine.hip
@@ -434,7 +434,7 @@
   if (!plain(pa)) return u;
   u.a4.C0 = x0.C; u.a4.N = a.N; u.a4.H = a.H >> 1; u.a4.W = a.W >> 1; u.a4.taps = 4; u.a4.Cout = 4 * r.cout; u.a4.mx_site = 1;
   u.b9.C0 = x1->C; u.b9.N = a.N; u.b9.H = a.H; u.b9.W = a.W; u.b9.taps = 9; u.b9.Cout = r.cout; u.b9.mx_site = 1;
-  u.p4 = plan_conv(u.a4, c.precision);
+  u.p4 = plan_conv(u.a4, c.precision, false, true);
   u.p9 = plan_conv(u.b9, c.precision);
   if (!plain(u.p4) || !plain(u.p9)) return u;
   static const int tile_bn[] = {256, 192, 128, 128, 64, 64, 32};
@@ -467,9 +467,10 @@
     k.C0 = C0; k.C1 = C1; k.N = c.N; k.H = H; k.W = W; k.taps = 1; k.Cout = r.cout;
     pk = plan_conv(k, c.precision);
   }
-  DRM_TRY(gn_params(c, x0, x1, Wb + r.n1_w, Wb + r.n1_b, sc1, sh1, pk.split() ? &k : nullptr, pa.gn_fold ? &a : nullptr));
+  UpconvSplit up = plan_upconv_split(c, r, a, pa, x0, x1);
+  ConvArgs* fold1 = up.on ? (up.p4.folds_gn() ? &up.a4 : nullptr) : (pa.folds_gn() ? &a : nullptr);
+  DRM_TRY(gn_params(c, x0, x1, Wb + r.n1_w, Wb + r.n1_b, sc1, sh1, pk.split() ? &k : nullptr, fold1));
   splitk_workspace(c, a, pa);
-  UpconvSplit up = plan_upconv_split(c, r, a, pa, x0, x1);
   if (up.on) {
     if (!c.dry()) {
       ConvArgs& a4 = up.a4;
@@ -493,7 +494,7 @@
   ConvArgs b;
   b.src0 = h1.p; b.C0 = r.cout; b.N = c.N; b.H = H; b.W = W; b.taps = 9; b.Cout = r.cout; b.mx_site = 1;
   const ConvPlan pb = plan_conv(b, c.precision, pool != nullptr, true);
-  DRM_TRY(gn_params(c, h1, nullptr, Wb + r.n2_w, Wb + r.n2_b, sc2, sh2, nullptr, pb.gn_fold ? &b : nullptr));
+  DRM_TRY(gn_params(c, h1, nullptr, Wb + r.n2_w, Wb + r.n2_b, sc2, sh2, nullptr, pb.folds_gn() ? &b : nullptr));
   splitk_workspace(c, b, pb);
   if (pooled) *pooled = pb.pool;
   if (pb.pool) DRM_TRY(expect_raw_sums(c, *pool));
@@ -530,7 +531,7 @@
   ConvArgs a;
   a.C0 = C; a.N = c.N; a.H = H; a.W = W; a.taps = 1; a.Cout = 3 * C;
   const ConvPlan pa = plan_conv(a, c.precision, false, true);
-  DRM_TRY(gn_params(c, x, nullptr, Wb + l.n_w, Wb + l.n_b, sc, sh, nullptr, pa.gn_fold ? &a : nullptr));
+  DRM_TRY(gn_params(c, x, nullptr, Wb + l.n_w, Wb + l.n_b, sc, sh, nullptr, pa.folds_gn() ? &a : nullptr));
   Act qkv_act = new_act(c, 3 * C, H, W);
   float* qkv = qkv_act.p;
   const AttnPlan ap = plan_attention(c.N, H, W, C, c.precision);
diff --git a/drmnet_amd/csrc/gn.hip b/drmnet_amd/csrc/gn.hip
--- a/drmnet_amd/csrc/gn.hip
+++ b/drmnet_amd/csrc/gn.hip
@@ -79,12 +79,12 @@
                                                            float* __restrict__ scale, float* __restrict__ shift, double cnt0, double cnt1,
                                                            float* __restrict__ guard_scale, float* __restrict__ guard_shift,
                                                            float* __restrict__ guard_inv) {
-  __shared__ __attribute__((aligned(16))) float scratch[72];
+  __shared__ __attribute__((aligned(16))) float scratch[GN_FOLD_SCRATCH];
   GnFold f;
   f.mom0 = mom0; f.mom1 = mom1; f.C0 = C0; f.C1 = C1; f.inv0 = inv0; f.inv1 = inv1; f.cnt0 = cnt0; f.cnt1 = cnt1;
   f.gamma = gamma; f.beta = beta; f.scale = scale; f.shift = shift;
   f.guard_scale = guard_scale; f.guard_shift = guard_shift; f.guard_inv = guard_inv;
-  gn_finalize_image(f, blockIdx.x, threadIdx.x, 256, scratch);
+  gn_finalize_range<1>(f, blockIdx.x, 1, threadIdx.x, 256, scratch);
 }
 
 __global__ __launch_bounds__(256) void act_pow2_scale_kernel(const double2* __restrict__ mom0, int C0, int lo0, int hi0, double cnt0,
@@ -141,6 +141,8 @@
                        const float* beta, int N, float* scale, float* shift, hipStream_t s, double cnt0, double cnt1, float* guard_scale,
                        float* guard_shift, float* guard_inv) {
   DRM_REQUIRE((C0 + C1) % 32 == 0, "GroupNorm32 needs channels % 32 == 0");
+  if (prof_enabled()) prof_variant("drm::gn_finalize_kernel");
+  ProfScope ps(PROF_GNSTATS, 10.0 * N * (C0 + C1), 24.0 * N * (C0 + C1), s);
   hipLaunchKernelGGL(gn_finalize_kernel, dim3(N), dim3(256), 0, s, mom0, C0, inv0, mom1, C1, inv1, gamma, beta, scale, shift, cnt0, cnt1, guard_scale,
                      guard_shift, guard_inv);
   DRM_HIP_CHECK(hipGetLastError());
diff --git a/drmnet_amd/csrc/gn_fold.h b/drmnet_amd/csrc/gn_fold.h
--- a/drmnet_amd/csrc/gn_fold.h
+++ b/drmnet_amd/csrc/gn_fold.h
@@ -18,6 +18,29 @@
   float* guard_inv = nullptr;
 };
 
+__host__ __device__ inline void conv_xcd_tiles(int total, int xcd, int& start, int& count) {
+  const int q8 = total >> 3, r8 = total & 7;
+  start = xcd < r8 ? xcd * (q8 + 1) : r8 * (q8 + 1) + (xcd - r8) * q8;
+  count = q8 + (xcd < r8 ? 1 : 0);
+}
+__host__ __device__ inline bool conv_xcd_images(int N, int TN, int per_group, int xcd, int& n_lo, int& n_hi) {
+  int start, count;
+  conv_xcd_tiles(((N + TN - 1) / TN) * per_group, xcd, start, count);
+  if (count <= 0) return false;
+  n_lo = (start / per_group) * TN;
+  n_hi = ((start + count - 1) / per_group) * TN + TN - 1;
+  if (n_hi > N - 1) n_hi = N - 1;
+  return true;
+}
+__host__ __device__ inline int conv_max_xcd_images(int N, int TN, int per_group) {
+  int most = 0;
+  for (int x = 0; x < 8; ++x) {
+    int lo, hi;
+    if (conv_xcd_images(N, TN, per_group, x, lo, hi) && hi - lo + 1 > most) most = hi - lo + 1;
+  }
+  return most;
+}
+
 __device__ __forceinline__ void gn_lds_barrier() {
   asm volatile("s_waitcnt lgkmcnt(0)" ::: "memory");
   __builtin_amdgcn_s_barrier();
@@ -25,9 +48,10 @@
 }
 
 constexpr int GN_FOLD_PRELOAD = 6;
-__device__ __forceinline__ void gn_finalize_image(const GnFold& f, int n, int t, int nthreads, float* lds, float* lds_tab = nullptr) {
-  float* g_mean = lds;
-  float* g_rstd = lds + 32;
+constexpr int GN_FOLD_SCRATCH = 72;
+constexpr int GN_FOLD_RANGE_CAP = 8;
+template <int U>
+__device__ __forceinline__ void gn_finalize_range(const GnFold& f, int n_lo, int cnt, int t, int nthreads, float* lds, float* lds_tab = nullptr) {
   const int C0 = f.C0, C1 = f.C1, C = C0 + C1, cpg = C / 32;
   float gm[GN_FOLD_PRELOAD], bt[GN_FOLD_PRELOAD];
   const bool pre = C <= GN_FOLD_PRELOAD * nthreads;
@@ -39,90 +63,112 @@
       bt[k] = f.beta[c];
     }
   }
-  if (f.guard_scale) {
-    double* red = reinterpret_cast<double*>(lds + 64);
-    double m = 0.0;
-    if (t < 256) {
-      for (int c = t; c < C; c += 256)
-        m = fmax(m, c < C0 ? f.mom0[(size_t)n * C0 + c].y * (f.cnt0 > 0 ? f.cnt0 : 1.0) : f.mom1[(size_t)n * C1 + (c - C0)].y * (f.cnt1 > 0 ? f.cnt1 : 1.0));
+  if (t < 256) {
+    for (int i0 = 0; i0 < cnt; i0 += U) {
+      if (f.guard_scale) {
+        const double s0 = f.cnt0 > 0 ? f.cnt0 : 1.0, s1 = f.cnt1 > 0 ? f.cnt1 : 1.0;
+        double m[U];
 #pragma unroll
-      for (int o = 32; o > 0; o >>= 1) m = fmax(m, __shfl_xor(m, o));
-      if ((t & 63) == 0) red[t >> 6] = m;
-    }
-    gn_lds_barrier();
-    const double bound = sqrt(fmax(fmax(red[0], red[1]), fmax(red[2], red[3])));
-    int k = 0;
-    if (bound > 0.0 && bound < INFINITY) {
-      int e;
-      frexp(bound, &e);
-      k = 15 - e;
-      k = k > 90 ? 90 : (k < -90 ? -90 : k);
-    }
-    const float gs = ldexpf(1.0f, k);
-    if (t == 0) f.guard_inv[n] = ldexpf(1.0f, -k);
-    for (int c = t; c < C; c += nthreads) {
-      f.guard_scale[(size_t)n * C + c] = gs;
-      f.guard_shift[(size_t)n * C + c] = 0.f;
-    }
-  }
-  if (t < 256) {
-    const int g = t >> 3, j = t & 7;
-    double m = 0.0, q = 0.0;
-    for (int k = j; k < cpg; k += 8) {
-      const int c = g * cpg + k;
-      if (c < C0) {
-        const double2 v = f.mom0[(size_t)n * C0 + c];
-        m += v.x * f.inv0;
-        q += v.y * f.inv0;
-      } else {
-        const double2 v = f.mom1[(size_t)n * C1 + (c - C0)];
-        m += v.x * f.inv1;
-        q += v.y * f.inv1;
+        for (int u = 0; u < U; ++u) m[u] = 0.0;
+        for (int c = t; c < C; c += 256) {
+          const bool first = c < C0;
+          const double2* src = first ? f.mom0 + c : f.mom1 + (c - C0);
+          const size_t ld = first ? C0 : C1;
+          const double s = first ? s0 : s1;
+          double y[U];
+#pragma unroll
+          for (int u = 0; u < U; ++u) y[u] = src[(size_t)(n_lo + min(i0 + u, cnt - 1)) * ld].y;
+#pragma unroll
+          for (int u = 0; u < U; ++u) m[u] = fmax(m[u], y[u] * s);
+        }
+#pragma unroll
+        for (int u = 0; u < U; ++u) {
+#pragma unroll
+          for (int o = 32; o > 0; o >>= 1) m[u] = fmax(m[u], __shfl_xor(m[u], o));
+          if ((t & 63) == 0 && i0 + u < cnt) reinterpret_cast<double*>(lds + (i0 + u) * GN_FOLD_SCRATCH + 64)[t >> 6] = m[u];
+        }
       }
-    }
+      const int g = t >> 3, j = t & 7;
+      double m[U], q[U];
 #pragma unroll
-    for (int o = 4; o > 0; o >>= 1) {
-      m += __shfl_xor(m, o);
-      q += __shfl_xor(q, o);
-    }
-    if (j == 0) {
-      m /= cpg;
-      q /= cpg;
-      double var = q - m * m;
-      if (var < 0.0) var = 0.0;
-      g_mean[g] = (float)m;
-      g_rstd[g] = (float)(1.0 / sqrt(var + 1e-5));
+      for (int u = 0; u < U; ++u) m[u] = q[u] = 0.0;
+      for (int k = j; k < cpg; k += 8) {
+        const int c = g * cpg + k;
+        const bool first = c < C0;
+        const double2* src = first ? f.mom0 + c : f.mom1 + (c - C0);
+        const size_t ld = first ? C0 : C1;
+        const double inv = first ? f.inv0 : f.inv1;
+        double2 v[U];
+#pragma unroll
+        for (int u = 0; u < U; ++u) v[u] = src[(size_t)(n_lo + min(i0 + u, cnt - 1)) * ld];
+#pragma unroll
+        for (int u = 0; u < U; ++u) {
+          m[u] += v[u].x * inv;
+          q[u] += v[u].y * inv;
+        }
+      }
+#pragma unroll
+      for (int u = 0; u < U; ++u) {
+#pragma unroll
+        for (int o = 4; o > 0; o >>= 1) {
+          m[u] += __shfl_xor(m[u], o);
+          q[u] += __shfl_xor(q[u], o);
+        }
+        if (j == 0 && i0 + u < cnt) {
+          const double mean = m[u] / cpg, sq = q[u] / cpg;
+          double var = sq - mean * mean;
+          if (var < 0.0) var = 0.0;
+          float* st = lds + (i0 + u) * GN_FOLD_SCRATCH;
+          st[g] = (float)mean;
+          st[32 + g] = (float)(1.0 / sqrt(var + 1e-5));
+        }
+      }
     }
   }
   gn_lds_barrier();
-  if (pre) {
-#pragma unroll
-    for (int k = 0; k < GN_FOLD_PRELOAD; ++k) {
-      const int c = t + k * nthreads;
-      if (c < C) {
-        const int g = c / cpg;
-        const float sc = g_rstd[g] * gm[k], sh = bt[k] - g_mean[g] * sc;
-        f.scale[(size_t)n * C + c] = sc;
-        f.shift[(size_t)n * C + c] = sh;
-        if (lds_tab) {
-          lds_tab[c] = sc;
-          lds_tab[C + c] = sh;
-        }
+  if (f.guard_scale) {
+    for (int i = 0; i < cnt; ++i) {
+      const double* red = reinterpret_cast<const double*>(lds + i * GN_FOLD_SCRATCH + 64);
+      const double bound = sqrt(fmax(fmax(red[0], red[1]), fmax(red[2], red[3])));
+      int k = 0;
+      if (bound > 0.0 && bound < INFINITY) {
+        int e;
+        frexp(bound, &e);
+        k = 15 - e;
+        k = k > 90 ? 90 : (k < -90 ? -90 : k);
+      }
+      const float gs = ldexpf(1.0f, k);
+      const size_t row = (size_t)(n_lo + i) * C;
+      if (t == 0) f.guard_inv[n_lo + i] = ldexpf(1.0f, -k);
+      for (int c = t; c < C; c += nthreads) {
+        f.guard_scale[row + c] = gs;
+        f.guard_shift[row + c] = 0.f;
       }
     }
-  } else {
-    for (int c = t; c < C; c += nthreads) {
-      const int g = c / cpg;
-      const float sc = g_rstd[g] * f.gamma[c], sh = f.beta[c] - g_mean[g] * sc;
-      f.scale[(size_t)n * C + c] = sc;
-      f.shift[(size_t)n * C + c] = sh;
+  }
+  auto put = [&](int c, float gamma, float beta) {
+    const int g = c / cpg;
+    for (int i = 0; i < cnt; ++i) {
+      const float* st = lds + i * GN_FOLD_SCRATCH;
+      const float sc = st[32 + g] * gamma, sh = beta - st[g] * sc;
+      f.scale[(size_t)(n_lo + i) * C + c] = sc;
+      f.shift[(size_t)(n_lo + i) * C + c] = sh;
       if (lds_tab) {
         lds_tab[c] = sc;
         lds_tab[C + c] = sh;
       }
     }
+  };
+  if (pre) {
+#pragma unroll
+    for (int k = 0; k < GN_FOLD_PRELOAD; ++k) {
+      const int c = t + k * nthreads;
+      if (c < C) put(c, gm[k], bt[k]);
+    }
+  } else {
+    for (int c = t; c < C; c += nthreads) put(c, f.gamma[c], f.beta[c]);
   }
-  gn_lds_barrier();
+  if (lds_tab) gn_lds_barrier();
 }
 
 }
diff --git a/drmnet_amd/ops.py b/drmnet_amd/ops.py
--- a/drmnet_amd/ops.py
+++ b/drmnet_amd/ops.py
@@ -20,6 +20,10 @@
 
 def set_upconv_split(mode: int) -> None:
     _lib.check(_lib.lib().drm_set_upconv_split(int(mode)))
+
+
+def set_gn_fold(mode: int) -> None:
+    _lib.check(_lib.lib().drm_set_gn_fold(int(mode)))
 
 
 UPCONV_TAP_GROUPS = {0: {0: (0,), 1: (1, 2)}, 1: {0: (0, 1), 1: (2,)}}
diff --git a/include/drmnet_hip.h b/include/drmnet_hip.h
--- a/include/drmnet_hip.h
+++ b/include/drmnet_hip.h
@@ -125,6 +125,11 @@
 int drm_set_graph_replay(int on);
 
 int drm_set_upconv_split(int mode);
+
+int drm_set_gn_fold(int mode);
+int drm_conv_xcd_images(int N, int images_per_tile, int tiles_per_group, int xcd, int* first, int* last);
+int drm_conv_max_xcd_images(int N, int images_per_tile, int tiles_per_group);
+int drm_conv_plan_gn_fold(int N, int H, int W, int Cin, int Cout, int taps, int precision, int* out);
 int64_t drm_graph_launches(void);
 
 #define DRM_PROFILE_KINDS 5
```

Result: no change. 883.8 (-0.5%).
